# krisbrud/gym-auv

Measured on NVIDIA B200. Metric: env-steps/sec (180-ray LiDAR, whole box), higher is better.
Workload: dtype f32 ray casting on f64 state/culling

## Files before the change

gym_auv_b200/_lib.py:

```python
from __future__ import annotations

import ctypes as C
import os

_HERE = os.path.dirname(os.path.abspath(__file__))
LIB_PATH = os.environ.get("AUV_B200_LIB", os.path.join(_HERE, "libauv_b200.so"))
ABI_VERSION = 22
REC_BYTES = 80
MAX_POLY_VERTS = 192
STATUS_REC_OVERFLOW = 1
STATUS_GEN_GAVE_UP = 2
STATUS_POLY_TOO_LARGE = 4
STATUS_PATH_TOO_LONG = 8
STATUS_BOUNDS = 16
STATUS_GEN_LAND_BLOCKED = 32
PP_W = 12
PATH_STAGE_BLOCKS = 512
NAV_W = 24
N_STATS = 16
STAT_NAMES = [
    "episodes",
    "reward",
    "reward_sq",
    "progress",
    "collisions",
    "reached_goal",
    "timesteps",
    "cross_track_error",
    "pathlength",
    "steps",
]

OBSERVE_STEP = 0
OBSERVE_RESET = 1
REWARDER_IDS = {"colav": 0, "pathfollow": 1}
CULL_IDS = {"reference": 0, "exact": 1}
VELOCITY_IDS = {"zero": 0, "nearest": 1}

_vp = C.c_void_p


class AuvConfig(C.Structure):
    _fields_ = [
        ("t_step_size", C.c_double),
        ("thrust_max_auv", C.c_double),
        ("moment_max_auv", C.c_double),
        ("vessel_width", C.c_double),
        ("look_ahead_distance", C.c_double),
        ("sensor_range", C.c_double),
        ("min_goal_distance", C.c_double),
        ("min_path_progress", C.c_double),
        ("min_cumulative_reward", C.c_double),
        ("feasibility_width_multiplier", C.c_double),
        ("max_timesteps", C.c_int32),
        ("sensor_interval_load_obstacles", C.c_int32),
        ("n_sensors", C.c_int32),
        ("n_sectors", C.c_int32),
        ("use_lidar", C.c_int32),
        ("sensor_log_transform", C.c_int32),
        ("sensor_use_velocity_observations", C.c_int32),
        ("rewarder", C.c_int32),
        ("test_mode", C.c_int32),
        ("cull_mode", C.c_int32),
        ("auto_reset", C.c_int32),
        ("velocity_mode", C.c_int32),
    ]


class AuvRayTable(C.Structure):
    _fields_ = [("cos_sin", _vp), ("weight", _vp), ("sector", _vp), ("unit64", _vp), ("weight_sum", C.c_double)]


class AuvPathHdr(C.Structure):
    _fields_ = [
        ("v0", C.c_int32),
        ("nseg", C.c_int32),
        ("b0", C.c_int32),
        ("s0", C.c_int32),
        ("ox", C.c_double),
        ("oy", C.c_double),
        ("length", C.c_double),
        ("end_x", C.c_double),
        ("end_y", C.c_double),
        ("extent", C.c_double),
    ]


class AuvPathBank(C.Structure):
    _fields_ = [
        ("n_paths", C.c_int32),
        ("n_knots", C.c_int32),
        ("hdr", _vp),
        ("poly_xy", _vp),
        ("poly_cum", _vp),
        ("poly_f32", _vp),
        ("blk_chord", _vp),
        ("blk_dev", _vp),
        ("sb_chord", _vp),
        ("sb_dev", _vp),
        ("pp", _vp),
        ("sub_chord", _vp),
        ("sub_dev", _vp),
    ]


class AuvScenarioPool(C.Structure):
    _fields_ = [
        ("n_scenarios", C.c_int32),
        ("k_moving", C.c_int32),
        ("k_static", C.c_int32),
        ("n_world", C.c_int32),
        ("path_id", _vp),
        ("vessel_init", _vp),
        ("mov_start", _vp),
        ("mov_width", _vp),
        ("mov_track", _vp),
        ("mov_pos0", _vp),
        ("mov_disp0", _vp),
        ("mov_counter0", _vp),
        ("vel_table", _vp),
        ("st_pos", _vp),
        ("st_radius", _vp),
        ("st_rec", _vp),
        ("mov_lin", _vp),
        ("linear_tracks", C.c_int32),
        ("lin_first_wrap", C.c_int32),
        ("lin_wrap_period", C.c_int32),
        ("reserved0", C.c_int32),
        ("world_circle", _vp),
        ("world_voff", _vp),
        ("world_verts", _vp),
        ("world_cell_off", _vp),
        ("world_cell_items", _vp),
        ("world_grid_x0", C.c_double),
        ("world_grid_y0", C.c_double),
        ("world_grid_cell", C.c_double),
        ("world_grid_nx", C.c_int32),
        ("world_grid_ny", C.c_int32),
        ("reset_obs", _vp),
        ("reset_max_progress", _vp),
        ("reset_mask", _vp),
    ]


class AuvBatch(C.Structure):
    _fields_ = [
        ("n_envs", C.c_int32),
        ("mask_words", C.c_int32),
        ("env_offset", C.c_int32),
        ("reset_stride", C.c_int32),
        ("scn_id", _vp),
        ("episode", _vp),
        ("state", _vp),
        ("step_counter", _vp),
        ("t_step", _vp),
        ("cum_reward", _vp),
        ("max_progress", _vp),
        ("cte_sum", _vp),
        ("nearby_mask", _vp),
        ("mov_pos", _vp),
        ("mov_disp", _vp),
        ("mov_counter", _vp),
        ("nav", _vp),
        ("rec", _vp),
        ("rec_cnt", _vp),
        ("status", _vp),
        ("rec_cap", C.c_int32),
        ("reserved1", C.c_int32),
        ("obst_steps", _vp),
        ("prev_seg", _vp),
        ("env_pid", _vp),
    ]


class AuvStepOut(C.Structure):
    _fields_ = [
        ("obs", _vp),
        ("reward", _vp),
        ("done", _vp),
        ("collision", _vp),
        ("reached_goal", _vp),
        ("goal_distance", _vp),
        ("progress", _vp),
        ("lidar_dist", _vp),
        ("windows", _vp),
        ("terminal_obs", _vp),
        ("sector_min_dist", _vp),
        ("sector_feasible_dist", _vp),
        ("stats", _vp),
        ("seg_tests", _vp),
        ("episode_out", _vp),
        ("tracks", _vp),
    ]


class AuvTracks(C.Structure):
    _fields_ = [("count", C.c_int32), ("stride", C.c_int32), ("capacity", C.c_int32), ("reserved0", C.c_int32),
                ("points", _vp), ("head", _vp), ("snap", _vp)]


TRACK_HEAD_W = 8


def track_snap_width(k_moving: int, k_static: int) -> int:
    return 4 + 8 * int(k_moving) + 4 * int(k_static)


class AuvGenParams(C.Structure):
    _fields_ = [
        ("seed", C.c_uint64),
        ("epoch", C.c_uint32),
        ("post_generate_update", C.c_int32),
        ("t_step_size", C.c_double),
        ("vessel_width", C.c_double),
        ("init_pos_jitter", C.c_double),
        ("mov_disp_std", C.c_double),
        ("mov_width_mean", C.c_double),
        ("mov_speed_lo", C.c_double),
        ("mov_speed_hi", C.c_double),
        ("st_disp_std", C.c_double),
        ("st_radius_mean", C.c_double),
        ("path_group", C.c_int32),
        ("path_period", C.c_int32),
        ("land_clearance", C.c_double),
    ]


class AuvRefreshScratch(C.Structure):
    _fields_ = [("seen_episode", _vp), ("ids", _vp), ("count", _vp), ("capacity", C.c_int32), ("reserved0", C.c_int32)]


class AuvPathBuild(C.Structure):
    _fields_ = [("hdr", _vp), ("poly_xy", _vp), ("poly_cum", _vp), ("poly_f32", _vp), ("blk_chord", _vp), ("blk_dev", _vp),
                ("sb_chord", _vp), ("sb_dev", _vp), ("pp", _vp), ("n_knots", C.c_int32), ("vcap", C.c_int32),
                ("sub_chord", _vp), ("sub_dev", _vp)]


class AuvCompact(C.Structure):
    _fields_ = [("head", _vp), ("mask", _vp), ("vals", _vp), ("counter", _vp), ("words", C.c_int32), ("capacity", C.c_int32)]


class AuvDelta(C.Structure):
    _fields_ = [("obs_host", _vp), ("shadow", _vp), ("shipped", _vp), ("gran", C.c_int32), ("ctas", C.c_int32)]


EXPORTS = [
    "auv_abi_version",
    "auv_sizeof",
    "auv_last_error",
    "auv_obs_dim",
    "auv_obstacle_update",
    "auv_vessel_step",
    "auv_navigate",
    "auv_observe",
    "auv_reset",
    "auv_step",
    "auv_step_host",
    "auv_fma_probe",
    "auv_timer_create",
    "auv_timer_destroy",
    "auv_step_timed",
    "auv_timer_read",
    "auv_pipeline_create",
    "auv_pipeline_destroy",
    "auv_pipeline_graph_state",
    "auv_step_chunked",
    "auv_step_host_chunked",
    "auv_step_host_submit",
    "auv_generate_moving_obstacles",
    "auv_linear_wrap",
    "auv_pool_pack",
    "auv_obstacle_state",
    "auv_reset_cache_fill",
    "auv_refresh_finished",
    "auv_step_host_compact_submit",
    "auv_step_host_delta_submit",
    "auv_compact_expand",
    "auv_pathbank_build",
    "auv_random_curve_waypoints",
]

_lib = None


class AuvLibraryError(RuntimeError):
    pass


def load():
    global _lib
    if _lib is not None:
        return _lib
    if not os.path.exists(LIB_PATH):
        raise AuvLibraryError(
            f"{LIB_PATH} not found: build it with `python -m gym_auv_b200.build` "
            "(or __graft_entry__.build()).  There is no CPU fallback."
        )
    lib = C.CDLL(LIB_PATH)
    for name in EXPORTS:
        if not hasattr(lib, name):
            raise AuvLibraryError(f"{LIB_PATH} does not export {name}")
    lib.auv_abi_version.restype = C.c_int
    lib.auv_last_error.restype = C.c_char_p
    lib.auv_obs_dim.argtypes = [C.POINTER(AuvConfig)]
    P = C.POINTER
    lib.auv_obstacle_update.argtypes = [P(AuvConfig), P(AuvScenarioPool), P(AuvBatch), _vp]
    lib.auv_vessel_step.argtypes = [P(AuvConfig), P(AuvBatch), _vp, _vp]
    lib.auv_observe.argtypes = [
        P(AuvConfig), P(AuvRayTable), P(AuvPathBank), P(AuvScenarioPool), P(AuvBatch), P(AuvStepOut), C.c_int, _vp,
    ]
    lib.auv_navigate.argtypes = [P(AuvConfig), P(AuvRayTable), P(AuvPathBank), P(AuvScenarioPool), P(AuvBatch), _vp]
    lib.auv_reset.argtypes = [P(AuvConfig), P(AuvScenarioPool), P(AuvBatch), _vp, _vp]
    lib.auv_step.argtypes = [
        P(AuvConfig), P(AuvRayTable), P(AuvPathBank), P(AuvScenarioPool), P(AuvBatch), _vp, P(AuvStepOut), _vp,
    ]
    lib.auv_step_host.argtypes = [
        P(AuvConfig), P(AuvRayTable), P(AuvPathBank), P(AuvScenarioPool), P(AuvBatch), _vp, _vp, P(AuvStepOut),
        _vp, _vp, _vp, _vp,
    ]
    lib.auv_pipeline_create.argtypes = [C.c_int]
    lib.auv_pipeline_create.restype = _vp
    lib.auv_pipeline_destroy.argtypes = [_vp]
    lib.auv_pipeline_destroy.restype = None
    lib.auv_pipeline_graph_state.argtypes = [_vp]
    lib.auv_step_chunked.argtypes = [
        P(AuvConfig), P(AuvRayTable), P(AuvPathBank), P(AuvScenarioPool), P(AuvBatch), _vp, P(AuvStepOut), _vp,
        _vp, C.c_int,
    ]
    lib.auv_step_host_chunked.argtypes = [
        P(AuvConfig), P(AuvRayTable), P(AuvPathBank), P(AuvScenarioPool), P(AuvBatch), _vp, _vp, P(AuvStepOut),
        _vp, _vp, _vp, _vp, _vp, C.c_int,
    ]
    lib.auv_step_host_submit.argtypes = lib.auv_step_host_chunked.argtypes
    lib.auv_generate_moving_obstacles.argtypes = [P(AuvGenParams), P(AuvPathBank), P(AuvScenarioPool), _vp, C.c_int, _vp, _vp]
    lib.auv_linear_wrap.argtypes = [C.c_double, C.c_double, C.c_int, P(C.c_int32), P(C.c_int32)]
    lib.auv_pool_pack.argtypes = [P(AuvConfig), P(AuvScenarioPool), _vp, C.c_int, _vp]
    lib.auv_obstacle_state.argtypes = [P(AuvConfig), P(AuvScenarioPool), P(AuvBatch), _vp, _vp, _vp, _vp]
    lib.auv_reset_cache_fill.argtypes = [P(AuvConfig), P(AuvRayTable), P(AuvPathBank), P(AuvScenarioPool), P(AuvBatch),
                                         P(AuvStepOut), _vp, C.c_int, C.c_int, _vp]
    lib.auv_refresh_finished.argtypes = [P(AuvConfig), P(AuvRayTable), P(AuvPathBank), P(AuvScenarioPool), P(AuvBatch),
                                         P(AuvBatch), P(AuvStepOut), P(AuvRefreshScratch), P(AuvGenParams), _vp]
    lib.auv_step_host_compact_submit.argtypes = [
        P(AuvConfig), P(AuvRayTable), P(AuvPathBank), P(AuvScenarioPool), P(AuvBatch), _vp, _vp, P(AuvStepOut),
        P(AuvCompact), _vp, _vp, _vp, _vp, C.c_int,
    ]
    lib.auv_step_host_delta_submit.argtypes = [
        P(AuvConfig), P(AuvRayTable), P(AuvPathBank), P(AuvScenarioPool), P(AuvBatch), _vp, _vp, P(AuvStepOut),
        P(AuvDelta), _vp, _vp, _vp, _vp, C.c_int,
    ]
    lib.auv_compact_expand.argtypes = [P(AuvConfig), C.c_int, P(AuvCompact), _vp, _vp, C.c_int]
    lib.auv_pathbank_build.argtypes = [_vp, _vp, _vp, C.c_int, P(AuvPathBuild), _vp, _vp]
    lib.auv_random_curve_waypoints.argtypes = [C.c_uint64, C.c_uint32, C.c_double, _vp, C.c_int, _vp, _vp, _vp]
    lib.auv_timer_create.argtypes = [C.c_int]
    lib.auv_timer_create.restype = _vp
    lib.auv_timer_destroy.argtypes = [_vp]
    lib.auv_timer_destroy.restype = None
    lib.auv_step_timed.argtypes = [
        P(AuvConfig), P(AuvRayTable), P(AuvPathBank), P(AuvScenarioPool), P(AuvBatch), _vp, P(AuvStepOut), _vp,
        _vp, C.c_int,
    ]
    lib.auv_timer_read.argtypes = [_vp, C.c_int, P(C.c_float)]
    lib.auv_fma_probe.argtypes = [_vp, C.c_int, C.c_int, C.c_int, _vp, P(C.c_double)]
    ver = lib.auv_abi_version()
    if ver != ABI_VERSION:
        raise AuvLibraryError(f"ABI mismatch: library {ver}, binding {ABI_VERSION}; rebuild")
    lib.auv_sizeof.argtypes = [C.c_int]
    for i, st in enumerate([AuvConfig, AuvRayTable, AuvPathBank, AuvScenarioPool, AuvBatch, AuvStepOut, AuvGenParams,
                            AuvPathHdr, AuvRefreshScratch, AuvCompact, AuvPathBuild, AuvDelta, AuvTracks]):
        if lib.auv_sizeof(i) != C.sizeof(st):
            raise AuvLibraryError(f"struct layout mismatch for {st.__name__}: C {lib.auv_sizeof(i)} vs ctypes {C.sizeof(st)}")
    _lib = lib
    return lib


def check(rc: int, what: str):
    if rc != 0:
        msg = load().auv_last_error().decode("utf-8", "replace")
        raise AuvLibraryError(f"{what} failed (rc={rc}): {msg}")
```

gym_auv_b200/csrc/auv_kernels.cu:

```cuda
#include "auv_device.cuh"
#include "auv_dynamics.cuh"
#include "auv_geometry.cuh"
#include "auv_navigate.cuh"
#include "auv_generate.cuh"
#include "auv_pathbuild.cuh"
#include "../../include/auv_b200.h"

#include <math.h>

namespace auv {

struct ObstLoad {
  double w, counter;
  int4 tr;
  double2 pos;
};
__device__ __forceinline__ ObstLoad obstacle_load(const AuvScenarioPool& pool, const AuvBatch& batch, long long pe,
                                                  long long ps) {
  ObstLoad o;
  o.w = pool.mov_width[ps];
  o.counter = batch.mov_counter[pe];
  o.tr = reinterpret_cast<const int4*>(pool.mov_track)[ps];
  o.pos = reinterpret_cast<const double2*>(batch.mov_pos)[pe];
  return o;
// ... 127 lines not shown
  double hx, hy;
  float ecx, ecy, rho;
  int a, b;
  int flags;
  int nv;
  int vbase;
  float step_len;
  int pad;
};
static_assert(sizeof(ObstRec) == AUV_REC_BYTES, "ObstRec layout");

__device__ __forceinline__ void reset_env_thread(const AuvScenarioPool& pool, const AuvBatch& batch, int e,
                                                 int scn) {
  const int n = batch.n_envs;
  const int km = pool.k_moving;
  batch.scn_id[e] = scn;
  batch.env_pid[e] = pool.path_id[scn];
  batch.prev_seg[e] = -1;
  batch.obst_steps[e] = 0;
  batch.episode[e] += 1;
  const double* vi = pool.vessel_init + 3ll * scn;
  batch.state[e] = vi[0];
  batch.state[n + e] = vi[1];
  batch.state[2 * n + e] = vi[2];
  batch.state[3 * n + e] = 0.0;
  batch.state[4 * n + e] = 0.0;
  batch.state[5 * n + e] = 0.0;
  batch.step_counter[e] = 0;
  batch.t_step[e] = 0;
  batch.cum_reward[e] = 0.0;
  batch.max_progress[e] = 0.0;
  batch.cte_sum[e] = 0.0;
  if (!pool.linear_tracks)
    for (int j = 0; j < km; ++j) {
      const long long ps = (long long)scn * km + j, pe = (long long)e * km + j;
      reinterpret_cast<double2*>(batch.mov_pos)[pe] = reinterpret_cast<const double2*>(pool.mov_pos0)[ps];
      reinterpret_cast<double2*>(batch.mov_disp)[pe] = reinterpret_cast<const double2*>(pool.mov_disp0)[ps];
      batch.mov_counter[pe] = pool.mov_counter0[ps];
    }
  for (int w = 0; w < batch.mask_words; ++w) batch.nearby_mask[(long long)e * batch.mask_words + w] = 0u;
}

__global__ void __launch_bounds__(128) k_reset(AuvScenarioPool pool, AuvBatch batch,
                                               const uint8_t* __restrict__ reset_mask) {
  const int e = blockIdx.x * blockDim.x + threadIdx.x;
  if (e >= batch.n_envs) return;
  if (reset_mask != nullptr && reset_mask[e] == 0) return;
  reset_env_thread(pool, batch, e, batch.scn_id[e]);
}

struct SlotGeom {
  bool valid, pent, world;
  double cx, cy, rho, geo, hx, hy;
  float step_len;
  int nv, vbase;
};

__device__ __forceinline__ SlotGeom load_slot(const AuvScenarioPool& pool, const AuvBatch& batch, int e, int scn,
                                              int j, double px, double py, int n_upd) {
  SlotGeom g;
  g.valid = g.pent = g.world = false;
  g.cx = g.cy = g.rho = g.geo = 0.0;
  g.hx = 1.0;
  g.hy = 0.0;
  g.step_len = 0.f;
  g.nv = g.vbase = 0;
  const int km = pool.k_moving, ks = pool.k_static, K = km + ks;
  if (j >= K) {
    const int wi = j - K;
    const double* c3 = pool.world_circle + 3ll * wi;
    g.vbase = pool.world_voff[wi];
    g.nv = pool.world_voff[wi + 1] - g.vbase;
    g.valid = g.nv >= 4;
    g.world = true;
    g.cx = c3[0] - px;
    g.cy = c3[1] - py;
    g.rho = c3[2];
  } else if (j < km) {
    const long long ps = (long long)scn * km + j;
    double w;
    double2 pos, dsp;
    if (pool.linear_tracks) {
      const double2* __restrict__ r = reinterpret_cast<const double2*>(pool.mov_lin + ps * 8);
      const double2 p0 = r[0];
      dsp = r[1];
      w = r[2].x;
      pos = p0;
      if (w > 0.0) {
        pos = lin_position(pool, r, p0, dsp, n_upd);
        if (n_upd == 0) dsp = reinterpret_cast<const double2*>(pool.mov_disp0)[ps];
      }
    } else {
      const long long pe = (long long)e * km + j;
      w = pool.mov_width[ps];
      pos = reinterpret_cast<const double2*>(batch.mov_pos)[pe];
      dsp = reinterpret_cast<const double2*>(batch.mov_disp)[pe];
    }
    if (w > 0.0) {
      g.valid = g.pent = true;
      g.geo = w;
      const double dl2 = dsp.x * dsp.x + dsp.y * dsp.y;
      if (dl2 > 0.0) {
        const double inv = rsqrt(dl2);
        g.hx = dsp.x * inv;
        g.hy = dsp.y * inv;
        g.step_len = (float)(dl2 * inv);
      }
      g.cx = (pos.x - px) + w * (5.0 / 18.0) + (w * (2.0 / 9.0)) * g.hx;
      g.cy = (pos.y - py) + (w * (2.0 / 9.0)) * g.hy;
      g.rho = w * 1.1180339887498949;
      g.nv = 6;
    }
  } else {
    const double2* __restrict__ r = reinterpret_cast<const double2*>(pool.st_rec + ((long long)scn * ks + (j - km)) * 4);
    const double2 c = r[0];
    const double rad = r[1].x;
    if (rad > 0.0) {
      g.valid = true;
      g.geo = rad;
      g.cx = c.x - px;
      g.cy = c.y - py;
      g.rho = rad;
      g.nv = ngon_sides(rad) + 1;
    }
  }
  return g;
}

__device__ __forceinline__ bool slot_is_near(const AuvScenarioPool& pool, const AuvBatch& batch,
                                             const double2* __restrict__ unit64, int e, int scn, int j, double px,
                                             double py, int n_upd, double range, double width) {
  const SlotGeom g = load_slot(pool, batch, e, scn, j, px, py, n_upd);
  if (!g.valid) return false;
  const double dc = sqrt(g.cx * g.cx + g.cy * g.cy);
  if (dc - g.rho - width >= range + 1e-6) return false;
  if (dc + g.rho - width < range - 1e-6) return true;
  const double bx0 = g.cx - (g.geo * (2.0 / 9.0)) * g.hx, by0 = g.cy - (g.geo * (2.0 / 9.0)) * g.hy;
  bool in_dummy;
  const double dist = g.world ? world_polygon_distance(reinterpret_cast<const double2*>(pool.world_verts) + g.vbase, g.nv, px,
                                                       py, in_dummy)
                              : boundary_distance(g.pent, g.cx, g.cy, bx0, by0, g.geo, g.hx, g.hy, g.nv, unit64);
  return (dist - width) < range;
}

#ifndef AUV_CULL_COOP
#define AUV_CULL_COOP 1
#endif
template <int G>
__device__ __forceinline__ void cull_env_group(const AuvConfig& cfg, const AuvScenarioPool& pool,
                                               const AuvBatch& batch, const double2* __restrict__ unit64,
                                               int* __restrict__ windows_out, int e, int scn, double px,
                                               double py, double psi, int step_counter, int n_upd, const int lane,
                                               const unsigned gm, const bool store) {
  const int sub = lane & (G - 1);
  const int R = cfg.n_sensors;
  const int S = pool.k_moving + pool.k_static + pool.n_world;
  const bool refresh = (step_counter % cfg.sensor_interval_load_obstacles) == 0;
  const double range = cfg.sensor_range, width = cfg.vessel_width;
  ObstRec* rec = reinterpret_cast<ObstRec*>(batch.rec) + (long long)e * batch.rec_cap;
  int cnt = 0;
  const int K = pool.k_moving + pool.k_static;
  const bool grid = pool.world_cell_off != nullptr && pool.n_world > 0;
  const int S_scan = grid ? K : S;
#if AUV_CULL_COOP
  const unsigned rmask = __ballot_sync(AUV_FULL, refresh && sub == 0 && store);
  for (unsigned rm = rmask; rm; rm &= rm - 1) {
    const int src = __ffs(rm) - 1;
    const int eb = __shfl_sync(AUV_FULL, e, src), sb = __shfl_sync(AUV_FULL, scn, src);
    const int nb = __shfl_sync(AUV_FULL, n_upd, src);
    const double pxb = __shfl_sync(AUV_FULL, px, src), pyb = __shfl_sync(AUV_FULL, py, src);
    for (int base = 0; base < S; base += 32) {
      unsigned word = 0u;
      if (base < S_scan) {
        const int j = base + lane;
        word = __ballot_sync(AUV_FULL, j < S_scan && slot_is_near(pool, batch, unit64, eb, sb, j, pxb, pyb, nb, range, width));
      }
      if (lane == src) batch.nearby_mask[(long long)eb * batch.mask_words + (base >> 5)] = word;
    }
  }
  if (rmask) __syncwarp();
#endif
  if (refresh) {
#if !AUV_CULL_COOP
    for (int base = 0; base < S; base += 32) {
      unsigned word = 0u;
      if (base < S_scan) {
#pragma unroll 1
        for (int k = 0; k < 32 / G; ++k) {
          const int j = base + k * G + sub;
          const bool near = j < S_scan && slot_is_near(pool, batch, unit64, e, scn, j, px, py, n_upd, range, width);
          word |= group_ballot<G>(gm, lane, near) << (k * G);
        }
      }
      if (store && sub == 0) batch.nearby_mask[(long long)e * batch.mask_words + (base >> 5)] = word;
    }
#endif
    if (grid) {
      __syncwarp(gm);
      const double rq = range + width + 1e-3, cell = pool.world_grid_cell;
      const int ix0 = max(0, (int)floor((px - rq - pool.world_grid_x0) / cell));
      const int ix1 = min(pool.world_grid_nx - 1, (int)floor((px + rq - pool.world_grid_x0) / cell));
      const int iy0 = max(0, (int)floor((py - rq - pool.world_grid_y0) / cell));
      const int iy1 = min(pool.world_grid_ny - 1, (int)floor((py + rq - pool.world_grid_y0) / cell));
      for (int iy = iy0; iy <= iy1; ++iy)
        for (int ix = ix0; ix <= ix1; ++ix) {
          const int c = iy * pool.world_grid_nx + ix;
          const int i0 = pool.world_cell_off[c], i1 = pool.world_cell_off[c + 1];
          for (int it = i0 + sub; it < i1; it += G) {
            const int j = K + pool.world_cell_items[it];
            if (store && slot_is_near(pool, batch, unit64, e, scn, j, px, py, n_upd, range, width))
              atomicOr(batch.nearby_mask + (long long)e * batch.mask_words + (j >> 5), 1u << (j & 31));
          }
        }
    }
    __syncwarp(gm);
  }
  for (int base = 0; base < S; base += 32) {
    const unsigned* mw = batch.nearby_mask + (long long)e * batch.mask_words + (base >> 5);
    const unsigned word = refresh ? __ldcg(mw) : *mw;
    if (windows_out != nullptr && store) {
      for (int j = base + sub; j < min(S, base + 32); j += G)
        reinterpret_cast<int2*>(windows_out)[(long long)e * S + j] = make_int2(0, 0);
      __syncwarp(gm);
    }
    const int nw = __popc(word);
    for (int r = sub; r < nw; r += G) {
      unsigned wv = word;
      for (int t = 0; t < r; ++t) wv &= wv - 1;
      const int j = base + __ffs(wv) - 1;
      const SlotGeom g = load_slot(pool, batch, e, scn, j, px, py, n_upd);
      int wa = 0, wb = 0;
      bool allrays = false, inside = false;
      double bx0 = 0.0, by0 = 0.0;
      if (g.valid) {
        int lo, hi;
        cull_bounds(g.cx, g.cy, g.rho, psi, R, lo, hi);
        window_from_bounds(lo, hi, R, cfg.cull_mode, wa, wb, allrays);
        bx0 = g.cx - (g.geo * (2.0 / 9.0)) * g.hx;
        by0 = g.cy - (g.geo * (2.0 / 9.0)) * g.hy;
        if (g.cx * g.cx + g.cy * g.cy <= g.rho * g.rho) {
          if (g.pent)
            inside = vessel_inside_pentagon(bx0, by0, g.geo, g.hx, g.hy);
          else if (g.world)
            world_polygon_distance(reinterpret_cast<const double2*>(pool.world_verts) + g.vbase, g.nv, px, py, inside);
        }
      }
      if (!store) continue;
      if (windows_out != nullptr) reinterpret_cast<int2*>(windows_out)[(long long)e * S + j] = make_int2(wa, wb);
      const int idx = cnt + r;
      AUV_CHECK(batch.status, j >= 0 && j < S && idx >= 0);
      if (idx >= batch.rec_cap) {
        if (batch.status != nullptr) atomicOr(batch.status, AUV_STATUS_REC_OVERFLOW);
        continue;
      }
      ObstRec q;
      q.cx = g.pent ? bx0 : g.cx;
      q.cy = g.pent ? by0 : g.cy;
      q.geo = g.geo;
      q.hx = g.hx;
      q.hy = g.hy;
      q.ecx = (float)g.cx;
      q.ecy = (float)g.cy;
      q.rho = (float)g.rho;
      q.a = wa;
      q.b = wb;
      q.flags = (g.pent ? (OFLAG_FILLED | OFLAG_PENTAGON) : 0) | (g.world ? (OFLAG_FILLED | OFLAG_WORLD) : 0) |
                (inside ? OFLAG_INSIDE : 0) | (allrays ? OFLAG_ALLRAYS : 0);
      q.nv = g.valid ? g.nv : 1;
      q.vbase = g.vbase;
      q.step_len = g.step_len;
      q.pad = 0;
      rec[idx] = q;
    }
    cnt = min(cnt + nw, batch.rec_cap);
  }
  if (store && sub == 0) {
    batch.rec_cnt[e] = cnt;
    batch.nav[(long long)e * AUV_NAV_W + NAV_CNT] = (double)cnt;
  }
}

__global__ void __launch_bounds__(128) k_worker_fill(AuvBatch wb, const int* __restrict__ ids, int first, int n,
                                                     const int* __restrict__ n_dev) {
  const int w = blockIdx.x * blockDim.x + threadIdx.x;
  if (w >= wb.n_envs) return;
  if (n_dev != nullptr) n = min(n, *n_dev);
  const int k = n > 0 ? min(w, n - 1) : 0;
  wb.scn_id[w] = ids ? ids[k] : first + k;
}
__global__ void __launch_bounds__(128) k_cache_scatter(AuvScenarioPool pool, AuvBatch wb, const float* __restrict__ wobs,
                                                       int obs_dim, int use_lidar, int n, const int* __restrict__ n_dev) {
  const int w = (blockIdx.x * blockDim.x + threadIdx.x) >> 5, lane = threadIdx.x & 31;
  if (n_dev != nullptr) n = min(n, *n_dev);
  if (w >= n || w >= wb.n_envs) return;
  const int m = wb.scn_id[w];
  float* dst = const_cast<float*>(pool.reset_obs) + (long long)m * obs_dim;
  const float* src = wobs + (long long)w * obs_dim;
  for (int k = lane; k < obs_dim; k += 32) dst[k] = src[k];
  if (lane == 0) const_cast<double*>(pool.reset_max_progress)[m] = wb.max_progress[w];
  if (use_lidar)
    for (int k = lane; k < wb.mask_words; k += 32)
      const_cast<uint32_t*>(pool.reset_mask)[(long long)m * wb.mask_words + k] = wb.nearby_mask[(long long)w * wb.mask_words + k];
}
__global__ void __launch_bounds__(128) k_refresh_collect(AuvBatch live, int n_scenarios, int* __restrict__ seen,
                                                         int* __restrict__ ids, int* __restrict__ count, int capacity) {
  const int e = blockIdx.x * blockDim.x + threadIdx.x;
  if (e >= live.n_envs) return;
  const int ep = live.episode[e];
  if (ep == seen[e]) return;
  const int k = atomicAdd(count, 1);
  if (k >= capacity) return;
  seen[e] = ep;
  ids[k] = (int)(((long long)live.scn_id[e] + (live.reset_stride > 0 ? live.reset_stride : live.n_envs)) % n_scenarios);
}

template <int G>
__device__ __noinline__ void obstacle_update_group(const AuvConfig& cfg, const AuvScenarioPool& pool, const AuvBatch& batch,
                                                   int e, int scn, int sub, bool store) {
  if (!store) return;
  const int km = pool.k_moving;
  const long long pe0 = (long long)e * km, ps0 = (long long)scn * km;
  for (int j = sub; j < km; j += 2 * G) {
    const bool two = j + G < km;
    const ObstLoad a = obstacle_load(pool, batch, pe0 + j, ps0 + j);
    const ObstLoad b = obstacle_load(pool, batch, pe0 + (two ? j + G : j), ps0 + (two ? j + G : j));
    obstacle_finish(cfg, pool, batch, pe0 + j, ps0 + j, a);
    if (two) obstacle_finish(cfg, pool, batch, pe0 + j + G, ps0 + j + G, b);
  }
}

__device__ __forceinline__ unsigned smem_u32(const void* p) { return (unsigned)__cvta_generic_to_shared(p); }
__device__ __forceinline__ void mbar_init(unsigned long long* bar, unsigned count) {
  asm volatile("mbarrier.init.shared::cta.b64 [%0], %1;" ::"r"(smem_u32(bar)), "r"(count) : "memory");
  asm volatile("fence.mbarrier_init.release.cluster;" ::: "memory");
}
__device__ __forceinline__ void mbar_expect_tx(unsigned long long* bar, unsigned bytes) {
  asm volatile("mbarrier.arrive.expect_tx.shared::cta.b64 _, [%0], %1;" ::"r"(smem_u32(bar)), "r"(bytes) : "memory");
}
__device__ __forceinline__ void bulk_g2s(void* dst, const void* src, unsigned bytes, unsigned long long* bar) {
  asm volatile("cp.async.bulk.shared::cluster.global.mbarrier::complete_tx::bytes [%0], [%1], %2, [%3];" ::"r"(smem_u32(dst)),
               "l"(src), "r"(bytes), "r"(smem_u32(bar))
               : "memory");
}
__device__ __forceinline__ void mbar_wait(unsigned long long* bar, unsigned parity) {
  asm volatile(
      "{\n"
      ".reg .pred p;\n"
      "AUV_WAIT:\n"
      "mbarrier.try_wait.parity.shared::cta.b64 p, [%0], %1;\n"
      "@p bra AUV_DONE;\n"
      "bra AUV_WAIT;\n"
      "AUV_DONE:\n"
      "}\n" ::"r"(smem_u32(bar)),
      "r"(parity)
      : "memory");
}

#ifndef AUV_NAV_G
#define AUV_NAV_G 4
#endif
#ifndef AUV_NAV_THREADS
#define AUV_NAV_THREADS 128
#endif
#ifndef AUV_NAV_MINB
#define AUV_NAV_MINB (1024 / AUV_NAV_THREADS)
#endif
#ifndef AUV_NAV_PHASE_SYNC
#define AUV_NAV_PHASE_SYNC 0
#endif
constexpr int NAV_STAGE_SB = (AUV_PATH_STAGE_BLOCKS + AUV_PATH_SUPER - 1) / AUV_PATH_SUPER;
constexpr int NAV_SUBBLOCKS = AUV_NAV_THREADS / 128;
struct __align__(16) NavStage {
  float4 chord[AUV_PATH_STAGE_BLOCKS];
  float2 aux[AUV_PATH_STAGE_BLOCKS];
  float4 sbc[NAV_STAGE_SB];
  float2 sba[NAV_STAGE_SB];
};
#ifndef AUV_NAV_SPLIT
#define AUV_NAV_SPLIT 1
#endif
template <bool DYN, bool OBST, int G>
__global__ void __launch_bounds__(AUV_NAV_THREADS, AUV_NAV_MINB) k_vessel_nav(const __grid_constant__ AuvConfig cfg,
                                                                const __grid_constant__ AuvPathBank paths,
                                                                const __grid_constant__ AuvScenarioPool pool,
                                                                const __grid_constant__ AuvBatch batch,
                                                                const double2* __restrict__ unit64,
                                                                int* __restrict__ windows_out,
                                                                const float* __restrict__ actions,
                                                                float* __restrict__ obs_out, int obs_dim, int e0, int e1) {
  extern __shared__ __align__(16) unsigned char nav_smem[];
  NavStage* stages = reinterpret_cast<NavStage*>(nav_smem);
  __shared__ __align__(8) unsigned long long s_bar[NAV_SUBBLOCKS];
  __shared__ int s_pid[AUV_NAV_THREADS / 32];
  const int lane = threadIdx.x & 31, sub = lane & (G - 1);
  const int sbk = threadIdx.x >> 7, tsb = threadIdx.x & 127;
  NavStage& st = stages[sbk];
  const unsigned gm = group_mask<G>(lane);
  const int eraw = e0 + (blockIdx.x * AUV_NAV_THREADS + threadIdx.x) / G;
  const bool store = eraw < e1;
  const int e = store ? eraw : e1 - 1;
  const int n = batch.n_envs;
  const int scn = batch.scn_id[e];
  const int pid = batch.env_pid[e];
  const int prev_seg = batch.prev_seg[e];
  int step_counter = batch.step_counter[e];
  int n_upd = batch.obst_steps[e];
  S6 y = load_state(batch.state, n, e);
  float2 act = make_float2(0.f, 0.f);
  if (DYN) act = reinterpret_cast<const float2*>(actions)[e];
  if (tsb == 0) mbar_init(&s_bar[sbk], 1);
  {
    int same;
    __match_all_sync(AUV_FULL, pid, &same);
    if (lane == 0) s_pid[threadIdx.x >> 5] = same ? pid : -1;
  }
  __syncthreads();
  const AuvPathHdr h = paths.hdr[pid];
  const int nblk = (h.nseg + AUV_PATH_BLOCK - 1) / AUV_PATH_BLOCK;
  const int nsb = (nblk + AUV_PATH_SUPER - 1) / AUV_PATH_SUPER;
  bool staged = s_pid[4 * sbk] >= 0 && nblk <= AUV_PATH_STAGE_BLOCKS;
#pragma unroll
  for (int w = 1; w < 4; ++w) staged = staged && s_pid[4 * sbk + w] == s_pid[4 * sbk];
  if (staged && tsb == 0) {
    const unsigned nb2 = (unsigned)(nblk + 1) & ~1u, ns2 = (unsigned)(nsb + 1) & ~1u;
    mbar_expect_tx(&s_bar[sbk], nb2 * 24u + ns2 * 24u);
    bulk_g2s(st.chord, reinterpret_cast<const float4*>(paths.blk_chord) + h.b0, nb2 * 16u, &s_bar[sbk]);
    bulk_g2s(st.aux, reinterpret_cast<const float2*>(paths.blk_dev) + h.b0, nb2 * 8u, &s_bar[sbk]);
    bulk_g2s(st.sbc, reinterpret_cast<const float4*>(paths.sb_chord) + h.s0, ns2 * 16u, &s_bar[sbk]);
    bulk_g2s(st.sba, reinterpret_cast<const float2*>(paths.sb_dev) + h.s0, ns2 * 8u, &s_bar[sbk]);
  }
  if (OBST) {
    ++n_upd;
    if (store && sub == 0) batch.obst_steps[e] = n_upd;
    if (!pool.linear_tracks) {
      obstacle_update_group<G>(cfg, pool, batch, e, scn, sub, store);
      __syncwarp();
    }
  }
  if (DYN) {
    y = vessel_rk_step(cfg, y, act);
    ++step_counter;
    if (store && sub == 0) {
      store_state(batch.state, n, e, y);
      batch.step_counter[e] = step_counter;
    }
  }
  if (AUV_NAV_PHASE_SYNC) __syncthreads();
  PathTabs T;
  if (staged) {
    mbar_wait(&s_bar[sbk], 0);
    T.sbc = st.sbc;
    T.sba = st.sba;
    T.chord = st.chord;
    T.aux = st.aux;
  } else {
    T.sbc = reinterpret_cast<const float4*>(paths.sb_chord) + h.s0;
    T.sba = reinterpret_cast<const float2*>(paths.sb_dev) + h.s0;
    T.chord = reinterpret_cast<const float4*>(paths.blk_chord) + h.b0;
    T.aux = reinterpret_cast<const float2*>(paths.blk_dev) + h.b0;
  }
  int seg;
  const double s = project_group<G>(paths, h, T, y.x, y.y, prev_seg, lane, gm, seg, batch.status);
  AUV_CHECK(batch.status, seg >= 0 && seg < h.nseg && (!staged || (nblk <= AUV_PATH_STAGE_BLOCKS && nsb <= NAV_STAGE_SB)));
  if (store && sub == 0) batch.prev_seg[e] = seg;
  if (AUV_NAV_SPLIT) {
    if (store && sub == 0) batch.nav[(long long)e * AUV_NAV_W + NAV_S] = s;
    return;
  }
  if (AUV_NAV_PHASE_SYNC) __syncthreads();
  navigate_env(cfg, paths, h, batch, pid, e, scn, s, y.x, y.y, y.psi, y.u, y.v, y.r,
               obs_out ? obs_out + (long long)e * obs_dim : nullptr, store && sub == 0);
  if (AUV_NAV_PHASE_SYNC) __syncthreads();
  if (cfg.use_lidar)
    cull_env_group<G>(cfg, pool, batch, unit64, windows_out, e, scn, y.x, y.y, y.psi, step_counter, n_upd, lane, gm, store);
}

template <int G>
__global__ void __launch_bounds__(128, 8) k_nav_cull(const __grid_constant__ AuvConfig cfg, const __grid_constant__ AuvPathBank paths,
                                                     const __grid_constant__ AuvScenarioPool pool,
                                                     const __grid_constant__ AuvBatch batch, const double2* __restrict__ unit64,
                                                     int* __restrict__ windows_out, float* __restrict__ obs_out, int obs_dim,
                                                     int e0, int e1) {
  const int lane = threadIdx.x & 31, sub = lane & (G - 1);
  const unsigned gm = group_mask<G>(lane);
  const int eraw = e0 + (blockIdx.x * 128 + threadIdx.x) / G;
  const bool store = eraw < e1;
  const int e = store ? eraw : e1 - 1;
  const int n = batch.n_envs;
  const int scn = batch.scn_id[e];
  const int pid = batch.env_pid[e];
  const int step_counter = batch.step_counter[e];
  const int n_upd = batch.obst_steps[e];
  const S6 y = load_state(batch.state, n, e);
  const double s = batch.nav[(long long)e * AUV_NAV_W + NAV_S];
  const AuvPathHdr h = paths.hdr[pid];
  __syncwarp();
  navigate_env(cfg, paths, h, batch, pid, e, scn, s, y.x, y.y, y.psi, y.u, y.v, y.r,
               obs_out ? obs_out + (long long)e * obs_dim : nullptr, store && sub == 0);
  if (cfg.use_lidar)
    cull_env_group<G>(cfg, pool, batch, unit64, windows_out, e, scn, y.x, y.y, y.psi, step_counter, n_upd, lane, gm, store);
}

#ifndef AUV_LIDAR_THREADS
#define AUV_LIDAR_THREADS 256
#endif
#ifndef AUV_LIDAR_RCAP
#define AUV_LIDAR_RCAP 96
#endif
#ifndef AUV_LIDAR_MAX_ENVS
#define AUV_LIDAR_MAX_ENVS 32
#endif

struct LidarArgs {
  AuvConfig cfg;
  AuvRayTable rays;
  AuvPathBank paths;
  AuvScenarioPool pool;
  AuvBatch batch;
  AuvStepOut out;
  const void* pad0;
  int mode;
  int obs_dim;
  int e0, e1;
  int envs_per_cta;
  int vmax;
  float pen_clear_ray;
  float inv_log_range;
  double clear_closeness;
  double inv_weight_sum;
  double feas_width;
  AuvTracks trk;
};

struct LidarSmem {
  double* hand;
  void* sdist;
  ObstRec* rec;
  int* rec_env;
  float2* verts;
  float2* unit;
  int* off;
  float* pen;
  int* flag;
  int* next;
};
__host__ __device__ constexpr size_t lidar_smem_bytes_for(int E, int rpad, int vmax, int vel) {
  return (size_t)E * 16 * 8 + (size_t)E * rpad * (vel ? 8 : 4) + AUV_LIDAR_RCAP * sizeof(ObstRec) + AUV_LIDAR_RCAP * 4 +
         (size_t)(AUV_LIDAR_THREADS / 32) * vmax * 8 + 64 * 8 + 48 * 4 + 32 * 4 + 32 * 4 + 32 * 4;
}
__device__ __forceinline__ LidarSmem lidar_carve(unsigned char* p, int E, int rpad, int vmax, int vel) {
  LidarSmem s;
  s.hand = reinterpret_cast<double*>(p);
  p += (size_t)E * 16 * 8;
  s.sdist = p;
  p += (size_t)E * rpad * (vel ? 8 : 4);
  s.rec = reinterpret_cast<ObstRec*>(p);
  p += AUV_LIDAR_RCAP * sizeof(ObstRec);
  s.rec_env = reinterpret_cast<int*>(p);
  p += AUV_LIDAR_RCAP * 4;
  s.verts = reinterpret_cast<float2*>(p);
  p += (size_t)(AUV_LIDAR_THREADS / 32) * vmax * 8;
  s.unit = reinterpret_cast<float2*>(p);
  p += 64 * 8;
  s.off = reinterpret_cast<int*>(p);
  p += 48 * 4;
  s.pen = reinterpret_cast<float*>(p);
  p += 32 * 4;
  s.flag = reinterpret_cast<int*>(p);
  p += 32 * 4;
  s.next = reinterpret_cast<int*>(p);
  return s;
}

__device__ __forceinline__ float cast_ngon(float ecx, float ecy, float rho, int nn, const float2* __restrict__ u64,
                                           float c, float s, float theta, float tc, float hc, float best, float rangef) {
  const float g = asinf(fminf(fmaxf(-hc / rho, -1.f), 1.f));
  const float invd = (float)nn * 0.15915494309189535f;
  const int sh = 6 - (31 - __clz(nn));
  const bool outside = tc * tc + hc * hc > rho * rho * 1.0001f + 1e-3f;
#pragma unroll
  for (int sol = 0; sol < 2; ++sol) {
    if (sol == 1 && outside) break;
    const float p = (sol == 0 ? theta + 3.14159265358979f - g : theta + g) * invd;
    const float kf = floorf(p);
    const int k0 = (int)kf;
    const int first = (p - kf < 0.5f) ? k0 - 1 : k0;
    float xp, yp;
    {
      const float2 un = u64[(first & (nn - 1)) << sh];
      const float vx = fmaf(rho, un.x, ecx), vy = fmaf(rho, un.y, ecy);
      xp = vx * c + vy * s;
      yp = vy * c - vx * s;
    }
#pragma unroll
    for (int w = 1; w <= 2; ++w) {
      const float2 un = u64[((first + w) & (nn - 1)) << sh];
      const float vx = fmaf(rho, un.x, ecx), vy = fmaf(rho, un.y, ecy);
      const float xc = vx * c + vy * s;
      const float yc = vy * c - vx * s;
      if ((yp <= 0.f && yc >= 0.f) || (yp >= 0.f && yc <= 0.f)) {
        const float t = xp + (xc - xp) * (yp / (yp - yc));
        if (t >= 0.f && t <= rangef) best = fminf(best, t);
      }
      xp = xc;
      yp = yc;
    }
  }
  return best;
}

__device__ __forceinline__ float cast_chain(const float2* __restrict__ vp, int nq, float c, float s, float best,
                                            float rangef) {
  float2 v = vp[0];
  float xp = v.x * c + v.y * s;
  float yp = v.y * c - v.x * s;
  for (int k = 1; k < nq; ++k) {
    v = vp[k];
    const float xc = v.x * c + v.y * s;
    const float yc = v.y * c - v.x * s;
    if ((yp <= 0.f && yc >= 0.f) || (yp >= 0.f && yc <= 0.f)) {
      const float t = xp + (xc - xp) * (yp / (yp - yc));
      if (t >= 0.f && t <= rangef) best = fminf(best, t);
    }
    xp = xc;
    yp = yc;
  }
  return best;
}

template <bool VEL>
__device__ __forceinline__ float range_get(const void* row, int i) {
  if (VEL) return __uint_as_float((unsigned)(reinterpret_cast<const unsigned long long*>(row)[i] >> 32));
  return reinterpret_cast<const float*>(row)[i];
}
template <bool VEL>
__device__ __forceinline__ void range_min(void* row, int i, float d, int slot) {
  if (VEL)
    atomicMin(reinterpret_cast<unsigned long long*>(row) + i,
              ((unsigned long long)__float_as_uint(d) << 32) | (unsigned)min(slot, 255));
  else
    atomicMin(reinterpret_cast<int*>(row) + i, __float_as_int(d));
}

#ifndef AUV_LIDAR_MINB
#define AUV_LIDAR_MINB 5
#endif
#ifndef AUV_LIDAR_LONG_POLY
#define AUV_LIDAR_LONG_POLY 1
#endif
template <bool VEL>
__device__ __noinline__ void cast_long_polygon(const double2* __restrict__ wv, int nq, int vmax, float2* wverts, double px,
                                               double py, double cpsi, double spsi, const double2* __restrict__ cos_sin,
                                               float ecx, float ecy, float rho, void* row, int slot, int lane, int n1, int n2,
                                               int lo1, int lo2, float rangef) {
  const float slack = rho * 1e-5f + 1e-4f;
  const int tot = n1 + n2;
  for (int v0 = 0; v0 < nq - 1; v0 += vmax - 1) {
    const int nqc = min(nq - v0, vmax);
    __syncwarp();
    for (int k = lane; k < nqc; k += 32) {
      const double2 w = wv[v0 + k];
      wverts[k] = make_float2((float)(w.x - px), (float)(w.y - py));
    }
    __syncwarp();
    for (int u = lane; u < tot; u += 32) {
      const int i = u < n1 ? lo1 + u : lo2 + (u - n1);
      const float cur = range_get<VEL>(row, i);
      const double2 cs = cos_sin[i];
      const float c = (float)(cs.x * cpsi - cs.y * spsi), sn = (float)(cs.y * cpsi + cs.x * spsi);
      const float tc = ecx * c + ecy * sn;
      const float hc = ecy * c - ecx * sn;
      if (fabsf(hc) > rho + slack || tc + rho + slack < 0.f || tc - rho - slack > cur) continue;
      const float got = cast_chain(wverts, nqc, c, sn, cur, rangef);
      if (got < cur) range_min<VEL>(row, i, got, slot);
    }
  }
}

template <bool COUNT, bool VEL, bool WORLD, bool TRACK = false>
__global__ void __launch_bounds__(AUV_LIDAR_THREADS, AUV_LIDAR_MINB) k_lidar(const __grid_constant__ LidarArgs A) {
  extern __shared__ __align__(16) unsigned char smem_raw[];
  constexpr int NW = AUV_LIDAR_THREADS / 32;
  const AuvConfig& cfg = A.cfg;
  const AuvBatch& batch = A.batch;
  const int tid = threadIdx.x, lane = tid & 31, warp = tid >> 5;
  const int R = cfg.n_sensors;
  const int rpad = cfg.use_lidar ? ((R + 31) & ~31) : 32;
  const int E = A.envs_per_cta;
  const int env0 = A.e0 + blockIdx.x * E;
  const int ne = min(E, A.e1 - env0);
  const LidarSmem sm = lidar_carve(smem_raw, E, rpad, A.vmax, VEL ? 1 : 0);
  const float rangef = (float)cfg.sensor_range;
  const float widthf = (float)cfg.vessel_width;
  const int n = batch.n_envs;
#define HAND(el, k) sm.hand[(el) * 16 + ((k) - NAV_HAND)]

  for (int k = tid; k < ne * 16; k += AUV_LIDAR_THREADS)
    sm.hand[k] = batch.nav[(long long)(env0 + (k >> 4)) * AUV_NAV_W + NAV_HAND + (k & 15)];
  if (cfg.use_lidar) {
    if (tid < 64) {
      const double2 un = reinterpret_cast<const double2*>(A.rays.unit64)[tid];
      sm.unit[tid] = make_float2((float)un.x, (float)un.y);
    }
    if (VEL) {
      const unsigned long long key0 = ((unsigned long long)__float_as_uint(rangef) << 32) | 255ull;
      for (int k = tid; k < ne * rpad; k += AUV_LIDAR_THREADS) reinterpret_cast<unsigned long long*>(sm.sdist)[k] = key0;
    } else {
      for (int k = tid; k < ne * rpad / 4; k += AUV_LIDAR_THREADS)
        reinterpret_cast<float4*>(sm.sdist)[k] = make_float4(rangef, rangef, rangef, rangef);
    }
  }
  __syncthreads();
  unsigned long long ntests = 0;
  if (cfg.use_lidar) {
    if (warp == 0) {
      const int c = lane < ne ? (int)HAND(lane, NAV_CNT) : 0;
      const int incl = warp_incl_scan(c, lane);
      sm.off[lane + 1] = incl;
      if (lane == 0) sm.off[0] = 0;
    }
    __syncthreads();
    const int total = sm.off[ne];
    const double2* __restrict__ unit = reinterpret_cast<const double2*>(A.rays.unit64);
    const double2* __restrict__ cos_sin = reinterpret_cast<const double2*>(A.rays.cos_sin);
    const float dth_f = (float)(2.0 * AUV_PI / (double)R);
    float2* wverts = sm.verts + (size_t)warp * A.vmax;
    for (int r0 = 0; r0 < total; r0 += AUV_LIDAR_RCAP) {
      const int nr = min(AUV_LIDAR_RCAP, total - r0);
      for (int k = tid; k < nr * 5; k += AUV_LIDAR_THREADS) {
        const int r = r0 + k / 5, piece = k - (k / 5) * 5;
        int lo = 0, hi = ne - 1;
        while (lo < hi) {
          const int mid = (lo + hi + 1) >> 1;
          if (sm.off[mid] <= r) lo = mid; else hi = mid - 1;
        }
        const int idx = r - sm.off[lo];
        AUV_CHECK(batch.status, lo >= 0 && lo < ne && idx >= 0 && idx < batch.rec_cap && k < AUV_LIDAR_RCAP * 5);
        const uint4* g = reinterpret_cast<const uint4*>(reinterpret_cast<const ObstRec*>(batch.rec) +
                                                        (long long)(env0 + lo) * batch.rec_cap + idx);
        reinterpret_cast<uint4*>(sm.rec)[k] = g[piece];
        if (piece == 0) sm.rec_env[r - r0] = lo | (idx << 8);
      }
      __syncthreads();
      for (int rr = warp; rr < nr; rr += NW) {
        const ObstRec& q = sm.rec[rr];
        const int el = sm.rec_env[rr] & 255, slot = sm.rec_env[rr] >> 8;
        const int fl = q.flags, nq = q.nv;
        AUV_CHECK(batch.status, rr < AUV_LIDAR_RCAP && el >= 0 && el < ne && slot >= 0 && slot < batch.rec_cap);
        int n1, n2 = 0, lo1 = 0, lo2 = 0;
        if (fl & OFLAG_ALLRAYS) {
          n1 = R;
        } else {
          lo1 = max(q.a, 0);
          const int hi1 = min(q.b, R);
          n1 = max(0, hi1 - lo1);
          lo2 = max(q.a + R, 0);
          if (n1 > 0) lo2 = max(lo2, hi1);
          n2 = max(0, min(q.b + R, R) - lo2);
        }
        const int tot = n1 + n2;
        if (COUNT) {
          for (int i = lane; i < R; i += 32) {
            const int hits = ((q.a <= i && i < q.b) ? 1 : 0) + ((q.a <= i - R && i - R < q.b) ? 1 : 0);
            if ((fl & OFLAG_ALLRAYS) || hits > 0) ntests += (unsigned)((nq - 1) * max(hits, 1));
          }
        }
        if (tot == 0) continue;
        void* row = VEL ? (void*)(reinterpret_cast<unsigned long long*>(sm.sdist) + (size_t)el * rpad)
                        : (void*)(reinterpret_cast<float*>(sm.sdist) + (size_t)el * rpad);
        if (fl & OFLAG_INSIDE) {
          for (int u = lane; u < tot; u += 32) range_min<VEL>(row, u < n1 ? lo1 + u : lo2 + (u - n1), 0.f, slot);
          continue;
        }
        const bool world = WORLD && (fl & OFLAG_WORLD);
        const bool ngon = !(fl & OFLAG_PENTAGON) && !world && nq > 16;
        if (!ngon) {
          if (nq > A.vmax) {
            if (AUV_LIDAR_LONG_POLY && world)
              cast_long_polygon<VEL>(reinterpret_cast<const double2*>(A.pool.world_verts) + q.vbase, nq, A.vmax, wverts,
                                     HAND(el, NAV_X), HAND(el, NAV_Y), HAND(el, NAV_COSPSI), HAND(el, NAV_SINPSI), cos_sin,
                                     q.ecx, q.ecy, q.rho, row, slot, lane, n1, n2, lo1, lo2, rangef);
            else if (lane == 0 && batch.status != nullptr)
              atomicOr(batch.status, AUV_STATUS_POLY_TOO_LARGE);
            continue;
          }
          __syncwarp();
          if (world) {
            const double px = HAND(el, NAV_X), py = HAND(el, NAV_Y);
            const double2* wv = reinterpret_cast<const double2*>(A.pool.world_verts) + q.vbase;
            for (int k = lane; k < nq; k += 32) {
              const double2 w = wv[k];
              wverts[k] = make_float2((float)(w.x - px), (float)(w.y - py));
            }
          } else if (fl & OFLAG_PENTAGON) {
            if (lane < 6) {
              double vx, vy;
              pent_vertex(lane == 5 ? 0 : lane, q.cx, q.cy, q.geo, q.hx, q.hy, vx, vy);
              wverts[lane] = make_float2((float)vx, (float)vy);
            }
          } else {
            const int ne_ = nq - 1, sh = 6 - (31 - __clz(ne_));
            if (lane < nq) {
              const double2 un = __ldg(&unit[(lane == ne_ ? 0 : lane) << sh]);
              wverts[lane] = make_float2((float)(q.cx + q.geo * un.x), (float)(q.cy + q.geo * un.y));
            }
          }
          __syncwarp();
        }
        const double cpsi = HAND(el, NAV_COSPSI), spsi = HAND(el, NAV_SINPSI);
        const float psi_m_pi = (float)(HAND(el, NAV_PSI) - AUV_PI);
        const float ecx = q.ecx, ecy = q.ecy, rho = q.rho;
        const float slack = rho * 1e-5f + 1e-4f;
        AUV_CHECK(batch.status, tot <= R && (n1 == 0 || (lo1 >= 0 && lo1 + n1 <= R)) && (n2 == 0 || (lo2 >= 0 && lo2 + n2 <= R)) &&
                                    (ngon || nq <= A.vmax));
        for (int u = lane; u < tot; u += 32) {
          const int i = u < n1 ? lo1 + u : lo2 + (u - n1);
          AUV_CHECK(batch.status, i >= 0 && i < R && i < rpad);
          const float cur = range_get<VEL>(row, i);
          const double2 cs = cos_sin[i];
          const float c = (float)(cs.x * cpsi - cs.y * spsi), sn = (float)(cs.y * cpsi + cs.x * spsi);
          const float tc = ecx * c + ecy * sn;
          const float hc = ecy * c - ecx * sn;
          if (fabsf(hc) > rho + slack || tc + rho + slack < 0.f || tc - rho - slack > cur) continue;
          float got;
          if (ngon) {
            const float theta = fmaf((float)(i + 1), dth_f, psi_m_pi);
            got = cast_ngon(ecx, ecy, rho, nq - 1, sm.unit, c, sn, theta, tc, hc, cur, rangef);
          } else {
            got = cast_chain(wverts, nq, c, sn, cur, rangef);
          }
          if (got < cur) range_min<VEL>(row, i, got, slot);
        }
      }
      __syncthreads();
    }
  }
  if (COUNT) {
#pragma unroll
    for (int o = 16; o > 0; o >>= 1) ntests += __shfl_xor_sync(AUV_FULL, ntests, o);
    if (lane == 0 && ntests) atomicAdd(A.out.seg_tests, ntests);
  }

  if (cfg.use_lidar) {
    const bool pooling = A.out.sector_min_dist != nullptr || A.out.sector_feasible_dist != nullptr;
    const bool vel_obs = cfg.sensor_use_velocity_observations != 0;
    const bool vec2 = (A.obs_dim & 1) == 0;
    const double2* __restrict__ cos_sin = reinterpret_cast<const double2*>(A.rays.cos_sin);
    for (int el = warp; el < ne; el += NW) {
      const int e = env0 + el;
      float* obs = A.out.obs + (long long)e * A.obs_dim;
      const int cnt = sm.off[el + 1] - sm.off[el];
      const void* row = VEL ? (const void*)(reinterpret_cast<const unsigned long long*>(sm.sdist) + (size_t)el * rpad)
                            : (const void*)(reinterpret_cast<const float*>(sm.sdist) + (size_t)el * rpad);
      float extra = 0.f;
      bool collision = false;
      if (cnt > 0) {
        const double cpsi = HAND(el, NAV_COSPSI), spsi = HAND(el, NAV_SINPSI);
        const ObstRec* grec = reinterpret_cast<const ObstRec*>(batch.rec) + (long long)e * batch.rec_cap;
        for (int k = lane; k < (R + 1) / 2; k += 32) {
          float cl2[2] = {0.f, 0.f};
#pragma unroll
          for (int h = 0; h < 2; ++h) {
            const int i = 2 * k + h;
            if (i >= R) continue;
            const float d = range_get<VEL>(row, i);
            float vxr = 0.f, vyr = 0.f;
            if (d < rangef) {
              if (cfg.sensor_log_transform)
                cl2[h] = 1.f - fminf(fmaxf(__logf(1.f + d) * A.inv_log_range, 0.f), 1.f);
              else
                cl2[h] = 1.f - fminf(fmaxf(d / rangef, 0.f), 1.f);
              cl2[h] = fminf(fmaxf(cl2[h], -1.f), 1.f);
              if (VEL) {
                const int slot = (int)(reinterpret_cast<const unsigned long long*>(row)[i] & 255ull);
                const ObstRec& q = grec[slot];
                if (q.flags & OFLAG_PENTAGON) {
                  const double2 cs = cos_sin[i];
                  const double c = cs.x * cpsi - cs.y * spsi, sn = cs.y * cpsi + cs.x * spsi;
                  const double dx = (double)q.step_len * q.hx, dy = (double)q.step_len * q.hy;
                  vxr = (float)(-sn * dx + c * dy);
                  vyr = (float)(-c * dx - sn * dy);
                }
              }
              extra += A.rays.weight[i] * (rangef * __expf(-0.1f * d + fmaxf(0.f, vyr)) - A.pen_clear_ray);
              collision = collision || (d < widthf);
            }
            if (vel_obs) {
              obs[6 + R + i] = fminf(fmaxf(vxr, -1.f), 1.f);
              obs[6 + 2 * R + i] = fminf(fmaxf(vyr, -1.f), 1.f);
            }
            if (!vec2) obs[6 + i] = cl2[h];
          }
          if (vec2) {
            if (2 * k + 1 < R)
              reinterpret_cast<float2*>(obs + 6)[k] = make_float2(cl2[0], cl2[1]);
            else
              obs[6 + 2 * k] = cl2[0];
          }
        }
        collision = __any_sync(AUV_FULL, collision);
        extra = warp_sum(extra);
      } else {
        if (vec2) {
          float2* o2 = reinterpret_cast<float2*>(obs + 6);
          for (int k = lane; k < R / 2; k += 32) o2[k] = make_float2(0.f, 0.f);
          if ((R & 1) && lane == 0) obs[6 + R - 1] = 0.f;
        } else {
          for (int i = lane; i < R; i += 32) obs[6 + i] = 0.f;
        }
        if (vel_obs)
          for (int k = lane; k < 2 * R; k += 32) obs[6 + R + k] = 0.f;
      }
      if (lane == 0) {
        sm.pen[el] = extra;
        sm.flag[el] = collision ? 1 : 0;
      }
      if (A.out.lidar_dist != nullptr)
        for (int i = lane; i < R; i += 32) A.out.lidar_dist[(long long)e * R + i] = range_get<VEL>(row, i);

      if (pooling) {
        const int ns = cfg.n_sectors;
        float* prow = reinterpret_cast<float*>(sm.verts + (size_t)warp * A.vmax);
        float* ssec = prow;
        __syncwarp();
        ssec[lane] = rangef;
        __syncwarp();
        for (int i0 = 0; i0 < R; i0 += 32) {
          const int i = i0 + lane;
          float d = i < R ? range_get<VEL>(row, i) : INFINITY;
          const int sid = i < R ? (int)A.rays.sector[i] : -1 - lane;
#pragma unroll
          for (int o = 1; o < 32; o <<= 1) {
            const float od = __shfl_down_sync(AUV_FULL, d, o);
            const int os = __shfl_down_sync(AUV_FULL, sid, o);
            if (lane + o < 32 && os == sid) d = fminf(d, od);
          }
          const int ps = __shfl_up_sync(AUV_FULL, sid, 1);
          const bool head = i < R && (lane == 0 || ps != sid);
          if (head && sid < 32) ssec[sid] = fminf(ssec[sid], d);
          __syncwarp();
        }
        if (A.out.sector_min_dist != nullptr && lane < ns) A.out.sector_min_dist[(long long)e * ns + lane] = ssec[lane];
        if (A.out.sector_feasible_dist != nullptr) {
          const float* frow;
          if (VEL) {
            float* tmp = reinterpret_cast<float*>(const_cast<void*>(row));
            __syncwarp();
            for (int i0 = 0; i0 < R; i0 += 32) {
              const int i = i0 + lane;
              const float d = i < R ? range_get<VEL>(row, i) : 0.f;
              __syncwarp();
              if (i < R) tmp[i] = d;
              __syncwarp();
            }
            frow = tmp;
          } else {
            frow = reinterpret_cast<const float*>(row);
          }
          if (lane < ns) {
            int lo = 0, hi = R;
            for (int k = 0; k < R; ++k) {
              const int sd = A.rays.sector[k];
              if (sd < lane) lo = k + 1;
              if (sd <= lane) hi = k + 1;
            }
            A.out.sector_feasible_dist[(long long)e * ns + lane] =
                hi > lo ? feasibility_pooling(frow + lo, hi - lo, A.feas_width, 2.0 * AUV_PI / (double)R) : rangef;
          }
        }
        __syncwarp();
      }
    }
  }
  __syncthreads();

  if (warp == 0 && lane < ne) {
    const int el = lane, e = env0 + el;
    const bool collision = cfg.use_lidar && (sm.flag[el] & 1);
    const double progress = HAND(el, NAV_H_PROGRESS), goal_dist = HAND(el, NAV_H_GOAL);
    const bool reached = HAND(el, NAV_REACHED) != 0.0;
    int fl = 0;
    if (A.mode == AUV_OBSERVE_RESET) {
      if (A.out.collision) A.out.collision[e] = collision;
// ... 154 lines not shown
      if (v != 0.f) s_vals[el * rpad + run + __popc(m & ((1u << lane) - 1u))] = v;
      if (lane == 0) s_mask[el * words + w] = m;
      run += __popc(m);
    }
    if (lane == 0) s_off[el + 1] = run;
  }
  __syncthreads();
  if (warp == 0) {
    const int c = lane < ne ? s_off[lane + 1] : 0;
    const int incl = warp_incl_scan(c, lane);
    __syncwarp();
    s_off[lane + 1] = incl;
    if (lane == 0) s_off[0] = 0;
    const int total = __shfl_sync(AUV_FULL, incl, 31);
    if (lane == 0) s_base = total > 0 ? atomicAdd(counter, (total + 31) & ~31) : 0;
  }
  __syncthreads();
  const int base = s_base, total = s_off[ne];
  for (int k = tid; k < ne * 8; k += AUV_SHIP_THREADS) {
    const int el = k >> 3, f = k & 7;
    float v;
    if (f < 6) v = obs[(long long)(env0 + el) * obs_dim + f];
    else if (f == 6) v = __int_as_float(s_off[el + 1] - s_off[el]);
    else v = __int_as_float(base + s_off[el]);
    head_h[(long long)env0 * 8 + k] = v;
  }
  for (int k = tid; k < ne * words; k += AUV_SHIP_THREADS) mask_h[(long long)env0 * words + k] = s_mask[k];
  if (tid < ne) {
    reward_h[env0 + tid] = reward[env0 + tid];
    done_h[env0 + tid] = done[env0 + tid];
  }
  if (base + total <= capacity)
    for (int k = tid; k < total; k += AUV_SHIP_THREADS) {
      int lo = 0, hi = ne - 1;
      while (lo < hi) {
        const int mid = (lo + hi + 1) >> 1;
        if (s_off[mid] <= k) lo = mid; else hi = mid - 1;
      }
      vals_h[base + k] = s_vals[lo * rpad + (k - s_off[lo])];
    }
}

#define AUV_DELTA_THREADS 64
#define AUV_DELTA_UNROLL 2
__global__ void __launch_bounds__(AUV_DELTA_THREADS, 24) k_obs_delta(const float* __restrict__ obs, float* __restrict__ shadow,
                                                                float* __restrict__ obs_h, long long f0, long long f1, int g4,
                                                                const float* __restrict__ reward,
                                                                const uint8_t* __restrict__ done, float* __restrict__ reward_h,
                                                                uint8_t* __restrict__ done_h, int e0, int e1,
                                                                unsigned long long* __restrict__ shipped) {
  const int lane = threadIdx.x & 31;
  const long long nthreads = (long long)gridDim.x * AUV_DELTA_THREADS;
  const long long gtid = (long long)blockIdx.x * AUV_DELTA_THREADS + threadIdx.x;
  for (long long e = e0 + gtid; e < e1; e += nthreads) {
    reward_h[e] = reward[e];
    done_h[e] = done[e];
  }
  const long long qfull = f1 >> 2, qend = (f1 + 3) >> 2;
  const unsigned cm = (g4 >= 32 ? 0xffffffffu : ((1u << g4) - 1u)) << (lane & ~(g4 - 1));
  unsigned count = 0u;
  for (long long qb = (f0 >> 2) + gtid - lane; qb < qend; qb += nthreads * AUV_DELTA_UNROLL) {
    uint4 cur[AUV_DELTA_UNROLL], old[AUV_DELTA_UNROLL];
#pragma unroll
    for (int u = 0; u < AUV_DELTA_UNROLL; ++u) {
      const long long q = qb + u * nthreads + lane;
      cur[u] = old[u] = make_uint4(0u, 0u, 0u, 0u);
      if (q < qfull) {
        cur[u] = __ldcs(reinterpret_cast<const uint4*>(obs) + q);
        old[u] = __ldcs(reinterpret_cast<const uint4*>(shadow) + q);
      }
    }
#pragma unroll
    for (int u = 0; u < AUV_DELTA_UNROLL; ++u) {
      const long long q = qb + u * nthreads + lane;
      const bool full = q < qfull, part = !full && q < qend;
      bool changed = (cur[u].x != old[u].x) | (cur[u].y != old[u].y) | (cur[u].z != old[u].z) | (cur[u].w != old[u].w);
      if (part)
        for (long long i = q << 2; i < f1; ++i) changed |= __float_as_uint(obs[i]) != __float_as_uint(shadow[i]);
      const unsigned any = __ballot_sync(AUV_FULL, changed);
      const bool ship = (any & cm) != 0u;
      if (ship) {
        if (full) {
          reinterpret_cast<uint4*>(obs_h)[q] = cur[u];
          reinterpret_cast<uint4*>(shadow)[q] = cur[u];
        } else if (part) {
          for (long long i = q << 2; i < f1; ++i) obs_h[i] = shadow[i] = obs[i];
        }
      }
      count += __popc(__ballot_sync(AUV_FULL, ship && (full || part) && (lane & (g4 - 1)) == 0));
    }
  }
  if (shipped != nullptr && lane == 0 && count) atomicAdd(shipped, (unsigned long long)count);
}

__global__ void __launch_bounds__(256) k_fma_probe(float* sink, int iters) {
  float a0 = threadIdx.x * 1e-3f, a1 = a0 + 1.f, a2 = a0 + 2.f, a3 = a0 + 3.f;
  float a4 = a0 + 4.f, a5 = a0 + 5.f, a6 = a0 + 6.f, a7 = a0 + 7.f;
  const float m = 0.999f, c = 1e-3f;
  for (int i = 0; i < iters; ++i) {
    a0 = fmaf(a0, m, c);
    a1 = fmaf(a1, m, c);
    a2 = fmaf(a2, m, c);
    a3 = fmaf(a3, m, c);
    a4 = fmaf(a4, m, c);
    a5 = fmaf(a5, m, c);
    a6 = fmaf(a6, m, c);
    a7 = fmaf(a7, m, c);
  }
  const float r = a0 + a1 + a2 + a3 + a4 + a5 + a6 + a7;
  if (r == 12345.678f) sink[0] = r;
}

}

#include <stdio.h>
#include <stdlib.h>
#include <string.h>
#include <atomic>

static thread_local char g_err[512] = "";

static int set_err(int code, const char* msg) {
  snprintf(g_err, sizeof(g_err), "%s", msg);
  return code;
}
static int cuda_check(cudaError_t e, const char* where) {
  if (e == cudaSuccess) return 0;
  snprintf(g_err, sizeof(g_err), "%s: %s", where, cudaGetErrorString(e));
  return (int)e;
}

extern "C" {

static int check_pool_tracks(const AuvScenarioPool* pool, const AuvBatch* batch);

int auv_abi_version(void) { return AUV_ABI_VERSION; }
int auv_sizeof(int which) {
  switch (which) {
    case 0: return (int)sizeof(AuvConfig);
    case 1: return (int)sizeof(AuvRayTable);
    case 2: return (int)sizeof(AuvPathBank);
    case 3: return (int)sizeof(AuvScenarioPool);
    case 4: return (int)sizeof(AuvBatch);
    case 5: return (int)sizeof(AuvStepOut);
    case 6: return (int)sizeof(AuvGenParams);
    case 7: return (int)sizeof(AuvPathHdr);
    case 8: return (int)sizeof(AuvRefreshScratch);
    case 9: return (int)sizeof(AuvCompact);
    case 10: return (int)sizeof(AuvPathBuild);
    case 11: return (int)sizeof(AuvDelta);
    case 12: return (int)sizeof(AuvTracks);
    default: return AUV_EINVAL;
  }
}
const char* auv_last_error(void) { return g_err; }

int auv_obs_dim(const AuvConfig* cfg) {
  if (!cfg) return AUV_EINVAL;
  int d = 6;
  if (cfg->use_lidar) {
    d += cfg->n_sensors;
    if (cfg->sensor_use_velocity_observations) d += 2 * cfg->n_sensors;
  }
  return d;
}

static int check_cfg(const AuvConfig* cfg) {
  if (!cfg) return set_err(AUV_EINVAL, "cfg is NULL");
  if (cfg->use_lidar && (cfg->n_sensors <= 0 || cfg->n_sensors > AUV_MAX_RAYS))
    return set_err(AUV_EINVAL, "n_sensors out of range");
  if (!(cfg->t_step_size > 0.0)) return set_err(AUV_EINVAL, "t_step_size must be > 0");
  if (cfg->sensor_interval_load_obstacles <= 0)
    return set_err(AUV_EINVAL, "sensor_interval_load_obstacles must be > 0");
  if (cfg->use_lidar && (cfg->n_sectors <= 0 || cfg->n_sectors > 32))
    return set_err(AUV_EINVAL, "n_sectors must be in 1..32");
  return 0;
}

static int launch_obstacle_update(const AuvConfig* cfg, const AuvScenarioPool* pool, const AuvBatch* batch,
                                  int e0, int cnt, void* stream) {
  const long long total = (long long)cnt * pool->k_moving;
  if (total == 0) return 0;
  const int threads = 256;
  const long long blocks = (total + threads - 1) / threads;
  auv::k_obstacle_update<<<(unsigned)blocks, threads, 0, (cudaStream_t)stream>>>(*cfg, *pool, *batch, e0, cnt);
  return cuda_check(cudaGetLastError(), "k_obstacle_update");
}

int auv_obstacle_update(const AuvConfig* cfg, const AuvScenarioPool* pool, AuvBatch* batch,
                        void* stream) {
  if (int rc = check_cfg(cfg)) return rc;
  if (!pool || !batch) return set_err(AUV_EINVAL, "pool/batch is NULL");
  if (batch->n_envs <= 0) return set_err(AUV_EINVAL, "n_envs must be > 0");
  if (!batch->obst_steps) return set_err(AUV_EINVAL, "batch.obst_steps is NULL");
  if (int rc = check_pool_tracks(pool, batch)) return rc;
  return launch_obstacle_update(cfg, pool, batch, 0, batch->n_envs, stream);
}

int auv_vessel_step(const AuvConfig* cfg, AuvBatch* batch, const float* actions, void* stream) {
  if (int rc = check_cfg(cfg)) return rc;
  if (!batch || !actions) return set_err(AUV_EINVAL, "batch/actions is NULL");
  if (batch->n_envs <= 0) return set_err(AUV_EINVAL, "n_envs must be > 0");
  const int threads = 128;
  const int blocks = (batch->n_envs + threads - 1) / threads;
  auv::k_vessel_step<<<blocks, threads, 0, (cudaStream_t)stream>>>(*cfg, *batch, actions);
  return cuda_check(cudaGetLastError(), "k_vessel_step");
}

int auv_reset(const AuvConfig* cfg, const AuvScenarioPool* pool, AuvBatch* batch,
              const uint8_t* reset_mask, void* stream) {
  if (int rc = check_cfg(cfg)) return rc;
  if (!pool || !batch) return set_err(AUV_EINVAL, "pool/batch is NULL");
  if (batch->n_envs <= 0) return set_err(AUV_EINVAL, "n_envs must be > 0");
  if (!batch->obst_steps || !batch->prev_seg || !batch->env_pid)
    return set_err(AUV_EINVAL, "batch.obst_steps / prev_seg / env_pid is NULL");
  if (int rc = check_pool_tracks(pool, batch)) return rc;
  const int threads = 128;
  const int blocks = (batch->n_envs + threads - 1) / threads;
  auv::k_reset<<<blocks, threads, 0, (cudaStream_t)stream>>>(*pool, *batch, reset_mask);
  return cuda_check(cudaGetLastError(), "k_reset");
}

static int check_pool_tracks(const AuvScenarioPool* pool, const AuvBatch* batch) {
  if (pool->k_static > 0 && !pool->st_rec) return set_err(AUV_EINVAL, "pool.st_rec is NULL (auv_pool_pack)");
  if (pool->k_moving > 0) {
    if (pool->linear_tracks) {
      if (!pool->mov_lin) return set_err(AUV_EINVAL, "pool.mov_lin is NULL with linear_tracks (auv_pool_pack)");
      if (pool->lin_first_wrap <= 0 || pool->lin_wrap_period <= 0)
        return set_err(AUV_EINVAL, "pool.lin_first_wrap / lin_wrap_period not set (auv_linear_wrap)");
    } else if (!batch->mov_pos || !batch->mov_disp || !batch->mov_counter) {
      return set_err(AUV_EINVAL, "batch.mov_pos / mov_disp / mov_counter is NULL with table-driven tracks");
    }
  }
  return 0;
}

static int check_batch(const AuvConfig* cfg, const AuvScenarioPool* pool, const AuvBatch* batch) {
  if (batch->n_envs <= 0) return set_err(AUV_EINVAL, "n_envs must be > 0");
  if (!batch->nav) return set_err(AUV_EINVAL, "batch.nav is NULL");
  if (pool->n_world < 0) return set_err(AUV_EINVAL, "n_world < 0");
  const int slots = pool->k_moving + pool->k_static + pool->n_world;
  if (slots > AUV_MAX_OBSTACLES) return set_err(AUV_EINVAL, "too many obstacle slots");
  if (batch->mask_words * 32 < slots) return set_err(AUV_EINVAL, "mask_words too small");
  if (pool->n_world > 0 && (!pool->world_circle || !pool->world_voff || !pool->world_verts))
    return set_err(AUV_EINVAL, "world arrays are NULL");
  if (cfg->use_lidar && (!batch->rec_cnt || (slots > 0 && (!batch->rec || batch->rec_cap <= 0))))
    return set_err(AUV_EINVAL, "batch.rec / rec_cnt / rec_cap missing");
  if (!batch->obst_steps || !batch->prev_seg || !batch->env_pid)
    return set_err(AUV_EINVAL, "batch.obst_steps / prev_seg / env_pid is NULL");
  if (int rc = check_pool_tracks(pool, batch)) return rc;
  return 0;
}

static int check_tracks(const AuvStepOut* out, const AuvBatch* batch) {
  const AuvTracks* t = out->tracks;
  if (t == nullptr) return 0;
  if (!t->points || !t->head || !t->snap) return set_err(AUV_EINVAL, "tracks: points / head / snap is NULL");
  if (t->count < 1 || t->stride < 1 || t->capacity < 1)
    return set_err(AUV_EINVAL, "tracks: count, stride and capacity must be >= 1");
  if ((long long)(t->count - 1) * t->stride >= (long long)batch->n_envs)
    return set_err(AUV_EINVAL, "tracks: (count - 1) * stride must be < n_envs");
  if ((size_t)t->points & 15u) return set_err(AUV_EINVAL, "tracks: points must be 16-byte aligned");
  if ((size_t)t->head & 15u) return set_err(AUV_EINVAL, "tracks: head must be 16-byte aligned");
  if ((size_t)t->snap & 7u) return set_err(AUV_EINVAL, "tracks: snap must be 8-byte aligned");
  if (out->seg_tests != nullptr) return set_err(AUV_EINVAL, "tracks cannot be recorded together with out.seg_tests");
  return 0;
}

static int check_observe_args(const AuvConfig* cfg, const AuvRayTable* rays, const AuvPathBank* paths,
                              const AuvScenarioPool* pool, AuvBatch* batch, AuvStepOut* out, int mode) {
  if (int rc = check_cfg(cfg)) return rc;
  if (!paths || !pool || !batch || !out) return set_err(AUV_EINVAL, "NULL argument");
  if (int rc = check_tracks(out, batch)) return rc;
  if (cfg->use_lidar && (!rays || !rays->unit64 || !rays->cos_sin || !rays->weight || !rays->sector))
    return set_err(AUV_EINVAL, "ray table is NULL with use_lidar");
  if (!out->obs) return set_err(AUV_EINVAL, "out.obs is NULL");
  if (mode == AUV_OBSERVE_STEP && (!out->reward || !out->done))
    return set_err(AUV_EINVAL, "out.reward/out.done is NULL");
  if (mode == AUV_OBSERVE_STEP && cfg->auto_reset &&
      (!pool->reset_obs || !pool->reset_max_progress || (cfg->use_lidar && !pool->reset_mask)))
    return set_err(AUV_EINVAL, "auto_reset needs the pool's cached first observations (pool.reset_*)");
  return check_batch(cfg, pool, batch);
}

static int nav_configure(size_t smem) {
  if (smem <= 48 * 1024) return 0;
  static std::atomic<size_t> configured[64];
  int dev = 0;
  if (cudaGetDevice(&dev) != cudaSuccess || dev < 0 || dev >= 64) dev = 0;
  if (smem <= configured[dev].load(std::memory_order_acquire)) return 0;
  const void* fns[3] = {(const void*)auv::k_vessel_nav<true, true, AUV_NAV_G>, (const void*)auv::k_vessel_nav<true, false, AUV_NAV_G>,
                        (const void*)auv::k_vessel_nav<false, false, AUV_NAV_G>};
  for (int i = 0; i < 3; ++i)
    if (int rc = cuda_check(cudaFuncSetAttribute(fns[i], cudaFuncAttributeMaxDynamicSharedMemorySize, (int)smem),
                            "cudaFuncSetAttribute(k_vessel_nav)"))
      return rc;
  configured[dev].store(smem, std::memory_order_release);
  return 0;
}

static int launch_vessel_nav(const AuvConfig* cfg, const AuvRayTable* rays, const AuvPathBank* paths,
                             const AuvScenarioPool* pool, AuvBatch* batch, AuvStepOut* out,
                             const float* actions, void* stream, int e0 = 0, int cnt = -1, bool with_obstacles = false,
                             cudaEvent_t between = nullptr ) {
  if ((paths->sub_chord == nullptr) != (paths->sub_dev == nullptr))
    return set_err(AUV_EINVAL, "paths: sub_chord and sub_dev are both set or both NULL");
  if (cnt < 0) cnt = batch->n_envs - e0;
  const int per_cta = AUV_NAV_THREADS / AUV_NAV_G;
  const int blocks = (cnt + per_cta - 1) / per_cta;
#ifndef AUV_NAV_EXTRA_SMEM
#define AUV_NAV_EXTRA_SMEM 0
#endif
  const size_t nsm = sizeof(auv::NavStage) * auv::NAV_SUBBLOCKS + AUV_NAV_EXTRA_SMEM;
  if (int rc = nav_configure(nsm)) return rc;
  const double2* unit = rays ? reinterpret_cast<const double2*>(rays->unit64) : nullptr;
  int* win = out ? out->windows : nullptr;
  float* obs = out ? out->obs : nullptr;
  const int od = auv_obs_dim(cfg);
  cudaStream_t s = (cudaStream_t)stream;
  if (actions && with_obstacles && pool->k_moving > 0)
    auv::k_vessel_nav<true, true, AUV_NAV_G><<<blocks, AUV_NAV_THREADS, nsm, s>>>(*cfg, *paths, *pool, *batch, unit, win, actions, obs, od, e0, e0 + cnt);
  else if (actions)
    auv::k_vessel_nav<true, false, AUV_NAV_G><<<blocks, AUV_NAV_THREADS, nsm, s>>>(*cfg, *paths, *pool, *batch, unit, win, actions, obs, od, e0, e0 + cnt);
  else
    auv::k_vessel_nav<false, false, AUV_NAV_G><<<blocks, AUV_NAV_THREADS, nsm, s>>>(*cfg, *paths, *pool, *batch, unit, win, nullptr, obs, od, e0, e0 + cnt);
  if (AUV_NAV_SPLIT) {
    if (int rc = cuda_check(cudaGetLastError(), "k_vessel_nav")) return rc;
    if (between != nullptr) cudaEventRecord(between, s);
    auv::k_nav_cull<AUV_NAV_G><<<(cnt + 31) / 32, 128, 0, s>>>(*cfg, *paths, *pool, *batch, unit, win, obs, od, e0, e0 + cnt);
    return cuda_check(cudaGetLastError(), "k_nav_cull");
  }
  return cuda_check(cudaGetLastError(), "k_vessel_nav");
}

static std::atomic<size_t> g_lidar_smem_configured[64];
static int lidar_configure(size_t smem) {
  int dev = 0;
  if (cudaGetDevice(&dev) != cudaSuccess || dev < 0 || dev >= 64) dev = 0;
  if (smem <= g_lidar_smem_configured[dev].load(std::memory_order_acquire)) return 0;
  const void* fns[12] = {(const void*)auv::k_lidar<false, false, false>, (const void*)auv::k_lidar<true, false, false>,
                         (const void*)auv::k_lidar<false, true, false>,  (const void*)auv::k_lidar<true, true, false>,
                         (const void*)auv::k_lidar<false, false, true>,  (const void*)auv::k_lidar<true, false, true>,
                         (const void*)auv::k_lidar<false, true, true>,   (const void*)auv::k_lidar<true, true, true>,
                         (const void*)auv::k_lidar<false, false, false, true>, (const void*)auv::k_lidar<false, true, false, true>,
                         (const void*)auv::k_lidar<false, false, true, true>,  (const void*)auv::k_lidar<false, true, true, true>};
  for (int i = 0; i < 12; ++i)
    if (int rc = cuda_check(cudaFuncSetAttribute(fns[i], cudaFuncAttributeMaxDynamicSharedMemorySize, (int)smem),
                            "cudaFuncSetAttribute(k_lidar)"))
      return rc;
  size_t seen = g_lidar_smem_configured[dev].load(std::memory_order_relaxed);
  while (seen < smem && !g_lidar_smem_configured[dev].compare_exchange_weak(seen, smem, std::memory_order_release)) {
  }
  return 0;
}
static int lidar_vmax(const AuvScenarioPool* pool) { return pool->n_world > 0 ? AUV_MAX_POLY_VERTS : 16; }
static int lidar_velocity(const AuvConfig* cfg) { return cfg->use_lidar && cfg->velocity_mode == AUV_VELOCITY_NEAREST; }
static int lidar_rpad(const AuvConfig* cfg) { return cfg->use_lidar ? ((cfg->n_sensors + 31) & ~31) : 32; }
static int lidar_envs_per_cta(const AuvConfig* cfg) {
  int e = AUV_LIDAR_MAX_ENVS;
  const size_t row = (size_t)lidar_rpad(cfg) * (lidar_velocity(cfg) ? 8 : 4);
  while (e > 1 && row * e > 40 * 1024) e >>= 1;
  return e;
}
static size_t lidar_smem_bytes(const AuvConfig* cfg, const AuvScenarioPool* pool) {
  return auv::lidar_smem_bytes_for(lidar_envs_per_cta(cfg), lidar_rpad(cfg), lidar_vmax(pool), lidar_velocity(cfg));
}

static int launch_lidar(const AuvConfig* cfg, const AuvRayTable* rays, const AuvPathBank* paths,
                        const AuvScenarioPool* pool, AuvBatch* batch, AuvStepOut* out, int mode,
                        void* stream, int e0 = 0, int cnt = -1) {
  if (cnt < 0) cnt = batch->n_envs - e0;
  auv::LidarArgs args;
  args.cfg = *cfg;
  if (rays) args.rays = *rays; else memset(&args.rays, 0, sizeof(args.rays));
  args.paths = *paths;
  args.pool = *pool;
  args.batch = *batch;
  args.out = *out;
  args.mode = mode;
  args.obs_dim = auv_obs_dim(cfg);
  args.e0 = e0;
  args.e1 = e0 + cnt;
  args.envs_per_cta = lidar_envs_per_cta(cfg);
  args.vmax = lidar_vmax(pool);
  args.clear_closeness = -cfg->sensor_range * exp(-0.1 * cfg->sensor_range);
  args.pen_clear_ray = (float)(-args.clear_closeness);
  args.inv_log_range = (float)(1.0 / log1p(cfg->sensor_range));
  args.inv_weight_sum = (rays && rays->weight_sum > 0.0) ? 1.0 / rays->weight_sum : 0.0;
  args.feas_width = cfg->vessel_width * cfg->feasibility_width_multiplier;
  const bool track = out->tracks != nullptr;
  if (track) args.trk = *out->tracks; else memset(&args.trk, 0, sizeof(args.trk));
  const size_t smem = lidar_smem_bytes(cfg, pool);
  if (int rc = lidar_configure(smem)) return rc;
  const int blocks = (cnt + args.envs_per_cta - 1) / args.envs_per_cta;
  cudaStream_t s = (cudaStream_t)stream;
  const bool count = out->seg_tests != nullptr, vel = lidar_velocity(cfg) != 0;
  const bool world = pool->n_world > 0;
#define AUV_LAUNCH_LIDAR(C, V, W) auv::k_lidar<C, V, W><<<blocks, AUV_LIDAR_THREADS, smem, s>>>(args)
#define AUV_LAUNCH_LIDAR_TRACK(V, W) auv::k_lidar<false, V, W, true><<<blocks, AUV_LIDAR_THREADS, smem, s>>>(args)
  if (track) {
    if (world && vel) AUV_LAUNCH_LIDAR_TRACK(true, true);
    else if (world) AUV_LAUNCH_LIDAR_TRACK(false, true);
    else if (vel) AUV_LAUNCH_LIDAR_TRACK(true, false);
    else AUV_LAUNCH_LIDAR_TRACK(false, false);
  } else if (world) {
    if (count && vel) AUV_LAUNCH_LIDAR(true, true, true);
    else if (count) AUV_LAUNCH_LIDAR(true, false, true);
    else if (vel) AUV_LAUNCH_LIDAR(false, true, true);
    else AUV_LAUNCH_LIDAR(false, false, true);
  } else {
    if (count && vel) AUV_LAUNCH_LIDAR(true, true, false);
    else if (count) AUV_LAUNCH_LIDAR(true, false, false);
    else if (vel) AUV_LAUNCH_LIDAR(false, true, false);
    else AUV_LAUNCH_LIDAR(false, false, false);
  }
#undef AUV_LAUNCH_LIDAR
#undef AUV_LAUNCH_LIDAR_TRACK
  return cuda_check(cudaGetLastError(), "k_lidar");
}

int auv_navigate(const AuvConfig* cfg, const AuvRayTable* rays, const AuvPathBank* paths,
                 const AuvScenarioPool* pool, AuvBatch* batch, void* stream) {
  if (int rc = check_cfg(cfg)) return rc;
  if (!paths || !pool || !batch) return set_err(AUV_EINVAL, "NULL argument");
  if (cfg->use_lidar && (!rays || !rays->unit64)) return set_err(AUV_EINVAL, "ray table is NULL with use_lidar");
  if (int rc = check_batch(cfg, pool, batch)) return rc;
  return launch_vessel_nav(cfg, rays, paths, pool, batch, nullptr, nullptr, stream);
}

int auv_observe(const AuvConfig* cfg, const AuvRayTable* rays, const AuvPathBank* paths,
                const AuvScenarioPool* pool, AuvBatch* batch, AuvStepOut* out, int mode,
                void* stream) {
  if (int rc = check_observe_args(cfg, rays, paths, pool, batch, out, mode)) return rc;
  if (int rc = launch_vessel_nav(cfg, rays, paths, pool, batch, out, nullptr, stream)) return rc;
  return launch_lidar(cfg, rays, paths, pool, batch, out, mode, stream);
}

int auv_step(const AuvConfig* cfg, const AuvRayTable* rays, const AuvPathBank* paths,
             const AuvScenarioPool* pool, AuvBatch* batch, const float* actions, AuvStepOut* out,
             void* stream) {
  if (!actions) return set_err(AUV_EINVAL, "actions is NULL");
  if (int rc = check_observe_args(cfg, rays, paths, pool, batch, out, AUV_OBSERVE_STEP)) return rc;
  if (int rc = launch_vessel_nav(cfg, rays, paths, pool, batch, out, actions, stream, 0, -1, true)) return rc;
  return launch_lidar(cfg, rays, paths, pool, batch, out, AUV_OBSERVE_STEP, stream);
}

#define AUV_PIPE_MAX_STREAMS 16
#define AUV_PIPE_MAX_CHUNKS 64
struct AuvPipeline {
  int n_streams;
  cudaStream_t st[AUV_PIPE_MAX_STREAMS];
  cudaEvent_t fork, join[AUV_PIPE_MAX_STREAMS];
  cudaEvent_t chunk[AUV_PIPE_MAX_CHUNKS];
  cudaGraphExec_t gexec;
  unsigned long long gkey;
  int graph_state;
};

AuvPipeline* auv_pipeline_create(int n_streams) {
  if (n_streams <= 0 || n_streams > AUV_PIPE_MAX_STREAMS) {
    set_err(AUV_EINVAL, "n_streams out of range");
    return nullptr;
  }
  AuvPipeline* p = new AuvPipeline;
  p->n_streams = n_streams;
  p->gexec = nullptr;
  p->gkey = 0;
  p->graph_state = getenv("AUV_B200_NO_GRAPH") ? -1 : 0;
  bool ok = cudaEventCreateWithFlags(&p->fork, cudaEventDisableTiming) == cudaSuccess;
  int made = 0;
  for (; ok && made < n_streams; ++made) {
    ok = cudaStreamCreateWithFlags(&p->st[made], cudaStreamNonBlocking) == cudaSuccess &&
         cudaEventCreateWithFlags(&p->join[made], cudaEventDisableTiming) == cudaSuccess;
  }
  for (int c = 0; ok && c < AUV_PIPE_MAX_CHUNKS; ++c)
    ok = cudaEventCreateWithFlags(&p->chunk[c], cudaEventDisableTiming) == cudaSuccess;
  if (!ok) {
    cuda_check(cudaGetLastError(), "auv_pipeline_create");
    delete p;
    return nullptr;
  }
  return p;
}
void auv_pipeline_destroy(AuvPipeline* p) {
  if (!p) return;
  for (int i = 0; i < p->n_streams; ++i) {
    cudaStreamDestroy(p->st[i]);
    cudaEventDestroy(p->join[i]);
  }
  for (int c = 0; c < AUV_PIPE_MAX_CHUNKS; ++c) cudaEventDestroy(p->chunk[c]);
  cudaEventDestroy(p->fork);
  if (p->gexec) cudaGraphExecDestroy(p->gexec);
  delete p;
}

int auv_pipeline_graph_state(const AuvPipeline* p) { return p ? p->graph_state : AUV_EINVAL; }

static int chunk_size(int n, int n_chunks) {
  int c = (n + n_chunks - 1) / n_chunks;
  return (c + 255) / 256 * 256;
}

static int step_chunked(const AuvConfig* cfg, const AuvRayTable* rays, const AuvPathBank* paths,
                        const AuvScenarioPool* pool, AuvBatch* batch, const float* actions, AuvStepOut* out,
                        void* stream, AuvPipeline* p, int n_chunks) {
  if (!p) return set_err(AUV_EINVAL, "pipeline is NULL");
  if (n_chunks <= 0) return set_err(AUV_EINVAL, "n_chunks must be > 0");
  if (int rc = check_observe_args(cfg, rays, paths, pool, batch, out, AUV_OBSERVE_STEP)) return rc;
  cudaStream_t s = (cudaStream_t)stream;
  const int n = batch->n_envs;
  const int cs = chunk_size(n, n_chunks);
  if (int rc = cuda_check(cudaEventRecord(p->fork, s), "fork")) return rc;
  int used = 0;
  for (int c = 0, e0 = 0; e0 < n; ++c, e0 += cs) {
    const int cnt = n - e0 < cs ? n - e0 : cs;
    cudaStream_t cst = p->st[c % p->n_streams];
    void* vs = (void*)cst;
    if (c < p->n_streams) {
      if (int rc = cuda_check(cudaStreamWaitEvent(cst, p->fork, 0), "wait fork")) return rc;
      used = c + 1;
    }
    if (int rc = launch_vessel_nav(cfg, rays, paths, pool, batch, out, actions, vs, e0, cnt, true)) return rc;
    if (int rc = launch_lidar(cfg, rays, paths, pool, batch, out, AUV_OBSERVE_STEP, vs, e0, cnt)) return rc;
  }
  for (int i = 0; i < used; ++i) {
    if (int rc = cuda_check(cudaEventRecord(p->join[i], p->st[i]), "join record")) return rc;
    if (int rc = cuda_check(cudaStreamWaitEvent(s, p->join[i], 0), "join wait")) return rc;
  }
  return 0;
}

static int launch_obs_ship(const AuvConfig* cfg, const AuvStepOut* out, const AuvCompact* cb, float* reward_host,
                           uint8_t* done_host, int e0, int cnt, cudaStream_t s) {
  const int R = cfg->use_lidar ? cfg->n_sensors : 0;
  const int words = cb->words;
  const size_t smem = (size_t)AUV_SHIP_ENVS * words * 32 * 4 + (size_t)AUV_SHIP_ENVS * words * 4 + (AUV_SHIP_ENVS + 1) * 4 + 16;
  static std::atomic<size_t> configured[64];
  int dev = 0;
  if (cudaGetDevice(&dev) != cudaSuccess || dev < 0 || dev >= 64) dev = 0;
  if (smem > 48 * 1024 && smem > configured[dev].load()) {
    if (int rc = cuda_check(cudaFuncSetAttribute(auv::k_obs_ship, cudaFuncAttributeMaxDynamicSharedMemorySize, (int)smem),
                            "cudaFuncSetAttribute(k_obs_ship)"))
      return rc;
    configured[dev].store(smem);
  }
  const int blocks = (cnt + AUV_SHIP_ENVS - 1) / AUV_SHIP_ENVS;
  auv::k_obs_ship<<<blocks, AUV_SHIP_THREADS, smem, s>>>(out->obs, auv_obs_dim(cfg), R, words, e0, e0 + cnt, out->reward, out->done,
                                                        cb->head, cb->mask, cb->vals, cb->counter, cb->capacity, reward_host,
                                                        done_host);
  return cuda_check(cudaGetLastError(), "k_obs_ship");
}

static int launch_obs_delta(const AuvConfig* cfg, const AuvStepOut* out, const AuvDelta* d, float* reward_host,
                            uint8_t* done_host, int e0, int cnt, cudaStream_t s) {
  const long long od = auv_obs_dim(cfg);
  const long long f0 = od * e0, f1 = od * (e0 + cnt);
  const long long quads = (f1 - f0 + 3) / 4;
  static std::atomic<int> sms[64];
  int dev = 0;
  if (cudaGetDevice(&dev) != cudaSuccess || dev < 0 || dev >= 64) dev = 0;
  int n_sm = sms[dev].load();
  if (n_sm == 0) {
    if (cudaDeviceGetAttribute(&n_sm, cudaDevAttrMultiProcessorCount, dev) != cudaSuccess || n_sm <= 0) n_sm = 148;
    sms[dev].store(n_sm);
  }
  long long blocks = d->ctas > 0 ? d->ctas : 2 * n_sm;
  const long long need = (quads + AUV_DELTA_THREADS - 1) / AUV_DELTA_THREADS;
  if (blocks > need) blocks = need;
  if (blocks < 1) blocks = 1;
  auv::k_obs_delta<<<(int)blocks, AUV_DELTA_THREADS, 0, s>>>(out->obs, d->shadow, d->obs_host, f0, f1, d->gran / 4, out->reward,
                                                            out->done, reward_host, done_host, e0, e0 + cnt, d->shipped);
  return cuda_check(cudaGetLastError(), "k_obs_delta");
}

static int enqueue_host_step(const AuvConfig* cfg, const AuvRayTable* rays, const AuvPathBank* paths,
                             const AuvScenarioPool* pool, AuvBatch* batch, const float* actions_host,
                             float* actions_dev, AuvStepOut* out, float* obs_host, float* reward_host,
                             uint8_t* done_host, cudaStream_t s, cudaStream_t ds, AuvPipeline* p, int n_chunks,
                             const AuvCompact* cb = nullptr, const AuvDelta* dl = nullptr) {
  const int n = batch->n_envs;
  const int cs = chunk_size(n, n_chunks);
  const size_t od = (size_t)auv_obs_dim(cfg);
  if (int rc = cuda_check(cudaMemcpyAsync(actions_dev, actions_host, (size_t)n * 2 * sizeof(float), cudaMemcpyHostToDevice, s),
                          "H2D actions"))
    return rc;
  if (cb != nullptr)
    if (int rc = cuda_check(cudaMemsetAsync(cb->counter, 0, sizeof(int32_t), s), "compact counter")) return rc;
  for (int c = 0, e0 = 0; e0 < n; ++c, e0 += cs) {
    const int cnt = n - e0 < cs ? n - e0 : cs;
    if (int rc = launch_vessel_nav(cfg, rays, paths, pool, batch, out, actions_dev, (void*)s, e0, cnt, true)) return rc;
    if (int rc = launch_lidar(cfg, rays, paths, pool, batch, out, AUV_OBSERVE_STEP, (void*)s, e0, cnt)) return rc;
    if (ds != s) {
      if (int rc = cuda_check(cudaEventRecord(p->chunk[c], s), "range done")) return rc;
      if (int rc = cuda_check(cudaStreamWaitEvent(ds, p->chunk[c], 0), "copy stream wait")) return rc;
    }
    if (dl != nullptr) {
      if (int rc = launch_obs_delta(cfg, out, dl, reward_host, done_host, e0, cnt, ds)) return rc;
    } else if (cb != nullptr) {
      if (int rc = launch_obs_ship(cfg, out, cb, reward_host, done_host, e0, cnt, ds)) return rc;
    } else if (int rc = cuda_check(cudaMemcpyAsync(obs_host + od * e0, out->obs + od * e0, (size_t)cnt * od * sizeof(float),
                                                   cudaMemcpyDeviceToHost, ds), "D2H obs"))
      return rc;
  }
  if (cb == nullptr && dl == nullptr) {
    if (int rc = cuda_check(cudaMemcpyAsync(reward_host, out->reward, (size_t)n * sizeof(float), cudaMemcpyDeviceToHost, ds),
                            "D2H reward"))
      return rc;
    if (int rc = cuda_check(cudaMemcpyAsync(done_host, out->done, (size_t)n, cudaMemcpyDeviceToHost, ds), "D2H done"))
      return rc;
  }
  if (ds != s) {
    if (int rc = cuda_check(cudaEventRecord(p->join[0], ds), "join record")) return rc;
    return cuda_check(cudaStreamWaitEvent(s, p->join[0], 0), "join wait");
  }
  return 0;
}

static unsigned long long fnv1a(unsigned long long h, const void* data, size_t n) {
  const unsigned char* b = (const unsigned char*)data;
  for (size_t i = 0; i < n; ++i) h = (h ^ b[i]) * 1099511628211ull;
  return h;
}

static int step_host_chunked(const AuvConfig* cfg, const AuvRayTable* rays, const AuvPathBank* paths,
                             const AuvScenarioPool* pool, AuvBatch* batch, const float* actions_host,
                             float* actions_dev, AuvStepOut* out, float* obs_host, float* reward_host,
                             uint8_t* done_host, void* stream, AuvPipeline* p, int n_chunks,
                             const AuvCompact* cb = nullptr, const AuvDelta* dl = nullptr) {
  if (!p) return set_err(AUV_EINVAL, "pipeline is NULL");
  if (n_chunks <= 0 || n_chunks > AUV_PIPE_MAX_CHUNKS) return set_err(AUV_EINVAL, "n_chunks out of range");
  if (int rc = check_observe_args(cfg, rays, paths, pool, batch, out, AUV_OBSERVE_STEP)) return rc;
  cudaStream_t s = (cudaStream_t)stream, ds = p->st[0];
  if (p->graph_state >= 0 && p->n_streams >= 2) {
    unsigned long long key = 1469598103934665603ull;
    key = fnv1a(key, cfg, sizeof(*cfg));
    if (rays) key = fnv1a(key, rays, sizeof(*rays));
    key = fnv1a(key, paths, sizeof(*paths));
    key = fnv1a(key, pool, sizeof(*pool));
    key = fnv1a(key, batch, sizeof(*batch));
    key = fnv1a(key, out, sizeof(*out));
    if (out->tracks) key = fnv1a(key, out->tracks, sizeof(*out->tracks));
    const void* ptrs[6] = {actions_host, actions_dev, obs_host, reward_host, done_host, (const void*)(size_t)n_chunks};
    key = fnv1a(key, ptrs, sizeof(ptrs));
    if (cb) key = fnv1a(key, cb, sizeof(*cb));
    if (dl) key = fnv1a(key, dl, sizeof(*dl));
    if (p->graph_state == 0 || key != p->gkey) {
      if (p->gexec) {
        cudaGraphExecDestroy(p->gexec);
        p->gexec = nullptr;
      }
      p->graph_state = 0;
      if (int rc0 = lidar_configure(lidar_smem_bytes(cfg, pool))) return rc0;
      if (int rc0 = nav_configure(sizeof(auv::NavStage) * auv::NAV_SUBBLOCKS + AUV_NAV_EXTRA_SMEM)) return rc0;
      cudaStream_t cs = p->st[1];
      cudaGraph_t graph = nullptr;
      int rc = 0;
      if (cudaStreamBeginCapture(cs, cudaStreamCaptureModeRelaxed) == cudaSuccess) {
        rc = enqueue_host_step(cfg, rays, paths, pool, batch, actions_host, actions_dev, out, obs_host, reward_host,
                               done_host, cs, ds, p, n_chunks, cb, dl);
        const cudaError_t ce = cudaStreamEndCapture(cs, &graph);
        if (rc == 0 && ce == cudaSuccess && graph != nullptr &&
            cudaGraphInstantiate(&p->gexec, graph, 0) == cudaSuccess) {
          p->graph_state = 1;
          p->gkey = key;
        }
        if (graph) cudaGraphDestroy(graph);
      }
      if (p->graph_state != 1) {
        cudaGetLastError();
        p->graph_state = -1;
        if (rc) return rc;
      }
    }
    if (p->graph_state == 1) return cuda_check(cudaGraphLaunch(p->gexec, s), "cudaGraphLaunch");
  }
  return enqueue_host_step(cfg, rays, paths, pool, batch, actions_host, actions_dev, out, obs_host, reward_host, done_host,
                           s, ds, p, n_chunks, cb, dl);
}

int auv_step_chunked(const AuvConfig* cfg, const AuvRayTable* rays, const AuvPathBank* paths,
                     const AuvScenarioPool* pool, AuvBatch* batch, const float* actions, AuvStepOut* out,
                     void* stream, AuvPipeline* p, int n_chunks) {
  if (!actions) return set_err(AUV_EINVAL, "actions is NULL");
  return step_chunked(cfg, rays, paths, pool, batch, actions, out, stream, p, n_chunks);
}

int auv_step_host_submit(const AuvConfig* cfg, const AuvRayTable* rays, const AuvPathBank* paths,
                         const AuvScenarioPool* pool, AuvBatch* batch, const float* actions_host,
                         float* actions_dev, AuvStepOut* out, float* obs_host, float* reward_host,
                         uint8_t* done_host, void* stream, AuvPipeline* p, int n_chunks) {
  if (!cfg || !batch || !out || !actions_host || !actions_dev || !obs_host || !reward_host || !done_host)
    return set_err(AUV_EINVAL, "NULL argument");
  return step_host_chunked(cfg, rays, paths, pool, batch, actions_host, actions_dev, out, obs_host, reward_host,
                           done_host, stream, p, n_chunks);
}

int auv_step_host_compact_submit(const AuvConfig* cfg, const AuvRayTable* rays, const AuvPathBank* paths,
                                 const AuvScenarioPool* pool, AuvBatch* batch, const float* actions_host,
                                 float* actions_dev, AuvStepOut* out, const AuvCompact* cb, float* reward_host,
                                 uint8_t* done_host, void* stream, AuvPipeline* p, int n_chunks) {
  if (!cfg || !batch || !out || !actions_host || !actions_dev || !cb || !reward_host || !done_host)
    return set_err(AUV_EINVAL, "NULL argument");
  if (!cb->head || !cb->mask || !cb->vals || !cb->counter) return set_err(AUV_EINVAL, "compact buffers are NULL");
  if (cfg->sensor_use_velocity_observations) return set_err(AUV_ENOTSUP, "compact transfer with velocity observations");
  const int R = cfg->use_lidar ? cfg->n_sensors : 0;
  if (cb->words != (R + 31) / 32 || cb->words <= 0) return set_err(AUV_EINVAL, "compact.words must be ceil(n_sensors / 32) >= 1");
  if ((long long)cb->capacity < (long long)batch->n_envs * cb->words * 32)
    return set_err(AUV_EINVAL, "compact.capacity must be >= n_envs * words * 32");
  return step_host_chunked(cfg, rays, paths, pool, batch, actions_host, actions_dev, out, nullptr, reward_host, done_host,
                           stream, p, n_chunks, cb);
}

int auv_step_host_delta_submit(const AuvConfig* cfg, const AuvRayTable* rays, const AuvPathBank* paths,
                               const AuvScenarioPool* pool, AuvBatch* batch, const float* actions_host,
                               float* actions_dev, AuvStepOut* out, const AuvDelta* d, float* reward_host,
                               uint8_t* done_host, void* stream, AuvPipeline* p, int n_chunks) {
  if (!cfg || !batch || !out || !actions_host || !actions_dev || !d || !reward_host || !done_host)
    return set_err(AUV_EINVAL, "NULL argument");
  if (!d->obs_host || !d->shadow) return set_err(AUV_EINVAL, "delta buffers are NULL");
  if (d->gran != 8 && d->gran != 16 && d->gran != 32) return set_err(AUV_EINVAL, "delta.gran must be 8, 16 or 32");
  if (((size_t)d->obs_host | (size_t)d->shadow | (size_t)out->obs) & 15u)
    return set_err(AUV_EINVAL, "delta: obs_host, shadow and out->obs must be 16 B aligned");
  return step_host_chunked(cfg, rays, paths, pool, batch, actions_host, actions_dev, out, nullptr, reward_host, done_host,
                           stream, p, n_chunks, nullptr, d);
}

int auv_compact_expand(const AuvConfig* cfg, int n_envs, const AuvCompact* cb, uint32_t* prev_mask, float* obs_host,
                       int n_threads) {
  if (!cfg || !cb || !prev_mask || !obs_host || n_envs <= 0) return set_err(AUV_EINVAL, "bad auv_compact_expand arguments");
  const int od = auv_obs_dim(cfg), words = cb->words;
  const float* head = cb->head;
  const uint32_t* mask = cb->mask;
  const float* vals = cb->vals;
  if (n_threads < 1) n_threads = 1;
#pragma omp parallel for num_threads(n_threads) schedule(static)
  for (int e = 0; e < n_envs; ++e) {
    float* row = obs_host + (size_t)e * od;
    const float* h = head + (size_t)e * 8;
    for (int k = 0; k < 6; ++k) row[k] = h[k];
    int off;
    memcpy(&off, h + 7, sizeof(int));
    const float* v = vals + off;
    uint32_t* pm = prev_mask + (size_t)e * words;
    const uint32_t* nm = mask + (size_t)e * words;
    float* cl = row + 6;
    for (int w = 0; w < words; ++w) {
      uint32_t clear = pm[w] & ~nm[w];
      while (clear) {
        cl[w * 32 + __builtin_ctz(clear)] = 0.f;
        clear &= clear - 1;
      }
      uint32_t set = nm[w];
      while (set) {
        cl[w * 32 + __builtin_ctz(set)] = *v++;
        set &= set - 1;
      }
      pm[w] = nm[w];
    }
  }
  return 0;
}

int auv_step_host_chunked(const AuvConfig* cfg, const AuvRayTable* rays, const AuvPathBank* paths,
                          const AuvScenarioPool* pool, AuvBatch* batch, const float* actions_host,
                          float* actions_dev, AuvStepOut* out, float* obs_host, float* reward_host,
                          uint8_t* done_host, void* stream, AuvPipeline* p, int n_chunks) {
  if (int rc = auv_step_host_submit(cfg, rays, paths, pool, batch, actions_host, actions_dev, out, obs_host, reward_host,
                                    done_host, stream, p, n_chunks))
    return rc;
  return cuda_check(cudaStreamSynchronize((cudaStream_t)stream), "sync");
}

#define AUV_TIMER_EVENTS 4
struct AuvTimer {
  int capacity;
  cudaEvent_t* ev;
};

AuvTimer* auv_timer_create(int capacity) {
  if (capacity <= 0) return nullptr;
  AuvTimer* t = new AuvTimer;
  t->capacity = capacity;
  t->ev = new cudaEvent_t[(size_t)capacity * AUV_TIMER_EVENTS];
  for (int i = 0; i < capacity * AUV_TIMER_EVENTS; ++i)
    if (cudaEventCreate(&t->ev[i]) != cudaSuccess) {
      for (int k = 0; k < i; ++k) cudaEventDestroy(t->ev[k]);
      delete[] t->ev;
      delete t;
      return nullptr;
    }
  return t;
}
void auv_timer_destroy(AuvTimer* t) {
  if (!t) return;
  for (int i = 0; i < t->capacity * AUV_TIMER_EVENTS; ++i) cudaEventDestroy(t->ev[i]);
  delete[] t->ev;
  delete t;
}
int auv_step_timed(const AuvConfig* cfg, const AuvRayTable* rays, const AuvPathBank* paths,
                   const AuvScenarioPool* pool, AuvBatch* batch, const float* actions, AuvStepOut* out,
                   void* stream, AuvTimer* t, int slot) {
  if (!t || slot < 0 || slot >= t->capacity) return set_err(AUV_EINVAL, "bad timer/slot");
  if (!actions) return set_err(AUV_EINVAL, "actions is NULL");
  if (int rc = check_observe_args(cfg, rays, paths, pool, batch, out, AUV_OBSERVE_STEP)) return rc;
  cudaStream_t s = (cudaStream_t)stream;
  cudaEvent_t* e = t->ev + AUV_TIMER_EVENTS * slot;
  cudaEventRecord(e[0], s);
  if (!AUV_NAV_SPLIT) cudaEventRecord(e[1], s);
  if (int rc = launch_vessel_nav(cfg, rays, paths, pool, batch, out, actions, stream, 0, -1, true,
                                 AUV_NAV_SPLIT ? e[1] : nullptr))
    return rc;
  cudaEventRecord(e[2], s);
  if (int rc = launch_lidar(cfg, rays, paths, pool, batch, out, AUV_OBSERVE_STEP, stream)) return rc;
  return cuda_check(cudaEventRecord(e[3], s), "cudaEventRecord");
}
int auv_timer_read(AuvTimer* t, int slot, float* ms) {
  if (!t || !ms || slot < 0 || slot >= t->capacity) return set_err(AUV_EINVAL, "bad timer/slot");
  cudaEvent_t* e = t->ev + AUV_TIMER_EVENTS * slot;
  for (int k = 0; k < AUV_TIMER_EVENTS - 1; ++k)
    if (int rc = cuda_check(cudaEventElapsedTime(&ms[k], e[k], e[k + 1]), "cudaEventElapsedTime")) return rc;
  return 0;
}

int auv_step_host(const AuvConfig* cfg, const AuvRayTable* rays, const AuvPathBank* paths,
                  const AuvScenarioPool* pool, AuvBatch* batch, const float* actions_host,
                  float* actions_dev, AuvStepOut* out, float* obs_host, float* reward_host,
                  uint8_t* done_host, void* stream) {
  if (!cfg || !batch || !out || !actions_host || !actions_dev || !obs_host || !reward_host || !done_host)
    return set_err(AUV_EINVAL, "NULL argument");
  if (int rc = check_tracks(out, batch)) return rc;
  cudaStream_t s = (cudaStream_t)stream;
  const size_t n = (size_t)batch->n_envs;
  if (int rc = cuda_check(cudaMemcpyAsync(actions_dev, actions_host, n * 2 * sizeof(float),
                                          cudaMemcpyHostToDevice, s), "H2D actions"))
    return rc;
  if (int rc = auv_step(cfg, rays, paths, pool, batch, actions_dev, out, stream)) return rc;
  const size_t od = (size_t)auv_obs_dim(cfg);
  if (int rc = cuda_check(cudaMemcpyAsync(obs_host, out->obs, n * od * sizeof(float),
                                          cudaMemcpyDeviceToHost, s), "D2H obs"))
    return rc;
  if (int rc = cuda_check(cudaMemcpyAsync(reward_host, out->reward, n * sizeof(float),
                                          cudaMemcpyDeviceToHost, s), "D2H reward"))
    return rc;
  if (int rc = cuda_check(cudaMemcpyAsync(done_host, out->done, n, cudaMemcpyDeviceToHost, s), "D2H done"))
    return rc;
  return cuda_check(cudaStreamSynchronize(s), "sync");
}

static int check_gen_world(const AuvGenParams* gp, const AuvScenarioPool* pool) {
  if (pool->n_world < 0) return set_err(AUV_EINVAL, "n_world < 0");
  if (pool->n_world == 0) return 0;
  if (!pool->world_circle || !pool->world_voff || !pool->world_verts) return set_err(AUV_EINVAL, "world arrays are NULL");
  if (pool->world_cell_off &&
      (!pool->world_cell_items || pool->world_grid_nx <= 0 || pool->world_grid_ny <= 0 || !(pool->world_grid_cell > 0.0)))
    return set_err(AUV_EINVAL, "world grid: NULL items or empty grid");
  if (!(gp->land_clearance >= 0.0)) return set_err(AUV_EINVAL, "land_clearance must be >= 0");
  return 0;
}

static int launch_generate(const AuvGenParams* gp, const AuvPathBank* paths, const AuvScenarioPool* pool,
                           const int32_t* ids, int n_ids, const int32_t* n_ids_dev, int32_t* status, cudaStream_t s) {
  const int threads = 128;
  auv::k_generate_scenario_heads<<<(unsigned)((n_ids + threads - 1) / threads), threads, 0, s>>>(*gp, *paths, *pool, ids, n_ids,
                                                                                               n_ids_dev, status);
  if (int rc = cuda_check(cudaGetLastError(), "k_generate_scenario_heads")) return rc;
  const long long total = (long long)n_ids * (pool->k_moving + pool->k_static);
  if (total == 0) return 0;
  cudaLaunchConfig_t lc = {};
  lc.gridDim = dim3((unsigned)((total + threads - 1) / threads));
  lc.blockDim = dim3(threads);
  lc.stream = s;
  cudaLaunchAttribute at[1];
  at[0].id = cudaLaunchAttributeProgrammaticStreamSerialization;
  at[0].val.programmaticStreamSerializationAllowed = 1;
  lc.attrs = at;
  lc.numAttrs = 1;
  return cuda_check(cudaLaunchKernelEx(&lc, auv::k_generate_moving_obstacles, *gp, *paths, *pool, ids, n_ids, n_ids_dev, status),
                    "k_generate_moving_obstacles");
}

int auv_generate_moving_obstacles(const AuvGenParams* gp, const AuvPathBank* paths, const AuvScenarioPool* pool,
                                  const int32_t* ids, int n_ids, int32_t* status, void* stream) {
  if (!gp || !paths || !pool) return set_err(AUV_EINVAL, "NULL argument");
  if (n_ids <= 0 || (!ids && n_ids > pool->n_scenarios)) return set_err(AUV_EINVAL, "n_ids out of range");
  if (paths->n_paths <= 0) return set_err(AUV_EINVAL, "empty path bank");
  if (pool->k_moving < 0 || pool->k_static < 0) return set_err(AUV_EINVAL, "negative slot count");
  if (!pool->path_id || !pool->vessel_init) return set_err(AUV_EINVAL, "pool.path_id / vessel_init is NULL");
  if (pool->k_moving > 0 && (!pool->mov_start || !pool->mov_width || !pool->mov_track || !pool->vel_table ||
                             !pool->mov_pos0 || !pool->mov_disp0 || !pool->mov_counter0))
    return set_err(AUV_EINVAL, "moving-obstacle arrays are NULL");
  if (pool->k_static > 0 && (!pool->st_pos || !pool->st_radius)) return set_err(AUV_EINVAL, "static-obstacle arrays are NULL");
  if (int rc = check_gen_world(gp, pool)) return rc;
  return launch_generate(gp, paths, pool, ids, n_ids, nullptr, status, (cudaStream_t)stream);
}

int auv_linear_wrap(double dt, double counter0, int vel_len, int32_t* first_wrap, int32_t* wrap_period) {
  if (!(dt > 0.0) || vel_len < 2 || !first_wrap || !wrap_period) return set_err(AUV_EINVAL, "bad auv_linear_wrap arguments");
  const int limit = 1 << 30;
  double c = counter0;
  int n = 0;
  for (;;) {
    ++n;
    c += dt;
    if ((int)floor(c) >= vel_len - 1) break;
    if (n >= limit) return set_err(AUV_EINVAL, "track never wraps");
  }
  *first_wrap = n;
  c = 0.0;
  n = 0;
  for (;;) {
    ++n;
    c += dt;
    if ((int)floor(c) >= vel_len - 1) break;
    if (n >= limit) return set_err(AUV_EINVAL, "track never wraps");
  }
  *wrap_period = n;
  return 0;
}

int auv_pool_pack(const AuvConfig* cfg, const AuvScenarioPool* pool, const int32_t* ids, int n_ids, void* stream) {
  if (int rc = check_cfg(cfg)) return rc;
  if (!pool) return set_err(AUV_EINVAL, "pool is NULL");
  if (n_ids <= 0 || (!ids && n_ids > pool->n_scenarios)) return set_err(AUV_EINVAL, "n_ids out of range");
  if (pool->k_static > 0 && (!pool->st_rec || !pool->st_pos || !pool->st_radius))
    return set_err(AUV_EINVAL, "static-obstacle arrays are NULL");
  if (pool->k_moving > 0 && pool->linear_tracks &&
      (!pool->mov_lin || !pool->mov_pos0 || !pool->mov_start || !pool->mov_width || !pool->mov_track || !pool->vel_table))
    return set_err(AUV_EINVAL, "moving-obstacle arrays are NULL");
  const long long total = (long long)n_ids * (pool->k_moving + pool->k_static);
  if (total == 0) return 0;
  const int threads = 128;
  auv::k_pool_pack<<<(unsigned)((total + threads - 1) / threads), threads, 0, (cudaStream_t)stream>>>(*cfg, *pool, ids, n_ids);
  return cuda_check(cudaGetLastError(), "k_pool_pack");
}

int auv_obstacle_state(const AuvConfig* cfg, const AuvScenarioPool* pool, const AuvBatch* batch, double* pos,
                       double* disp, double* counter, void* stream) {
  if (int rc = check_cfg(cfg)) return rc;
  if (!pool || !batch) return set_err(AUV_EINVAL, "pool/batch is NULL");
  if (batch->n_envs <= 0) return set_err(AUV_EINVAL, "n_envs must be > 0");
  if (!batch->obst_steps) return set_err(AUV_EINVAL, "batch.obst_steps is NULL");
  if (int rc = check_pool_tracks(pool, batch)) return rc;
  const long long total = (long long)batch->n_envs * pool->k_moving;
  if (total == 0) return 0;
  const int threads = 128;
  auv::k_obstacle_state<<<(unsigned)((total + threads - 1) / threads), threads, 0, (cudaStream_t)stream>>>(*cfg, *pool, *batch, pos,
                                                                                                         disp, counter);
  return cuda_check(cudaGetLastError(), "k_obstacle_state");
}

static int reset_cache_fill(const AuvConfig* cfg, const AuvRayTable* rays, const AuvPathBank* paths,
                            const AuvScenarioPool* pool, AuvBatch* worker, AuvStepOut* wout, const int32_t* ids, int first,
                            int n, const int32_t* n_dev, void* stream) {
  if (n <= 0 || n > worker->n_envs) return set_err(AUV_EINVAL, "n must be in 1..worker.n_envs");
  if (!pool->reset_obs || !pool->reset_max_progress || (cfg->use_lidar && !pool->reset_mask))
    return set_err(AUV_EINVAL, "pool.reset_* is NULL");
  if (int rc = check_observe_args(cfg, rays, paths, pool, worker, wout, AUV_OBSERVE_RESET)) return rc;
  cudaStream_t s = (cudaStream_t)stream;
  const int wn = worker->n_envs, threads = 128;
  auv::k_worker_fill<<<(wn + threads - 1) / threads, threads, 0, s>>>(*worker, ids, first, n, n_dev);
  if (int rc = cuda_check(cudaGetLastError(), "k_worker_fill")) return rc;
  if (int rc = auv_reset(cfg, pool, worker, nullptr, stream)) return rc;
  if (int rc = auv_observe(cfg, rays, paths, pool, worker, wout, AUV_OBSERVE_RESET, stream)) return rc;
  auv::k_cache_scatter<<<(n * 32 + threads - 1) / threads, threads, 0, s>>>(*pool, *worker, wout->obs, auv_obs_dim(cfg),
                                                                          cfg->use_lidar, n, n_dev);
  return cuda_check(cudaGetLastError(), "k_cache_scatter");
}

int auv_reset_cache_fill(const AuvConfig* cfg, const AuvRayTable* rays, const AuvPathBank* paths,
                         const AuvScenarioPool* pool, AuvBatch* worker, AuvStepOut* worker_out, const int32_t* ids,
                         int first, int n, void* stream) {
  if (!cfg || !paths || !pool || !worker || !worker_out) return set_err(AUV_EINVAL, "NULL argument");
  if (!ids && (first < 0 || first + n > pool->n_scenarios)) return set_err(AUV_EINVAL, "scenario range out of bounds");
  return reset_cache_fill(cfg, rays, paths, pool, worker, worker_out, ids, first, n, nullptr, stream);
}

int auv_refresh_finished(const AuvConfig* cfg, const AuvRayTable* rays, const AuvPathBank* paths,
                         const AuvScenarioPool* pool, const AuvBatch* live, AuvBatch* worker, AuvStepOut* worker_out,
                         const AuvRefreshScratch* rs, const AuvGenParams* gp, void* stream) {
  if (!cfg || !paths || !pool || !live || !worker || !worker_out || !rs || !gp) return set_err(AUV_EINVAL, "NULL argument");
  if (!rs->seen_episode || !rs->ids || !rs->count || rs->capacity <= 0 || rs->capacity > worker->n_envs)
    return set_err(AUV_EINVAL, "refresh scratch: NULL array or capacity not in 1..worker.n_envs");
  if (pool->n_scenarios != 2 * (live->reset_stride > 0 ? live->reset_stride : live->n_envs))
    return set_err(AUV_EINVAL, "refresh needs a pool of exactly 2 * reset_stride (default n_envs) scenarios");
  if (int rc = check_gen_world(gp, pool)) return rc;
  cudaStream_t s = (cudaStream_t)stream;
  const int threads = 128;
  if (int rc = cuda_check(cudaMemsetAsync(rs->count, 0, sizeof(int32_t), s), "memset")) return rc;
  auv::k_refresh_collect<<<(live->n_envs + threads - 1) / threads, threads, 0, s>>>(*live, pool->n_scenarios, rs->seen_episode,
                                                                                    rs->ids, rs->count, rs->capacity);
  if (int rc = cuda_check(cudaGetLastError(), "k_refresh_collect")) return rc;
  if (int rc = launch_generate(gp, paths, pool, rs->ids, rs->capacity, rs->count, live->status, s)) return rc;
  return reset_cache_fill(cfg, rays, paths, pool, worker, worker_out, rs->ids, 0, rs->capacity, rs->count, stream);
}

int auv_pathbank_build(const double* waypoints, const int32_t* n_wp, const int32_t* path_ids, int n,
                       const AuvPathBuild* out, int32_t* status, void* stream) {
  if (!waypoints || !n_wp || !out || n <= 0) return set_err(AUV_EINVAL, "bad auv_pathbank_build arguments");
  if (!out->hdr || !out->poly_xy || !out->poly_cum || !out->poly_f32 || !out->blk_chord || !out->blk_dev || !out->sb_chord ||
      !out->sb_dev || !out->pp)
    return set_err(AUV_EINVAL, "AuvPathBuild holds a NULL array");
  if (out->n_knots != auv::PB_NK) return set_err(AUV_EINVAL, "n_knots must be 1000");
  if ((out->sub_chord == nullptr) != (out->sub_dev == nullptr))
    return set_err(AUV_EINVAL, "AuvPathBuild: sub_chord and sub_dev are both set or both NULL");
  if (out->vcap <= 0 || out->vcap % (2 * AUV_PATH_BLOCK * AUV_PATH_SUPER) != 0)
    return set_err(AUV_EINVAL, "vcap must be a positive multiple of 2 * AUV_PATH_BLOCK * AUV_PATH_SUPER");
  const size_t smem = auv::pathbuild_smem_bytes();
  static std::atomic<int> configured[64];
  int dev = 0;
  if (cudaGetDevice(&dev) != cudaSuccess || dev < 0 || dev >= 64) dev = 0;
  if (!configured[dev].load()) {
    if (int rc = cuda_check(cudaFuncSetAttribute(auv::k_path_build, cudaFuncAttributeMaxDynamicSharedMemorySize, (int)smem),
                            "cudaFuncSetAttribute(k_path_build)"))
      return rc;
    configured[dev].store(1);
  }
  auv::PathBuildOut o;
  o.hdr = out->hdr;
  o.poly_xy = out->poly_xy;
  o.poly_cum = out->poly_cum;
  o.poly_f32 = out->poly_f32;
  o.blk_chord = out->blk_chord;
  o.blk_dev = out->blk_dev;
  o.sb_chord = out->sb_chord;
  o.sb_dev = out->sb_dev;
  o.pp = out->pp;
  o.vcap = out->vcap;
  o.sub_chord = out->sub_chord;
  o.sub_dev = out->sub_dev;
  auv::k_path_build<<<n, auv::PB_THREADS, smem, (cudaStream_t)stream>>>(waypoints, n_wp, path_ids, n, o, status);
  return cuda_check(cudaGetLastError(), "k_path_build");
}

int auv_random_curve_waypoints(uint64_t seed, uint32_t epoch, double length, const int32_t* path_ids, int n,
                               double* waypoints, int32_t* n_wp, void* stream) {
  if (!waypoints || !n_wp || n <= 0 || !(length > 0.0)) return set_err(AUV_EINVAL, "bad auv_random_curve_waypoints arguments");
  auv::k_random_curve_waypoints<<<(n + 127) / 128, 128, 0, (cudaStream_t)stream>>>(seed, epoch, length, path_ids, n, waypoints, n_wp);
  return cuda_check(cudaGetLastError(), "k_random_curve_waypoints");
}

int auv_fma_probe(float* sink, int blocks, int threads, int iters, void* stream, double* flops_out) {
  if (!sink || blocks <= 0 || threads <= 0 || threads > 256 || iters <= 0)
    return set_err(AUV_EINVAL, "bad probe arguments");
  auv::k_fma_probe<<<blocks, threads, 0, (cudaStream_t)stream>>>(sink, iters);
  if (flops_out) *flops_out = 2.0 * 8.0 * (double)iters * (double)blocks * (double)threads;
  return cuda_check(cudaGetLastError(), "k_fma_probe");
}

}
```

gym_auv_b200/vec_env.py:

```python
from __future__ import annotations

import ctypes as C
import os
import time
from typing import Dict, Optional

import numpy as np
import torch

from . import _lib
from .config import Config
from .scenarios import LAND_CLEARANCE, ScenarioSet, linear_track_positions, table_track_positions
from .spaces import Box, Dict as DictSpace


def sector_partition(isensor: int, n_sensors: int, n_sectors: int, c: float = 0.1) -> int:
    a, b = n_sensors, n_sectors

    def sigma(x):
        return b / (1 + np.exp((-x + a / 2) / (c * a)))

    return int(np.floor(sigma(isensor) - sigma(0)))


# ... 140 lines not shown
        host_transfer: Optional[str] = None,
        delta_gran: int = 16,
        record_tracks: int = 0,
        track_capacity: int = 2048,
        count_ray_tests: Optional[bool] = None,
        _shared: Optional[dict] = None,
    ):
        self.device = torch.device(device)
        if self.device.type != "cuda" or not torch.cuda.is_available():
            raise RuntimeError("AUVVecEnv needs a CUDA device: the step path has no CPU fallback")
        self.lib = _lib.load()
        self.config = config.copy() if config is not None else Config()
        self.scenarios = scenarios
        if _shared is None:
            scenarios.validate()
        self.num_envs = N = int(num_envs)
        self.test_mode = test_mode
        self.debug = debug
        self.env_offset = int(env_offset)
        self.cfg = make_auv_config(self.config, scenarios.rewarder, test_mode, auto_reset, cull_mode, velocity_mode)
        self._velocity_mode = velocity_mode
        self.obs_dim = self.lib.auv_obs_dim(C.byref(self.cfg))
        self.n_sensors = R = int(self.config.vessel.n_sensors)
        dev = self.device
        t = lambda a, dt: torch.as_tensor(np.ascontiguousarray(a), dtype=dt).to(dev)

        self.sensor_angles, cos_sin, weight, wsum, sector = ray_table(R, int(self.config.vessel.n_sectors))
        k64 = np.arange(64) * (2 * np.pi / 64)
        unit64 = np.stack([np.cos(k64), np.sin(k64)], axis=1)
        unit64[np.abs(unit64) < 1e-15] = 0.0
        if _shared is not None:
            self._ray = _shared["ray"]
        else:
            self._ray = dict(cos_sin=t(cos_sin, torch.float64), weight=t(weight, torch.float32),
                             sector=t(sector, torch.uint8), unit64=t(unit64, torch.float64))
        self.sector_index = sector
        self.rays = _lib.AuvRayTable(
            self._ray["cos_sin"].data_ptr(), self._ray["weight"].data_ptr(), self._ray["sector"].data_ptr(), self._ray["unit64"].data_ptr(), wsum
        )

        bank = scenarios.bank
        self._bank = _shared["bank"] if _shared is not None else bank.device_arrays(dev)
        b = self._bank
        self.paths = _lib.AuvPathBank(
            bank.n_paths, getattr(bank, "n_knots", None) or bank.knots.shape[1], b["hdr"].data_ptr(), b["poly_xy"].data_ptr(), b["poly_cum"].data_ptr(),
            b["poly_f32"].data_ptr(), b["blk_chord"].data_ptr(), b["blk_dev"].data_ptr(), b["sb_chord"].data_ptr(), b["sb_dev"].data_ptr(),
            b["pp"].data_ptr(), b["sub_chord"].data_ptr(), b["sub_dev"].data_ptr(),
        )

        M, Km, Ks = scenarios.n_scenarios, scenarios.k_moving, scenarios.k_static
        self.k_moving, self.k_static = Km, Ks
        mw = max(1, (Km + Ks + scenarios.world.n + 31) // 32)
        if mw > 32:
            raise ValueError("at most 1024 obstacle slots (moving + static + world polygons) per env")
        if _shared is None:
            pos0, disp0, counter0 = scenarios.initial_obstacle_state(float(self.config.simulation.t_step_size))
            vel = scenarios.vel_table if len(scenarios.vel_table) else np.zeros((1, 2))
        self._pool = _shared["pool"] if _shared is not None else dict(
            path_id=t(scenarios.path_id, torch.int32),
            vessel_init=t(scenarios.vessel_init, torch.float64),
            mov_start=t(scenarios.mov_start, torch.float64),
            mov_width=t(scenarios.mov_width, torch.float64),
            mov_track=t(scenarios.mov_track, torch.int32),
            mov_pos0=t(pos0, torch.float64),
            mov_disp0=t(disp0, torch.float64),
            mov_counter0=t(counter0, torch.float64),
            vel_table=t(vel, torch.float64),
            st_pos=t(scenarios.st_pos, torch.float64),
            st_radius=t(scenarios.st_radius, torch.float64),
            st_rec=torch.zeros((M, max(Ks, 1), 4), dtype=torch.float64, device=dev),
        )
        if _shared is not None:
            self.linear = _shared["linear"]
        else:
            lin = scenarios.linear_track_info(float(self.config.simulation.t_step_size)) if linear_tracks else None
            self.linear = None
            if lin is not None and Km > 0:
                first, period = C.c_int32(0), C.c_int32(0)
                _lib.check(self.lib.auv_linear_wrap(float(self.config.simulation.t_step_size), lin["counter0"],
                                                    lin["vel_len"], C.byref(first), C.byref(period)), "auv_linear_wrap")
                self.linear = dict(first_wrap=int(first.value), wrap_period=int(period.value), **lin)
                self._pool["mov_lin"] = torch.zeros((M, Km, 8), dtype=torch.float64, device=dev)
        world = scenarios.world
        self.n_world = Pw = world.n
        if Pw and _shared is None:
            self._pool.update(
                world_circle=t(world.circle, torch.float64), world_voff=t(world.voff, torch.int32),
                world_verts=t(world.verts, torch.float64),
            )
            if world_grid and Pw > 32:
                g = world.grid(float(self.config.vessel.sensor_range) + 10.0)
                self._pool.update(world_cell_off=t(g["off"], torch.int32), world_cell_items=t(g["items"], torch.int32))
                self._pool["world_grid"] = g
        if _shared is None:
            self._pool.update(
                reset_obs=torch.zeros((M, self.obs_dim), dtype=torch.float32, device=dev),
                reset_max_progress=torch.zeros(M, dtype=torch.float64, device=dev),
                reset_mask=torch.zeros((M, mw), dtype=torch.int32, device=dev),
            )
        p = self._pool
        wptr = lambda k: p[k].data_ptr() if k in p else None
        lin = self.linear
        self.pool = _lib.AuvScenarioPool(
            M, Km, Ks, Pw, p["path_id"].data_ptr(), p["vessel_init"].data_ptr(), p["mov_start"].data_ptr(),
            p["mov_width"].data_ptr(), p["mov_track"].data_ptr(), p["mov_pos0"].data_ptr(), p["mov_disp0"].data_ptr(),
            p["mov_counter0"].data_ptr(), p["vel_table"].data_ptr(), p["st_pos"].data_ptr(), p["st_radius"].data_ptr(),
            p["st_rec"].data_ptr(), wptr("mov_lin"), int(lin is not None), lin["first_wrap"] if lin else 0,
            lin["wrap_period"] if lin else 0, 0,
            wptr("world_circle"), wptr("world_voff"), wptr("world_verts"),
            wptr("world_cell_off"), wptr("world_cell_items"),
            p["world_grid"]["x0"] if "world_grid" in p else 0.0, p["world_grid"]["y0"] if "world_grid" in p else 0.0,
            p["world_grid"]["cell"] if "world_grid" in p else 0.0,
            p["world_grid"]["nx"] if "world_grid" in p else 0, p["world_grid"]["ny"] if "world_grid" in p else 0,
            p["reset_obs"].data_ptr(), p["reset_max_progress"].data_ptr(), p["reset_mask"].data_ptr(),
        )
        if _shared is None:
            with torch.cuda.device(self.device):
                _lib.check(self.lib.auv_pool_pack(C.byref(self.cfg), C.byref(self.pool), None, M, self._stream()),
                           "auv_pool_pack")

        z = lambda shape, dt: torch.zeros(shape, dtype=dt, device=dev)
        self._st = dict(
            scn_id=((torch.arange(N, device=dev, dtype=torch.int64) + self.env_offset) % M).to(torch.int32),
            episode=z(N, torch.int32),
            state=z((6, N), torch.float64),
            step_counter=z(N, torch.int32),
            t_step=z(N, torch.int32),
            cum_reward=z(N, torch.float64),
            max_progress=z(N, torch.float64),
            cte_sum=z(N, torch.float64),
            nearby_mask=z((N, mw), torch.int32),
            nav=z((N, _lib.NAV_W), torch.float64),
            obst_steps=z(N, torch.int32),
            prev_seg=torch.full((N,), -1, dtype=torch.int32, device=dev),
            env_pid=z(N, torch.int32),
        )
        if self.linear is None:
            self._st.update(
                mov_pos=z((N, max(Km, 1), 2), torch.float64),
                mov_disp=z((N, max(Km, 1), 2), torch.float64),
                mov_counter=z((N, max(Km, 1)), torch.float64),
            )
        slots = Km + Ks + Pw
        self.rec_cap = int(max_nearby) if max_nearby is not None else (slots if slots <= 64 else 64)
        self.rec_cap = max(1, min(self.rec_cap, max(slots, 1)))
        self._scratch = dict(
            rec=torch.zeros((N, self.rec_cap, _lib.REC_BYTES), dtype=torch.uint8, device=dev),
            rec_cnt=z(N, torch.int32), status=z(1, torch.int32),
        )
        s = self._st
        sptr = lambda k: s[k].data_ptr() if k in s else None
        self.reset_stride = int(reset_stride)
        self.batch = _lib.AuvBatch(
            N, mw, self.env_offset, self.reset_stride, s["scn_id"].data_ptr(), s["episode"].data_ptr(), s["state"].data_ptr(),
            s["step_counter"].data_ptr(), s["t_step"].data_ptr(), s["cum_reward"].data_ptr(),
            s["max_progress"].data_ptr(), s["cte_sum"].data_ptr(), s["nearby_mask"].data_ptr(),
            sptr("mov_pos"), sptr("mov_disp"), sptr("mov_counter"), s["nav"].data_ptr(),
            self._scratch["rec"].data_ptr(), self._scratch["rec_cnt"].data_ptr(),
            self._scratch["status"].data_ptr(), self.rec_cap, 0,
            s["obst_steps"].data_ptr(), s["prev_seg"].data_ptr(), s["env_pid"].data_ptr(),
        )

        K = Km + Ks + Pw
        self._out = dict(
            obs=z((N, self.obs_dim), torch.float32),
            reward=z(N, torch.float32),
            done=z(N, torch.uint8),
            collision=z(N, torch.uint8),
            reached_goal=z(N, torch.uint8),
            goal_distance=z(N, torch.float32),
            progress=z(N, torch.float32),
            terminal_obs=z((N, self.obs_dim), torch.float32),
            stats=z(_lib.N_STATS, torch.float64),
            seg_tests=z(1, torch.int64),
            episode_out=z((N, 8), torch.float32),
        )
        if sector_outputs and self.config.vessel.use_lidar:
            ns = int(self.config.vessel.n_sectors)
            self._out["sector_min_dist"] = z((N, ns), torch.float32)
            self._out["sector_feasible_dist"] = z((N, ns), torch.float32)
        if debug:
            self._out["lidar_dist"] = z((N, max(R, 1)), torch.float32)
            self._out["windows"] = z((N, max(K, 1), 2), torch.int32)
        count_ray_tests = bool(debug) if count_ray_tests is None else bool(count_ray_tests)
        if count_ray_tests and int(record_tracks) > 0:
            raise ValueError("record_tracks cannot be combined with the ray-test counter of debug: "
                             "pass count_ray_tests=False")
        if int(record_tracks) > 0:
            del self._out["seg_tests"]
        o = self._out
        ptr = lambda k: o[k].data_ptr() if k in o else None
        self.record_tracks = Kt = max(0, min(int(record_tracks), N))
        self.track_capacity = T = int(track_capacity)
        self.tracked_envs = np.zeros(0, dtype=np.int64)
        self._tracks, self.tracks = None, None
        if Kt:
            if T < 1:
                raise ValueError("track_capacity must be >= 1")
            stride = N // Kt
            self.tracked_envs = np.arange(Kt, dtype=np.int64) * stride
            W = _lib.track_snap_width(Km, Ks)
            self._tracks = dict(points=z((Kt, 2, T, 4), torch.float32), head=z((Kt, 2, _lib.TRACK_HEAD_W), torch.int32),
                                snap=z((Kt, 2, W), torch.float64), stride=stride)
            tk = self._tracks
            self.tracks = _lib.AuvTracks(Kt, stride, T, 0, tk["points"].data_ptr(), tk["head"].data_ptr(),
                                         tk["snap"].data_ptr())
        self.out = _lib.AuvStepOut(
            ptr("obs"), ptr("reward"), ptr("done"), ptr("collision"), ptr("reached_goal"), ptr("goal_distance"),
            ptr("progress"), ptr("lidar_dist"), ptr("windows"), ptr("terminal_obs"), ptr("sector_min_dist"),
            ptr("sector_feasible_dist"), ptr("stats"),
            ptr("seg_tests") if count_ray_tests else None, ptr("episode_out"),
            C.addressof(self.tracks) if Kt else None,
        )
        self.actions_dev = z((N, 2), torch.float32)
        self._pinned = None
        can_compact = bool(self.config.vessel.use_lidar) and not bool(self.config.vessel.sensor_use_velocity_observations)
        if host_transfer not in (None, "dense", "compact", "delta"):
            raise ValueError("host_transfer must be 'dense', 'compact' or 'delta'")
        if host_transfer == "compact" and not can_compact:
            raise ValueError("host_transfer='compact' needs LiDAR observations without velocity channels")
        if host_transfer is None:
            host_transfer = "delta" if compact_host is None else ("compact" if compact_host and can_compact else "dense")
        self.host_transfer = host_transfer
        self.compact_host = self.host_transfer == "compact"
        self.delta_gran = int(delta_gran)
        self._delta_seen = (0, 0)
        import os as _os

        self.host_threads = int(host_threads) if host_threads else max(1, min(16, len(_os.sched_getaffinity(0))))
        self.expand_seconds = 0.0
        self.wait_seconds = 0.0
        self.chunks = max(1, int(chunks))
        self.host_chunks = max(1, min(64, int(host_chunks))) if host_chunks else self.chunks
        self._pipe = None
        if self.chunks > 1 or self.host_chunks > 1:
            ns = int(chunk_streams) if chunk_streams else max(2, min(self.chunks, 4))
            with torch.cuda.device(self.device):
                self._pipe = self.lib.auv_pipeline_create(ns)
            if not self._pipe:
                raise _lib.AuvLibraryError("auv_pipeline_create failed: " + self.lib.auv_last_error().decode())
            self.chunk_streams = ns
        self.total_steps = 0

        self.action_space = Box(low=np.array([-1, -0.15]), high=np.array([1, 0.15]), dtype=np.float32)
        self.observation_space = Box(low=-np.ones(self.obs_dim), high=np.ones(self.obs_dim), dtype=np.float32)
        self.dict_observation = bool(self.config.vessel.use_dict_observation) and bool(self.config.vessel.use_lidar)
        if self.dict_observation:
            self.observation_space = DictSpace({
                "proprioceptive": Box(-1.0, 1.0, shape=(6,), dtype=np.float32),
                "lidar": Box(-1.0, 1.0, shape=((self.obs_dim - 6) // R, R), dtype=np.float32),
            })
        self._max_nearby = max_nearby
        self._cull_mode = cull_mode
        if auto_reset and _shared is None:
            self._build_reset_cache()

    def _worker(self, cap: int) -> "AUVVecEnv":
        if not hasattr(self, "_workers"):
            self._workers = {}
        w = self._workers.get(cap)
        if w is None:
            w = self._workers[cap] = AUVVecEnv(
                self.scenarios, cap, self.config, device=self.device, test_mode=self.test_mode, auto_reset=False,
                cull_mode=self._cull_mode, max_nearby=self._max_nearby, velocity_mode=self._velocity_mode,
                _shared=self._shared_tables())
        return w

    def _build_reset_cache(self, ids: Optional[torch.Tensor] = None, chunk: int = 65536):
        M = self.scenarios.n_scenarios
        total = M if ids is None else int(ids.numel())
        if total == 0:
            return
        cap = 1024 if total <= 1024 else (8192 if total <= 8192 else min(chunk, 65536))
        w = self._worker(cap)
        idp = ids.to(self.device, torch.int32).contiguous() if ids is not None else None
        cfg, rays, paths, pool, _ = self._refs()
        with torch.cuda.device(self.device):
            for start in range(0, total, cap):
                n = min(cap, total - start)
                p = C.c_void_p(idp.data_ptr() + 4 * start) if idp is not None else None
                _lib.check(self.lib.auv_reset_cache_fill(cfg, rays, paths, pool, C.byref(w.batch), C.byref(w.out), p,
                                                         start if idp is None else 0, n, self._stream()),
                           "auv_reset_cache_fill")
        if cap > 8192:
            torch.cuda.synchronize(self.device)
            self._workers.pop(cap, None)

    def gen_params(self, seed: int, epoch: int) -> "_lib.AuvGenParams":
        v = self.config.vessel
        return _lib.AuvGenParams(
            seed=int(seed) & 0xFFFFFFFFFFFFFFFF, epoch=int(epoch) & 0xFFFFFFFF,
            post_generate_update=int(bool(self.scenarios.post_generate_update)),
            t_step_size=float(self.config.simulation.t_step_size), vessel_width=float(v.vessel_width),
            init_pos_jitter=50.0, mov_disp_std=500.0, mov_width_mean=10.0, mov_speed_lo=1.0, mov_speed_hi=3.0,
            st_disp_std=250.0, st_radius_mean=30.0,
            path_group=int(self.scenarios.path_group), path_period=int(self.scenarios.path_period or self.scenarios.n_scenarios),
            land_clearance=LAND_CLEARANCE,
        )

    def regenerate_scenarios(self, ids: Optional[torch.Tensor] = None, seed: int = 0, epoch: int = 1):
        M, Km = self.scenarios.n_scenarios, self.k_moving
        if Km and self._pool["vel_table"].shape[0] < M * Km:
            raise ValueError("pool.vel_table must hold n_scenarios * k_moving entries (constant-velocity tracks)")
        gp = self.gen_params(seed, epoch)
        self._pool["host_stale"] = True
        idp, n = None, M
        if ids is not None:
            ids = ids.to(self.device, torch.int32).contiguous()
            idp, n = C.c_void_p(ids.data_ptr()), int(ids.numel())
            if n == 0:
                return 0
        with torch.cuda.device(self.device):
            _lib.check(self.lib.auv_generate_moving_obstacles(
                C.byref(gp), C.byref(self.paths), C.byref(self.pool), idp, n,
                C.c_void_p(self._scratch["status"].data_ptr()), self._stream()), "auv_generate_moving_obstacles")
        self._build_reset_cache(ids)
        return n

    def regenerate_paths(self, ids: Optional[torch.Tensor] = None, seed: int = 0, epoch: int = 1, length: float = 800.0):
        from .pathbank import DevicePathBank

        bank = self.scenarios.bank
        if not isinstance(bank, DevicePathBank):
            raise ValueError("regenerate_paths needs a device-built path bank (scenarios built with device_paths=True)")
        n = bank.n_paths
        idp = None
        if ids is not None:
            ids = ids.to(self.device, torch.int32).contiguous()
            idp, n = C.c_void_p(ids.data_ptr()), int(ids.numel())
            if n == 0:
                return 0
        wp = torch.zeros((n, 2, 8), dtype=torch.float64, device=self.device)
        nwp = torch.zeros(n, dtype=torch.int32, device=self.device)
        bs = bank.build_struct(self._bank)
        with torch.cuda.device(self.device):
            _lib.check(self.lib.auv_random_curve_waypoints(int(seed) & 0xFFFFFFFFFFFFFFFF, int(epoch) & 0xFFFFFFFF, float(length),
                                                           idp, n, C.c_void_p(wp.data_ptr()), C.c_void_p(nwp.data_ptr()),
                                                           self._stream()), "auv_random_curve_waypoints")
            _lib.check(self.lib.auv_pathbank_build(C.c_void_p(wp.data_ptr()), C.c_void_p(nwp.data_ptr()), idp, n, C.byref(bs),
                                                   C.c_void_p(self._scratch["status"].data_ptr()), self._stream()),
                       "auv_pathbank_build")
        hw, hn = wp.cpu().numpy(), nwp.cpu().numpy()
        slots = range(bank.n_paths) if ids is None else ids.cpu().numpy().tolist()
        for k, pth in enumerate(slots):
            bank.waypoints[int(pth)] = hw[k, :, : int(hn[k])].copy()
            self.scenarios.waypoints[int(pth)] = bank.waypoints[int(pth)]
        bank._tables = None
        self.check_status()
        return n

    def refresh_finished(self, seed: int = 0) -> int:
        N, M = self.reset_stride or self.num_envs, self.scenarios.n_scenarios
        if M != 2 * N:
            raise ValueError("refresh_finished needs a pool of exactly 2 * reset_stride (default num_envs) scenarios")
        ep = self._st["episode"]
        if getattr(self, "_seen_episode", None) is None:
            self._seen_episode = torch.zeros_like(ep)
            self._gen_epoch = 1
        changed = torch.nonzero(ep != self._seen_episode).flatten()
        self._seen_episode.copy_(ep)
        if changed.numel() == 0:
            return 0
        free = (self._st["scn_id"][changed].to(torch.int64) + N) % M
        self._gen_epoch += 1
        return self.regenerate_scenarios(free, seed=seed, epoch=self._gen_epoch)

    def refresh_finished_device(self, seed: int = 0, capacity: int = 4096):
        N, M = self.num_envs, self.scenarios.n_scenarios
        if M != 2 * (self.reset_stride or N):
            raise ValueError("refresh_finished_device needs a pool of exactly 2 * reset_stride (default num_envs) scenarios")
        capacity = int(min(capacity, 65536))
        rs = getattr(self, "_refresh", None)
        if rs is None or rs["cap"] != capacity:
            dev = self.device
            rs = self._refresh = dict(
                cap=capacity, seen=self._st["episode"].clone(), ids=torch.zeros(capacity, dtype=torch.int32, device=dev),
                count=torch.zeros(1, dtype=torch.int32, device=dev), epoch=getattr(self, "_gen_epoch", 1))
            rs["struct"] = _lib.AuvRefreshScratch(rs["seen"].data_ptr(), rs["ids"].data_ptr(), rs["count"].data_ptr(),
                                                  capacity, 0)
        w = self._worker(1024 if capacity <= 1024 else (8192 if capacity <= 8192 else 65536))
        rs["epoch"] += 1
        self._gen_epoch = rs["epoch"]
        gp = self.gen_params(seed, rs["epoch"])
        self._pool["host_stale"] = True
        cfg, rays, paths, pool, batch = self._refs()
        with torch.cuda.device(self.device):
            _lib.check(self.lib.auv_refresh_finished(cfg, rays, paths, pool, batch, C.byref(w.batch), C.byref(w.out),
                                                     C.byref(rs["struct"]), C.byref(gp), self._stream()),
                       "auv_refresh_finished")

    def pull_scenarios(self) -> ScenarioSet:
        import dataclasses

        p = self._pool
        h = lambda k: p[k].cpu().numpy().copy()
        return dataclasses.replace(
            self.scenarios, path_id=h("path_id"), vessel_init=h("vessel_init"), mov_start=h("mov_start"),
            mov_width=h("mov_width"), mov_track=h("mov_track"), vel_table=h("vel_table"), st_pos=h("st_pos"),
            st_radius=h("st_radius"), _bank=self.scenarios.bank, _world=self.scenarios._world,
        )

    def _shared_tables(self):
        return dict(ray=self._ray, bank=self._bank, pool=self._pool, linear=self.linear)

    def obstacle_state(self):
        if self.linear is None:
            return self._st["mov_pos"], self._st["mov_disp"], self._st["mov_counter"]
        N, Km = self.num_envs, max(self.k_moving, 1)
        pos = torch.zeros((N, Km, 2), dtype=torch.float64, device=self.device)
        disp = torch.zeros_like(pos)
        cnt = torch.zeros((N, Km), dtype=torch.float64, device=self.device)
        if self.k_moving:
            with torch.cuda.device(self.device):
                _lib.check(self.lib.auv_obstacle_state(
                    C.byref(self.cfg), C.byref(self.pool), C.byref(self.batch), C.c_void_p(pos.data_ptr()),
                    C.c_void_p(disp.data_ptr()), C.c_void_p(cnt.data_ptr()), self._stream()), "auv_obstacle_state")
        return pos, disp, cnt

    def _stream(self):
        return C.c_void_p(torch.cuda.current_stream(self.device).cuda_stream)

    def _refs(self):
        return C.byref(self.cfg), C.byref(self.rays), C.byref(self.paths), C.byref(self.pool), C.byref(self.batch)

    def check_status(self):
        st = int(self._scratch["status"].item())
        if st & _lib.STATUS_GEN_GAVE_UP:
            raise RuntimeError("scenario generator: an obstacle slot was still rejected after 100000 draws")
        if st & _lib.STATUS_GEN_LAND_BLOCKED:
            raise RuntimeError("scenario generator: a scenario's start area is covered by land "
                               "(no vessel start clear of land after 4096 draws)")
        if st & _lib.STATUS_BOUNDS:
            raise RuntimeError("AUV_DEBUG_BOUNDS build: an index check inside a step kernel failed "
                               f"(source lines OR-ed together: {st >> 8})")
        if st & _lib.STATUS_PATH_TOO_LONG:
            raise RuntimeError("a generated path's polyline does not fit its slot: raise DevicePathBank(vcap=...)")
        if st & _lib.STATUS_POLY_TOO_LARGE:
            raise RuntimeError(f"a world polygon has more than {_lib.MAX_POLY_VERTS} vertices: split it")
        if st & _lib.STATUS_REC_OVERFLOW:
            raise RuntimeError(
                f"more than max_nearby={self.rec_cap} obstacles were within sensor range of one env: "
                "construct AUVVecEnv with a larger max_nearby"
            )

    def observation_dict(self, obs=None):
        o = self._out["obs"] if obs is None else obs
        R = self.n_sensors
        return {"proprioceptive": o[:, :6], "lidar": o[:, 6:].reshape(o.shape[0], -1, R)}

    def _fmt(self, obs):
        return self.observation_dict(obs) if self.dict_observation else obs

    def reset(self, check: bool = True) -> torch.Tensor:
        cfg, rays, paths, pool, batch = self._refs()
        with torch.cuda.device(self.device):
            _lib.check(self.lib.auv_reset(cfg, pool, batch, None, self._stream()), "auv_reset")
            _lib.check(
                self.lib.auv_observe(cfg, rays, paths, pool, batch, C.byref(self.out), _lib.OBSERVE_RESET, self._stream()),
                "auv_observe",
            )
        if check:
            self.check_status()
        return self._fmt(self._out["obs"])

    def reset_envs(self, mask: torch.Tensor, scenario_ids: Optional[torch.Tensor] = None) -> torch.Tensor:
        mask = mask.to(device=self.device, dtype=torch.uint8).contiguous()
        if scenario_ids is not None:
            sel = mask.bool()
            self._st["scn_id"][sel] = scenario_ids.to(self.device, torch.int32)[sel]
        cfg, rays, paths, pool, batch = self._refs()
        with torch.cuda.device(self.device):
            _lib.check(self.lib.auv_reset(cfg, pool, batch, C.c_void_p(mask.data_ptr()), self._stream()), "auv_reset")
            _lib.check(
                self.lib.auv_observe(cfg, rays, paths, pool, batch, C.byref(self.out), _lib.OBSERVE_RESET, self._stream()),
                "auv_observe",
            )
        return self._out["obs"]

    def step(self, actions: torch.Tensor):
        if actions.shape != (self.num_envs, 2):
            raise ValueError(f"actions must have shape ({self.num_envs}, 2), got {tuple(actions.shape)}")
        a = actions.to(device=self.device, dtype=torch.float32).contiguous()
        cfg, rays, paths, pool, batch = self._refs()
        with torch.cuda.device(self.device):
            if self._pipe and self.chunks > 1:
                _lib.check(
                    self.lib.auv_step_chunked(cfg, rays, paths, pool, batch, C.c_void_p(a.data_ptr()), C.byref(self.out),
                                              self._stream(), self._pipe, self.chunks),
                    "auv_step_chunked",
                )
            else:
                _lib.check(
                    self.lib.auv_step(cfg, rays, paths, pool, batch, C.c_void_p(a.data_ptr()), C.byref(self.out), self._stream()),
                    "auv_step",
                )
        self.total_steps += 1
        return self._fmt(self._out["obs"]), self._out["reward"], self._out["done"], self.info()

    def step_host(self, actions: np.ndarray):
        if self.host_transfer != "dense":
            self.step_async(actions)
            return self.step_wait()
        pin = self.step_host_buffers()
        pin["act"].numpy()[...] = actions
        cfg, rays, paths, pool, batch = self._refs()
        with torch.cuda.device(self.device):
            hargs = (cfg, rays, paths, pool, batch, C.c_void_p(pin["act"].data_ptr()),
                     C.c_void_p(self.actions_dev.data_ptr()), C.byref(self.out), C.c_void_p(pin["obs"].data_ptr()),
                     C.c_void_p(pin["reward"].data_ptr()), C.c_void_p(pin["done"].data_ptr()), self._stream())
            if self._pipe and self.host_chunks > 1:
                _lib.check(self.lib.auv_step_host_chunked(*hargs, self._pipe, self.host_chunks), "auv_step_host_chunked")
            else:
                _lib.check(self.lib.auv_step_host(*hargs), "auv_step_host")
        self.total_steps += 1
        return pin["obs"].numpy(), pin["reward"].numpy(), pin["done"].numpy()

    def step_async(self, actions: np.ndarray):
        if getattr(self, "_async_pending", False):
            raise RuntimeError("step_async() called twice without step_wait()")
        if self._pinned is None:
            self.step_host_buffers()
        if self._pipe is None:
            with torch.cuda.device(self.device):
                self._pipe = self.lib.auv_pipeline_create(2)
            if not self._pipe:
                raise _lib.AuvLibraryError("auv_pipeline_create failed: " + self.lib.auv_last_error().decode())
            self.chunk_streams = 2
        if getattr(self, "_async_stream", None) is None:
            self._async_stream = torch.cuda.Stream(device=self.device)
            self._async_done = torch.cuda.Event()
        pin = self._pinned
        if getattr(self, "_async_call", None) is None:
            cfg, rays, paths, pool, batch = self._refs()
            head = (cfg, rays, paths, pool, batch, C.c_void_p(pin["act"].data_ptr()), C.c_void_p(self.actions_dev.data_ptr()),
                    C.byref(self.out))
            tail = (C.c_void_p(pin["reward"].data_ptr()), C.c_void_p(pin["done"].data_ptr()),
                    C.c_void_p(self._async_stream.cuda_stream), self._pipe, max(1, self.host_chunks))
            if self.host_transfer == "delta":
                self._async_call = (self.lib.auv_step_host_delta_submit, head + (C.byref(pin["delta"]),) + tail,
                                    "auv_step_host_delta_submit")
            elif self.compact_host:
                self._async_call = (self.lib.auv_step_host_compact_submit, head + (C.byref(pin["compact"]),) + tail,
                                    "auv_step_host_compact_submit")
            else:
                self._async_call = (self.lib.auv_step_host_submit, head + (C.c_void_p(pin["obs"].data_ptr()),) + tail,
                                    "auv_step_host_submit")
            self._act_np = pin["act"].numpy()
        self._act_np[...] = actions
        cur = torch.cuda.current_stream(self.device)
        if cur != self._async_stream:
            self._async_stream.wait_stream(cur)
        fn, fargs, name = self._async_call
        with torch.cuda.device(self.device):
            rc = fn(*fargs)
        if rc:
            _lib.check(rc, name)
        self._async_done.record(self._async_stream)
        self._async_pending = True
        self.total_steps += 1

    def step_wait(self):
        if not getattr(self, "_async_pending", False):
            raise RuntimeError("step_wait() without a pending step_async()")
        t0 = time.perf_counter()
        self._async_done.synchronize()
        self.wait_seconds += time.perf_counter() - t0
        torch.cuda.current_stream(self.device).wait_event(self._async_done)
        self._async_pending = False
        pin = self._pinned
        if self.compact_host:
            t0 = time.perf_counter()
            _lib.check(self.lib.auv_compact_expand(
                C.byref(self.cfg), self.num_envs, C.byref(pin["compact"]), C.c_void_p(pin["prev_mask"].ctypes.data),
                C.c_void_p(pin["obs_dense"].ctypes.data), self.host_threads), "auv_compact_expand")
            self.expand_seconds += time.perf_counter() - t0
            return pin["obs_dense"], pin["reward"].numpy(), pin["done"].numpy()
        return pin["obs"].numpy(), pin["reward"].numpy(), pin["done"].numpy()

    def groups(self, n_groups: int = 2, **kw):
        n = self.num_envs // int(n_groups)
        if n <= 0:
            raise ValueError("more groups than envs")
        shared = self._shared_tables()
        kw.setdefault("host_chunks", max(1, self.host_chunks // int(n_groups)))
        kw.setdefault("host_transfer", self.host_transfer)
        kw.setdefault("delta_gran", self.delta_gran)
        kw.setdefault("record_tracks", self.record_tracks)
        kw.setdefault("track_capacity", self.track_capacity)
        return [AUVVecEnv(self.scenarios, n, self.config, device=self.device, test_mode=self.test_mode,
                          auto_reset=bool(self.cfg.auto_reset), cull_mode=self._cull_mode, env_offset=g * n,
                          max_nearby=self._max_nearby, velocity_mode=self._velocity_mode,
                          reset_stride=self.reset_stride or self.num_envs, host_threads=self.host_threads,
                          _shared=shared, **kw)
                for g in range(int(n_groups))]

    def ring(self, n_groups: int = 4, **kw) -> "EnvGroupRing":
        return EnvGroupRing(self.groups(n_groups, **kw))

    def step_host_buffers(self):
        N = self.num_envs
        if self._pinned is None:
            self._pinned = dict(
                act=torch.zeros((N, 2), dtype=torch.float32).pin_memory(),
                reward=torch.zeros(N, dtype=torch.float32).pin_memory(),
                done=torch.zeros(N, dtype=torch.uint8).pin_memory(),
            )
            if self.compact_host:
                W = (self.n_sensors + 31) // 32
                p = self._pinned
                p["head"] = torch.zeros((N, 8), dtype=torch.float32).pin_memory()
                p["mask"] = torch.zeros((N, W), dtype=torch.int32).pin_memory()
                p["vals"] = torch.zeros(N * W * 32, dtype=torch.float32).pin_memory()
                p["counter"] = torch.zeros(1, dtype=torch.int32, device=self.device)
                p["prev_mask"] = np.zeros((N, W), dtype=np.uint32)
                p["obs_dense"] = np.zeros((N, self.obs_dim), dtype=np.float32)
                p["compact"] = _lib.AuvCompact(p["head"].data_ptr(), p["mask"].data_ptr(), p["vals"].data_ptr(),
                                               p["counter"].data_ptr(), W, N * W * 32)
            else:
                self._pinned["obs"] = torch.zeros((N, self.obs_dim), dtype=torch.float32).pin_memory()
                if self.host_transfer == "delta":
                    p = self._pinned
                    p["shadow"] = torch.zeros((N, self.obs_dim), dtype=torch.float32, device=self.device)
                    p["shipped"] = torch.zeros(1, dtype=torch.int64, device=self.device)
                    p["delta"] = _lib.AuvDelta(p["obs"].data_ptr(), p["shadow"].data_ptr(), p["shipped"].data_ptr(),
                                               self.delta_gran, int(os.environ.get("AUV_B200_DELTA_CTAS", "0")))
        return self._pinned

    @property
    def h2d_bytes_per_step(self) -> int:
        return self.num_envs * 2 * 4

    @property
    def d2h_bytes_per_step(self) -> int:
        if self.compact_host and self._pinned is not None:
            p = self._pinned
            nz = int(p["head"].numpy().view(np.int32)[:, 6].sum())
            return self.num_envs * (32 + 4 * p["mask"].shape[1] + 4 + 1) + 4 * nz
        if self.host_transfer == "delta" and self._pinned is not None:
            chunks, steps = int(self._pinned["shipped"].item()), self.total_steps
            c0, s0 = self._delta_seen
            self._delta_seen = (chunks, steps)
            return self.num_envs * (4 + 1) + int((chunks - c0) * self.delta_gran * 4 / max(1, steps - s0))
        return self.num_envs * (self.obs_dim * 4 + 4 + 1)

    def info(self) -> Dict[str, torch.Tensor]:
        o = self._out
        return dict(
            collision=o["collision"],
            reached_goal=o["reached_goal"],
            goal_distance=o["goal_distance"],
            progress=o["progress"],
            terminal_observation=o["terminal_obs"],
        )

    def obstacle_update(self):
        cfg, _, _, pool, batch = self._refs()
        with torch.cuda.device(self.device):
            _lib.check(self.lib.auv_obstacle_update(cfg, pool, batch, self._stream()), "auv_obstacle_update")

    def vessel_step(self, actions: torch.Tensor):
        a = actions.to(device=self.device, dtype=torch.float32).contiguous()
        cfg, _, _, _, batch = self._refs()
        with torch.cuda.device(self.device):
            _lib.check(self.lib.auv_vessel_step(cfg, batch, C.c_void_p(a.data_ptr()), self._stream()), "auv_vessel_step")

    def navigate(self):
        cfg, rays, paths, pool, batch = self._refs()
        with torch.cuda.device(self.device):
            _lib.check(self.lib.auv_navigate(cfg, rays, paths, pool, batch, self._stream()), "auv_navigate")
        return self._st["nav"]

    def observe(self, mode=_lib.OBSERVE_STEP):
        cfg, rays, paths, pool, batch = self._refs()
        with torch.cuda.device(self.device):
            _lib.check(
                self.lib.auv_observe(cfg, rays, paths, pool, batch, C.byref(self.out), mode, self._stream()),
                "auv_observe",
            )
        return self._out["obs"]

    def _track_slot(self, i: int) -> Optional[int]:
        if self._tracks is None:
            return None
        i, stride = int(i), self._tracks["stride"]
        if i < 0 or i % stride or i // stride >= self.record_tracks:
            return None
        return i // stride

    def _track_sync(self):
        torch.cuda.current_stream(self.device).synchronize()
        if getattr(self, "_async_stream", None) is not None:
            self._async_stream.synchronize()

    def _path_table(self, pid: int):
        from .pathbank import DevicePathBank, build_path

        bank = self.scenarios.bank
        if isinstance(bank, DevicePathBank) and bank._tables is None:
            return build_path(bank.waypoints[pid])
        return bank.tables[pid]

    def _assemble(self, head_row, points_row, snap_row):
        if self.linear is None and self.k_moving and self._pool.get("host_stale"):
            raise RuntimeError("obstacle histories of a table-driven pool are rebuilt from the host scenarios, which "
                               "GPU scenario generation has made stale: record tracks with linear_tracks='auto' "
                               "on generated pools")
        return assemble_episode(head_row, points_row, snap_row, self.track_capacity, self.k_moving, self.k_static,
                                float(self.config.simulation.t_step_size), self.linear, self.scenarios,
                                self._path_table, self.scenarios.world_polygons)

    def last_episode(self, i: int) -> Optional[dict]:
        slot = self._track_slot(i)
        if slot is None:
            return None
        self._track_sync()
        tk = self._tracks
        head = tk["head"][slot].cpu().numpy()
        p = pick_finished_row(head)
        if p is None:
            return None
        return self._assemble(head[p], tk["points"][slot, p].cpu().numpy(), tk["snap"][slot, p].cpu().numpy())

    def current_episode(self, i: int) -> Optional[dict]:
        slot = self._track_slot(i)
        if slot is None:
            return None
        self._track_sync()
        tk, i = self._tracks, int(i)
        ep, scn = int(self._st["episode"][i].item()), int(self._st["scn_id"][i].item())
        p = ep & 1
        head = tk["head"][slot, p].cpu().numpy()
        if int(head[0]) != ep or int(head[1]) == 0:
            head = np.array([ep, 0, 0, 0, 0, scn, 0, 0], dtype=np.int32)
        pool, km, ks = self._pool, self.k_moving, self.k_static
        parts = [pool["path_id"][scn:scn + 1].to(torch.float64), pool["vessel_init"][scn]]
        if km:
            parts.append(pool["mov_lin"][scn].reshape(-1) if "mov_lin" in pool
                         else torch.zeros(8 * km, dtype=torch.float64, device=self.device))
        if ks:
            parts.append(pool["st_rec"][scn, :ks].reshape(-1))
        snap = torch.cat(parts).cpu().numpy()
        return self._assemble(head, tk["points"][slot, p].cpu().numpy(), snap)

    @property
    def state(self) -> torch.Tensor:
        return self._st["state"]

    def get_attr(self, name: str):
        table = dict(
            t_step=self._st["t_step"], cumulative_reward=self._st["cum_reward"], episode=self._st["episode"],
            step_counter=self._st["step_counter"], max_progress=self._st["max_progress"], scn_id=self._st["scn_id"],
            nearby_mask=self._st["nearby_mask"], nav=self._st["nav"], obst_steps=self._st["obst_steps"],
        )
        if name in table:
            return table[name]
        if name in ("mov_pos", "mov_disp", "mov_counter"):
            return dict(zip(("mov_pos", "mov_disp", "mov_counter"), self.obstacle_state()))[name]
        if name in self._out:
            return self._out[name]
        raise AttributeError(name)

    def episode_stats(self, reduce: bool = True) -> Dict[str, float]:
        from .sharding import reduce_stats, summarize_stats

        self.check_status()
        st = self._out["stats"].clone()
        st[9] = float(self.total_steps) * self.num_envs
        if reduce:
            st = reduce_stats(st)
        return summarize_stats(st.cpu().numpy(), float(self.config.simulation.t_step_size))

    def close(self):
        if self._pipe:
            torch.cuda.synchronize(self.device)
            self.lib.auv_pipeline_destroy(self._pipe)
            self._pipe = None
            self._async_call = None

    def __del__(self):
        try:
            self.close()
        except Exception:
            pass


class EnvGroupRing:

    def __init__(self, groups):
        self.groups = list(groups)
        self.pending = []
        self.spins = 0

    def __len__(self):
        return len(self.groups)

    @property
    def envs_per_group(self) -> int:
        return self.groups[0].num_envs

    def reset(self):
        return [g.reset() for g in self.groups]

    def send(self, g: int, actions: np.ndarray):
        self.groups[g].step_async(actions)
        self.pending.append(g)

    def recv(self):
        if not self.pending:
            raise RuntimeError("recv() with no step in flight")
        t0 = time.perf_counter()
        while True:
            for k, g in enumerate(self.pending):
                if self.groups[g]._async_done.query():
                    del self.pending[k]
                    self.groups[g].wait_seconds += time.perf_counter() - t0
                    obs, rew, done = self.groups[g].step_wait()
                    return g, obs, rew, done
            self.spins += 1

    def drain(self):
        out = []
        while self.pending:
            out.append(self.recv())
        return out

    def close(self):
        for g in self.groups:
            g.close()
        self.groups = []
```

include/auv_b200.h:

```cpp
#ifndef AUV_B200_H
#define AUV_B200_H

#include <stdint.h>

#ifdef __cplusplus
extern "C" {
#endif

#define AUV_ABI_VERSION 22

#define AUV_EINVAL (-1)
#define AUV_ENOTSUP (-2)

#define AUV_REWARDER_COLAV 0
#define AUV_REWARDER_PATHFOLLOW 1

#define AUV_CULL_REFERENCE 0
#define AUV_CULL_EXACT 1

#define AUV_VELOCITY_ZERO 0
#define AUV_VELOCITY_NEAREST 1

#define AUV_MAX_RAYS 1024
#define AUV_MAX_OBSTACLES 1024
#ifndef AUV_PATH_BLOCK
#define AUV_PATH_BLOCK 32
#endif
#ifndef AUV_PATH_SUPER
#define AUV_PATH_SUPER 16
#endif
#define AUV_PATH_SUB 8
#define AUV_NAV_W 24
#define AUV_REC_BYTES 80
#define AUV_MAX_POLY_VERTS 192
#define AUV_STATUS_REC_OVERFLOW 1
#define AUV_STATUS_GEN_GAVE_UP 2
#define AUV_STATUS_PATH_TOO_LONG 8
#define AUV_STATUS_BOUNDS 16
#define AUV_STATUS_POLY_TOO_LARGE 4
#define AUV_STATUS_GEN_LAND_BLOCKED 32
#ifndef AUV_PATH_STAGE_BLOCKS
#define AUV_PATH_STAGE_BLOCKS 512
#endif
#define AUV_PP_W 12

typedef struct AuvConfig {
  double t_step_size;
  double thrust_max_auv;
  double moment_max_auv;
  double vessel_width;
  double look_ahead_distance;
  double sensor_range;
  double min_goal_distance;
  double min_path_progress;
  double min_cumulative_reward;
  double feasibility_width_multiplier;
  int32_t max_timesteps;
  int32_t sensor_interval_load_obstacles;
  int32_t n_sensors;
  int32_t n_sectors;
  int32_t use_lidar;
  int32_t sensor_log_transform;
  int32_t sensor_use_velocity_observations;
  int32_t rewarder;
  int32_t test_mode;
  int32_t cull_mode;
  int32_t auto_reset;
  int32_t velocity_mode;
} AuvConfig;

typedef struct AuvRayTable {
  const double* cos_sin;
  const float* weight;
  const uint8_t* sector;
  const double* unit64;
  double weight_sum;
} AuvRayTable;

typedef struct AuvPathHdr {
  int32_t v0;
  int32_t nseg;
  int32_t b0;
  int32_t s0;
  double ox, oy;
  double length;
  double end_x, end_y;
  double extent;
} AuvPathHdr;

typedef struct AuvPathBank {
  int32_t n_paths;
  int32_t n_knots;
  const AuvPathHdr* hdr;
  const double* poly_xy;
  const double* poly_cum;
  const float* poly_f32;
  const float* blk_chord;
  const float* blk_dev;
  const float* sb_chord;
  const float* sb_dev;
  const double* pp;
  const float* sub_chord;
  const float* sub_dev;
} AuvPathBank;

typedef struct AuvScenarioPool {
  int32_t n_scenarios;
  int32_t k_moving;
  int32_t k_static;
  int32_t n_world;
  const int32_t* path_id;
  const double* vessel_init;
  const double* mov_start;
  const double* mov_width;
  const int32_t* mov_track;
  const double* mov_pos0;
  const double* mov_disp0;
  const double* mov_counter0;
  const double* vel_table;
  const double* st_pos;
  const double* st_radius;
  const double* st_rec;
  const double* mov_lin;
  int32_t linear_tracks;
  int32_t lin_first_wrap;
  int32_t lin_wrap_period;
  int32_t reserved0;
  const double* world_circle;
  const int32_t* world_voff;
  const double* world_verts;
  const int32_t* world_cell_off;
  const int32_t* world_cell_items;
  double world_grid_x0, world_grid_y0, world_grid_cell;
  int32_t world_grid_nx, world_grid_ny;
  const float* reset_obs;
  const double* reset_max_progress;
  const uint32_t* reset_mask;
} AuvScenarioPool;

typedef struct AuvBatch {
  int32_t n_envs;
  int32_t mask_words;
  int32_t env_offset;
  int32_t reset_stride;
  int32_t* scn_id;
  int32_t* episode;
  double* state;
  int32_t* step_counter;
  int32_t* t_step;
  double* cum_reward;
  double* max_progress;
  double* cte_sum;
  uint32_t* nearby_mask;
  double* mov_pos;
  double* mov_disp;
  double* mov_counter;
  double* nav;
  void* rec;
  int32_t* rec_cnt;
  int32_t* status;
  int32_t rec_cap;
  int32_t reserved1;
  int32_t* obst_steps;
  int32_t* prev_seg;
  int32_t* env_pid;
} AuvBatch;

typedef struct AuvTracks {
  int32_t count;
  int32_t stride;
  int32_t capacity;
  int32_t reserved0;
  float* points;
  int32_t* head;
  double* snap;
} AuvTracks;

typedef struct AuvStepOut {
  float* obs;
  float* reward;
  uint8_t* done;
  uint8_t* collision;
  uint8_t* reached_goal;
  float* goal_distance;
  float* progress;
  float* lidar_dist;
  int32_t* windows;
  float* terminal_obs;
  float* sector_min_dist;
  float* sector_feasible_dist;
  double* stats;
  unsigned long long* seg_tests;
  float* episode_out;
  const AuvTracks* tracks;
} AuvStepOut;

#define AUV_STAT_EPISODES 0
#define AUV_STAT_REWARD 1
#define AUV_STAT_REWARD_SQ 2
#define AUV_STAT_PROGRESS 3
#define AUV_STAT_COLLISIONS 4
#define AUV_STAT_REACHED_GOAL 5
#define AUV_STAT_TIMESTEPS 6
#define AUV_STAT_CROSS_TRACK 7
#define AUV_STAT_PATHLENGTH 8
#define AUV_STAT_STEPS 9
#define AUV_N_STATS 16

#define AUV_OBSERVE_STEP 0
#define AUV_OBSERVE_RESET 1

int auv_abi_version(void);
int auv_sizeof(int which);
const char* auv_last_error(void);
int auv_obs_dim(const AuvConfig* cfg);

int auv_obstacle_update(const AuvConfig* cfg, const AuvScenarioPool* pool, AuvBatch* batch,
                        void* stream);
int auv_vessel_step(const AuvConfig* cfg, AuvBatch* batch, const float* actions ,
                    void* stream);
int auv_navigate(const AuvConfig* cfg, const AuvRayTable* rays, const AuvPathBank* paths,
                 const AuvScenarioPool* pool, AuvBatch* batch, void* stream);
int auv_observe(const AuvConfig* cfg, const AuvRayTable* rays, const AuvPathBank* paths,
                const AuvScenarioPool* pool, AuvBatch* batch, AuvStepOut* out, int mode,
                void* stream);
int auv_reset(const AuvConfig* cfg, const AuvScenarioPool* pool, AuvBatch* batch,
              const uint8_t* reset_mask, void* stream);
int auv_step(const AuvConfig* cfg, const AuvRayTable* rays, const AuvPathBank* paths,
             const AuvScenarioPool* pool, AuvBatch* batch, const float* actions,
             AuvStepOut* out, void* stream);
int auv_step_host(const AuvConfig* cfg, const AuvRayTable* rays, const AuvPathBank* paths,
                  const AuvScenarioPool* pool, AuvBatch* batch, const float* actions_host,
                  float* actions_dev, AuvStepOut* out, float* obs_host, float* reward_host,
                  uint8_t* done_host, void* stream);
typedef struct AuvPipeline AuvPipeline;
AuvPipeline* auv_pipeline_create(int n_streams);
void auv_pipeline_destroy(AuvPipeline* p);
int auv_pipeline_graph_state(const AuvPipeline* p);
int auv_step_chunked(const AuvConfig* cfg, const AuvRayTable* rays, const AuvPathBank* paths,
                     const AuvScenarioPool* pool, AuvBatch* batch, const float* actions,
                     AuvStepOut* out, void* stream, AuvPipeline* p, int n_chunks);
int auv_step_host_chunked(const AuvConfig* cfg, const AuvRayTable* rays, const AuvPathBank* paths,
                          const AuvScenarioPool* pool, AuvBatch* batch, const float* actions_host,
                          float* actions_dev, AuvStepOut* out, float* obs_host, float* reward_host,
                          uint8_t* done_host, void* stream, AuvPipeline* p, int n_chunks);
int auv_step_host_submit(const AuvConfig* cfg, const AuvRayTable* rays, const AuvPathBank* paths,
                         const AuvScenarioPool* pool, AuvBatch* batch, const float* actions_host,
                         float* actions_dev, AuvStepOut* out, float* obs_host, float* reward_host,
                         uint8_t* done_host, void* stream, AuvPipeline* p, int n_chunks);
typedef struct AuvCompact {
  float* head;
  uint32_t* mask;
  float* vals;
  int32_t* counter;
  int32_t words;
  int32_t capacity;
} AuvCompact;
int auv_step_host_compact_submit(const AuvConfig* cfg, const AuvRayTable* rays, const AuvPathBank* paths,
                                 const AuvScenarioPool* pool, AuvBatch* batch, const float* actions_host,
                                 float* actions_dev, AuvStepOut* out, const AuvCompact* cb, float* reward_host,
                                 uint8_t* done_host, void* stream, AuvPipeline* p, int n_chunks);
int auv_compact_expand(const AuvConfig* cfg, int n_envs, const AuvCompact* cb, uint32_t* prev_mask, float* obs_host,
                       int n_threads);
typedef struct AuvDelta {
  float* obs_host;
  float* shadow;
  unsigned long long* shipped;
  int32_t gran;
  int32_t ctas;
} AuvDelta;
int auv_step_host_delta_submit(const AuvConfig* cfg, const AuvRayTable* rays, const AuvPathBank* paths,
                               const AuvScenarioPool* pool, AuvBatch* batch, const float* actions_host,
                               float* actions_dev, AuvStepOut* out, const AuvDelta* d, float* reward_host,
                               uint8_t* done_host, void* stream, AuvPipeline* p, int n_chunks);
typedef struct AuvTimer AuvTimer;
AuvTimer* auv_timer_create(int capacity);
void auv_timer_destroy(AuvTimer* t);
int auv_step_timed(const AuvConfig* cfg, const AuvRayTable* rays, const AuvPathBank* paths,
                   const AuvScenarioPool* pool, AuvBatch* batch, const float* actions,
                   AuvStepOut* out, void* stream, AuvTimer* t, int slot);
int auv_timer_read(AuvTimer* t, int slot, float* ms);
typedef struct AuvGenParams {
  uint64_t seed;
  uint32_t epoch;
  int32_t post_generate_update;
  double t_step_size;
  double vessel_width;
  double init_pos_jitter;
  double mov_disp_std;
  double mov_width_mean;
  double mov_speed_lo;
  double mov_speed_hi;
  double st_disp_std;
  double st_radius_mean;
  int32_t path_group;
  int32_t path_period;
  double land_clearance;
} AuvGenParams;
int auv_generate_moving_obstacles(const AuvGenParams* gp, const AuvPathBank* paths, const AuvScenarioPool* pool,
                                  const int32_t* ids, int n_ids, int32_t* status, void* stream);
int auv_reset_cache_fill(const AuvConfig* cfg, const AuvRayTable* rays, const AuvPathBank* paths,
                         const AuvScenarioPool* pool, AuvBatch* worker, AuvStepOut* worker_out, const int32_t* ids,
                         int first, int n, void* stream);
typedef struct AuvRefreshScratch {
  int32_t* seen_episode;
  int32_t* ids;
  int32_t* count;
  int32_t capacity;
  int32_t reserved0;
} AuvRefreshScratch;
int auv_refresh_finished(const AuvConfig* cfg, const AuvRayTable* rays, const AuvPathBank* paths,
                         const AuvScenarioPool* pool, const AuvBatch* live, AuvBatch* worker, AuvStepOut* worker_out,
                         const AuvRefreshScratch* rs, const AuvGenParams* gp, void* stream);
typedef struct AuvPathBuild {
  AuvPathHdr* hdr;
  double* poly_xy;
  double* poly_cum;
  float* poly_f32;
  float* blk_chord;
  float* blk_dev;
  float* sb_chord;
  float* sb_dev;
  double* pp;
  int32_t n_knots;
  int32_t vcap;
  float* sub_chord;
  float* sub_dev;
} AuvPathBuild;
int auv_pathbank_build(const double* waypoints, const int32_t* n_wp, const int32_t* path_ids, int n,
                       const AuvPathBuild* out, int32_t* status, void* stream);
int auv_random_curve_waypoints(uint64_t seed, uint32_t epoch, double length, const int32_t* path_ids, int n,
                               double* waypoints, int32_t* n_wp, void* stream);
int auv_linear_wrap(double dt, double counter0, int vel_len, int32_t* first_wrap, int32_t* wrap_period);
int auv_pool_pack(const AuvConfig* cfg, const AuvScenarioPool* pool, const int32_t* ids, int n_ids, void* stream);
int auv_obstacle_state(const AuvConfig* cfg, const AuvScenarioPool* pool, const AuvBatch* batch, double* pos,
                       double* disp, double* counter, void* stream);
int auv_fma_probe(float* sink, int blocks, int threads, int iters, void* stream,
                  double* flops_out);

#ifdef __cplusplus
}
#endif
#endif
```

Measured before the change: 414.9 million.

## Overlap finished-episode refresh on a high-priority stream with device-bounded launches

Adds an async refresh path that forks scenario regeneration and reset-cache fill onto a separate high-priority stream, joined before lidar in the chunked step and before any host-visible access. The collect kernel becomes a single-block deterministic prefix-scan instead of per-env atomics. Nav, cull and lidar kernels gain a LIMIT variant that early-exits blocks beyond a device-side live count, so oversized fixed grids do little work. This aims to hide refresh cost behind stepping, but adds many join points and risks races if a caller misses one.

```diff
diff --git a/gym_auv_b200/_lib.py b/gym_auv_b200/_lib.py
--- a/gym_auv_b200/_lib.py
+++ b/gym_auv_b200/_lib.py
@@ -273,6 +273,8 @@
     "auv_obstacle_state",
     "auv_reset_cache_fill",
     "auv_refresh_finished",
+    "auv_refresh_finished_async",
+    "auv_pipeline_join",
     "auv_step_host_compact_submit",
     "auv_step_host_delta_submit",
     "auv_compact_expand",
@@ -340,6 +342,10 @@
                                          P(AuvStepOut), _vp, C.c_int, C.c_int, _vp]
     lib.auv_refresh_finished.argtypes = [P(AuvConfig), P(AuvRayTable), P(AuvPathBank), P(AuvScenarioPool), P(AuvBatch),
                                          P(AuvBatch), P(AuvStepOut), P(AuvRefreshScratch), P(AuvGenParams), _vp]
+    lib.auv_refresh_finished_async.argtypes = [P(AuvConfig), P(AuvRayTable), P(AuvPathBank), P(AuvScenarioPool),
+                                               P(AuvBatch), P(AuvBatch), P(AuvStepOut), P(AuvRefreshScratch),
+                                               P(AuvGenParams), _vp, _vp]
+    lib.auv_pipeline_join.argtypes = [_vp, _vp]
     lib.auv_step_host_compact_submit.argtypes = [
         P(AuvConfig), P(AuvRayTable), P(AuvPathBank), P(AuvScenarioPool), P(AuvBatch), _vp, _vp, P(AuvStepOut),
         P(AuvCompact), _vp, _vp, _vp, _vp, C.c_int,
diff --git a/gym_auv_b200/csrc/auv_kernels.cu b/gym_auv_b200/csrc/auv_kernels.cu
--- a/gym_auv_b200/csrc/auv_kernels.cu
+++ b/gym_auv_b200/csrc/auv_kernels.cu
@@ -453,16 +453,41 @@
     for (int k = lane; k < wb.mask_words; k += 32)
       const_cast<uint32_t*>(pool.reset_mask)[(long long)m * wb.mask_words + k] = wb.nearby_mask[(long long)w * wb.mask_words + k];
 }
-__global__ void __launch_bounds__(128) k_refresh_collect(AuvBatch live, int n_scenarios, int* __restrict__ seen,
-                                                         int* __restrict__ ids, int* __restrict__ count, int capacity) {
-  const int e = blockIdx.x * blockDim.x + threadIdx.x;
-  if (e >= live.n_envs) return;
-  const int ep = live.episode[e];
-  if (ep == seen[e]) return;
-  const int k = atomicAdd(count, 1);
-  if (k >= capacity) return;
-  seen[e] = ep;
-  ids[k] = (int)(((long long)live.scn_id[e] + (live.reset_stride > 0 ? live.reset_stride : live.n_envs)) % n_scenarios);
+constexpr int REFRESH_COLLECT_THREADS = 1024;
+__global__ void __launch_bounds__(REFRESH_COLLECT_THREADS) k_refresh_collect(AuvBatch live, int n_scenarios, int* __restrict__ seen,
+                                                                             int* __restrict__ ids, int* __restrict__ count,
+                                                                             int capacity) {
+  __shared__ int warp_incl[REFRESH_COLLECT_THREADS / 32];
+  const int n = live.n_envs, t = threadIdx.x, lane = t & 31, wid = t >> 5;
+  const int per = (n + REFRESH_COLLECT_THREADS - 1) / REFRESH_COLLECT_THREADS;
+  const int e0 = min(n, t * per), e1 = min(n, e0 + per);
+  int cnt = 0;
+  for (int e = e0; e < e1; ++e) cnt += live.episode[e] != seen[e];
+  int incl = cnt;
+  for (int d = 1; d < 32; d <<= 1) {
+    const int v = __shfl_up_sync(AUV_FULL, incl, d);
+    if (lane >= d) incl += v;
+  }
+  if (lane == 31) warp_incl[wid] = incl;
+  __syncthreads();
+  if (wid == 0) {
+    int w = warp_incl[lane];
+    for (int d = 1; d < 32; d <<= 1) {
+      const int v = __shfl_up_sync(AUV_FULL, w, d);
+      if (lane >= d) w += v;
+    }
+    warp_incl[lane] = w;
+  }
+  __syncthreads();
+  int rank = incl - cnt + (wid > 0 ? warp_incl[wid - 1] : 0);
+  if (t == REFRESH_COLLECT_THREADS - 1) *count = rank + cnt;
+  const int stride = live.reset_stride > 0 ? live.reset_stride : n;
+  for (int e = e0; e < e1 && rank < capacity; ++e) {
+    const int ep = live.episode[e];
+    if (ep == seen[e]) continue;
+    seen[e] = ep;
+    ids[rank++] = (int)(((long long)live.scn_id[e] + stride) % n_scenarios);
+  }
 }
 
 template <int G>
@@ -538,7 +563,9 @@
                                                                 const double2* __restrict__ unit64,
                                                                 int* __restrict__ windows_out,
                                                                 const float* __restrict__ actions,
-                                                                float* __restrict__ obs_out, int obs_dim, int e0, int e1) {
+                                                                float* __restrict__ obs_out, int obs_dim, int e0, int e1,
+                                                                const int* __restrict__ n_live) {
+  if (!DYN && n_live != nullptr && (int)blockIdx.x * (AUV_NAV_THREADS / G) >= *n_live) return;
   extern __shared__ __align__(16) unsigned char nav_smem[];
   NavStage* stages = reinterpret_cast<NavStage*>(nav_smem);
   __shared__ __align__(8) unsigned long long s_bar[NAV_SUBBLOCKS];
@@ -626,12 +653,13 @@
     cull_env_group<G>(cfg, pool, batch, unit64, windows_out, e, scn, y.x, y.y, y.psi, step_counter, n_upd, lane, gm, store);
 }
 
-template <int G>
+template <int G, bool LIMIT = false>
 __global__ void __launch_bounds__(128, 8) k_nav_cull(const __grid_constant__ AuvConfig cfg, const __grid_constant__ AuvPathBank paths,
                                                      const __grid_constant__ AuvScenarioPool pool,
                                                      const __grid_constant__ AuvBatch batch, const double2* __restrict__ unit64,
                                                      int* __restrict__ windows_out, float* __restrict__ obs_out, int obs_dim,
-                                                     int e0, int e1) {
+                                                     int e0, int e1, const int* __restrict__ n_live) {
+  if (LIMIT && (int)blockIdx.x * (128 / G) >= *n_live) return;
   const int lane = threadIdx.x & 31, sub = lane & (G - 1);
   const unsigned gm = group_mask<G>(lane);
   const int eraw = e0 + (blockIdx.x * 128 + threadIdx.x) / G;
@@ -669,7 +697,7 @@
   AuvScenarioPool pool;
   AuvBatch batch;
   AuvStepOut out;
-  const void* pad0;
+  const int* n_live;
   int mode;
   int obs_dim;
   int e0, e1;
@@ -828,8 +856,9 @@
   }
 }
 
-template <bool COUNT, bool VEL, bool WORLD, bool TRACK = false>
+template <bool COUNT, bool VEL, bool WORLD, bool TRACK = false, bool LIMIT = false>
 __global__ void __launch_bounds__(AUV_LIDAR_THREADS, AUV_LIDAR_MINB) k_lidar(const __grid_constant__ LidarArgs A) {
+  if (LIMIT && (int)blockIdx.x * A.envs_per_cta >= *A.n_live) return;
   extern __shared__ __align__(16) unsigned char smem_raw[];
   constexpr int NW = AUV_LIDAR_THREADS / 32;
   const AuvConfig& cfg = A.cfg;
@@ -1590,7 +1619,8 @@
 static int launch_vessel_nav(const AuvConfig* cfg, const AuvRayTable* rays, const AuvPathBank* paths,
                              const AuvScenarioPool* pool, AuvBatch* batch, AuvStepOut* out,
                              const float* actions, void* stream, int e0 = 0, int cnt = -1, bool with_obstacles = false,
-                             cudaEvent_t between = nullptr ) {
+                             cudaEvent_t between = nullptr ,
+                             const int* n_live = nullptr ) {
   if ((paths->sub_chord == nullptr) != (paths->sub_dev == nullptr))
     return set_err(AUV_EINVAL, "paths: sub_chord and sub_dev are both set or both NULL");
   if (cnt < 0) cnt = batch->n_envs - e0;
@@ -1607,15 +1637,20 @@
   const int od = auv_obs_dim(cfg);
   cudaStream_t s = (cudaStream_t)stream;
   if (actions && with_obstacles && pool->k_moving > 0)
-    auv::k_vessel_nav<true, true, AUV_NAV_G><<<blocks, AUV_NAV_THREADS, nsm, s>>>(*cfg, *paths, *pool, *batch, unit, win, actions, obs, od, e0, e0 + cnt);
+    auv::k_vessel_nav<true, true, AUV_NAV_G><<<blocks, AUV_NAV_THREADS, nsm, s>>>(*cfg, *paths, *pool, *batch, unit, win, actions, obs, od, e0, e0 + cnt, nullptr);
   else if (actions)
-    auv::k_vessel_nav<true, false, AUV_NAV_G><<<blocks, AUV_NAV_THREADS, nsm, s>>>(*cfg, *paths, *pool, *batch, unit, win, actions, obs, od, e0, e0 + cnt);
+    auv::k_vessel_nav<true, false, AUV_NAV_G><<<blocks, AUV_NAV_THREADS, nsm, s>>>(*cfg, *paths, *pool, *batch, unit, win, actions, obs, od, e0, e0 + cnt, nullptr);
   else
-    auv::k_vessel_nav<false, false, AUV_NAV_G><<<blocks, AUV_NAV_THREADS, nsm, s>>>(*cfg, *paths, *pool, *batch, unit, win, nullptr, obs, od, e0, e0 + cnt);
+    auv::k_vessel_nav<false, false, AUV_NAV_G><<<blocks, AUV_NAV_THREADS, nsm, s>>>(*cfg, *paths, *pool, *batch, unit, win, nullptr, obs, od, e0, e0 + cnt,
+                                                                                        n_live);
   if (AUV_NAV_SPLIT) {
     if (int rc = cuda_check(cudaGetLastError(), "k_vessel_nav")) return rc;
     if (between != nullptr) cudaEventRecord(between, s);
-    auv::k_nav_cull<AUV_NAV_G><<<(cnt + 31) / 32, 128, 0, s>>>(*cfg, *paths, *pool, *batch, unit, win, obs, od, e0, e0 + cnt);
+    const unsigned cull_blocks = (unsigned)((cnt + 128 / AUV_NAV_G - 1) / (128 / AUV_NAV_G));
+    if (n_live != nullptr && !actions)
+      auv::k_nav_cull<AUV_NAV_G, true><<<cull_blocks, 128, 0, s>>>(*cfg, *paths, *pool, *batch, unit, win, obs, od, e0, e0 + cnt, n_live);
+    else
+      auv::k_nav_cull<AUV_NAV_G><<<cull_blocks, 128, 0, s>>>(*cfg, *paths, *pool, *batch, unit, win, obs, od, e0, e0 + cnt, nullptr);
     return cuda_check(cudaGetLastError(), "k_nav_cull");
   }
   return cuda_check(cudaGetLastError(), "k_vessel_nav");
@@ -1626,13 +1661,15 @@
   int dev = 0;
   if (cudaGetDevice(&dev) != cudaSuccess || dev < 0 || dev >= 64) dev = 0;
   if (smem <= g_lidar_smem_configured[dev].load(std::memory_order_acquire)) return 0;
-  const void* fns[12] = {(const void*)auv::k_lidar<false, false, false>, (const void*)auv::k_lidar<true, false, false>,
+  const void* fns[16] = {(const void*)auv::k_lidar<false, false, false>, (const void*)auv::k_lidar<true, false, false>,
                          (const void*)auv::k_lidar<false, true, false>,  (const void*)auv::k_lidar<true, true, false>,
                          (const void*)auv::k_lidar<false, false, true>,  (const void*)auv::k_lidar<true, false, true>,
                          (const void*)auv::k_lidar<false, true, true>,   (const void*)auv::k_lidar<true, true, true>,
                          (const void*)auv::k_lidar<false, false, false, true>, (const void*)auv::k_lidar<false, true, false, true>,
-                         (const void*)auv::k_lidar<false, false, true, true>,  (const void*)auv::k_lidar<false, true, true, true>};
-  for (int i = 0; i < 12; ++i)
+                         (const void*)auv::k_lidar<false, false, true, true>,  (const void*)auv::k_lidar<false, true, true, true>,
+                         (const void*)auv::k_lidar<false, false, false, false, true>, (const void*)auv::k_lidar<false, true, false, false, true>,
+                         (const void*)auv::k_lidar<false, false, true, false, true>,  (const void*)auv::k_lidar<false, true, true, false, true>};
+  for (int i = 0; i < 16; ++i)
     if (int rc = cuda_check(cudaFuncSetAttribute(fns[i], cudaFuncAttributeMaxDynamicSharedMemorySize, (int)smem),
                             "cudaFuncSetAttribute(k_lidar)"))
       return rc;
@@ -1656,7 +1693,7 @@
 
 static int launch_lidar(const AuvConfig* cfg, const AuvRayTable* rays, const AuvPathBank* paths,
                         const AuvScenarioPool* pool, AuvBatch* batch, AuvStepOut* out, int mode,
-                        void* stream, int e0 = 0, int cnt = -1) {
+                        void* stream, int e0 = 0, int cnt = -1, const int* n_live = nullptr) {
   if (cnt < 0) cnt = batch->n_envs - e0;
   auv::LidarArgs args;
   args.cfg = *cfg;
@@ -1669,6 +1706,7 @@
   args.obs_dim = auv_obs_dim(cfg);
   args.e0 = e0;
   args.e1 = e0 + cnt;
+  args.n_live = n_live;
   args.envs_per_cta = lidar_envs_per_cta(cfg);
   args.vmax = lidar_vmax(pool);
   args.clear_closeness = -cfg->sensor_range * exp(-0.1 * cfg->sensor_range);
@@ -1686,7 +1724,13 @@
   const bool world = pool->n_world > 0;
 #define AUV_LAUNCH_LIDAR(C, V, W) auv::k_lidar<C, V, W><<<blocks, AUV_LIDAR_THREADS, smem, s>>>(args)
 #define AUV_LAUNCH_LIDAR_TRACK(V, W) auv::k_lidar<false, V, W, true><<<blocks, AUV_LIDAR_THREADS, smem, s>>>(args)
-  if (track) {
+#define AUV_LAUNCH_LIDAR_LIMIT(V, W) auv::k_lidar<false, V, W, false, true><<<blocks, AUV_LIDAR_THREADS, smem, s>>>(args)
+  if (n_live != nullptr && !track && !count) {
+    if (world && vel) AUV_LAUNCH_LIDAR_LIMIT(true, true);
+    else if (world) AUV_LAUNCH_LIDAR_LIMIT(false, true);
+    else if (vel) AUV_LAUNCH_LIDAR_LIMIT(true, false);
+    else AUV_LAUNCH_LIDAR_LIMIT(false, false);
+  } else if (track) {
     if (world && vel) AUV_LAUNCH_LIDAR_TRACK(true, true);
     else if (world) AUV_LAUNCH_LIDAR_TRACK(false, true);
     else if (vel) AUV_LAUNCH_LIDAR_TRACK(true, false);
@@ -1704,6 +1748,7 @@
   }
 #undef AUV_LAUNCH_LIDAR
 #undef AUV_LAUNCH_LIDAR_TRACK
+#undef AUV_LAUNCH_LIDAR_LIMIT
   return cuda_check(cudaGetLastError(), "k_lidar");
 }
 
@@ -1743,6 +1788,9 @@
   cudaGraphExec_t gexec;
   unsigned long long gkey;
   int graph_state;
+  cudaStream_t rst;
+  cudaEvent_t rfork, rdone;
+  int refresh_armed;
 };
 
 AuvPipeline* auv_pipeline_create(int n_streams) {
@@ -1755,7 +1803,13 @@
   p->gexec = nullptr;
   p->gkey = 0;
   p->graph_state = getenv("AUV_B200_NO_GRAPH") ? -1 : 0;
+  p->refresh_armed = 0;
   bool ok = cudaEventCreateWithFlags(&p->fork, cudaEventDisableTiming) == cudaSuccess;
+  int prio_low = 0, prio_high = 0;
+  ok = ok && cudaDeviceGetStreamPriorityRange(&prio_low, &prio_high) == cudaSuccess &&
+       cudaStreamCreateWithPriority(&p->rst, cudaStreamNonBlocking, prio_high) == cudaSuccess &&
+       cudaEventCreateWithFlags(&p->rfork, cudaEventDisableTiming) == cudaSuccess &&
+       cudaEventCreateWithFlags(&p->rdone, cudaEventDisableTiming) == cudaSuccess;
   int made = 0;
   for (; ok && made < n_streams; ++made) {
     ok = cudaStreamCreateWithFlags(&p->st[made], cudaStreamNonBlocking) == cudaSuccess &&
@@ -1778,11 +1832,20 @@
   }
   for (int c = 0; c < AUV_PIPE_MAX_CHUNKS; ++c) cudaEventDestroy(p->chunk[c]);
   cudaEventDestroy(p->fork);
+  cudaStreamDestroy(p->rst);
+  cudaEventDestroy(p->rfork);
+  cudaEventDestroy(p->rdone);
   if (p->gexec) cudaGraphExecDestroy(p->gexec);
   delete p;
 }
 
 int auv_pipeline_graph_state(const AuvPipeline* p) { return p ? p->graph_state : AUV_EINVAL; }
+
+int auv_pipeline_join(AuvPipeline* p, void* stream) {
+  if (!p) return set_err(AUV_EINVAL, "pipeline is NULL");
+  if (!p->refresh_armed) return 0;
+  return cuda_check(cudaStreamWaitEvent((cudaStream_t)stream, p->rdone, 0), "refresh join");
+}
 
 static int chunk_size(int n, int n_chunks) {
   int c = (n + n_chunks - 1) / n_chunks;
@@ -1809,12 +1872,15 @@
       used = c + 1;
     }
     if (int rc = launch_vessel_nav(cfg, rays, paths, pool, batch, out, actions, vs, e0, cnt, true)) return rc;
+    if (p->refresh_armed)
+      if (int rc = cuda_check(cudaStreamWaitEvent(cst, p->rdone, 0), "refresh wait")) return rc;
     if (int rc = launch_lidar(cfg, rays, paths, pool, batch, out, AUV_OBSERVE_STEP, vs, e0, cnt)) return rc;
   }
   for (int i = 0; i < used; ++i) {
     if (int rc = cuda_check(cudaEventRecord(p->join[i], p->st[i]), "join record")) return rc;
     if (int rc = cuda_check(cudaStreamWaitEvent(s, p->join[i], 0), "join wait")) return rc;
   }
+  p->refresh_armed = 0;
   return 0;
 }
 
@@ -1919,6 +1985,8 @@
   if (n_chunks <= 0 || n_chunks > AUV_PIPE_MAX_CHUNKS) return set_err(AUV_EINVAL, "n_chunks out of range");
   if (int rc = check_observe_args(cfg, rays, paths, pool, batch, out, AUV_OBSERVE_STEP)) return rc;
   cudaStream_t s = (cudaStream_t)stream, ds = p->st[0];
+  if (int rc = auv_pipeline_join(p, stream)) return rc;
+  p->refresh_armed = 0;
   if (p->graph_state >= 0 && p->n_streams >= 2) {
     unsigned long long key = 1469598103934665603ull;
     key = fnv1a(key, cfg, sizeof(*cfg));
@@ -2249,7 +2317,8 @@
   auv::k_worker_fill<<<(wn + threads - 1) / threads, threads, 0, s>>>(*worker, ids, first, n, n_dev);
   if (int rc = cuda_check(cudaGetLastError(), "k_worker_fill")) return rc;
   if (int rc = auv_reset(cfg, pool, worker, nullptr, stream)) return rc;
-  if (int rc = auv_observe(cfg, rays, paths, pool, worker, wout, AUV_OBSERVE_RESET, stream)) return rc;
+  if (int rc = launch_vessel_nav(cfg, rays, paths, pool, worker, wout, nullptr, stream, 0, -1, false, nullptr, n_dev)) return rc;
+  if (int rc = launch_lidar(cfg, rays, paths, pool, worker, wout, AUV_OBSERVE_RESET, stream, 0, -1, n_dev)) return rc;
   auv::k_cache_scatter<<<(n * 32 + threads - 1) / threads, threads, 0, s>>>(*pool, *worker, wout->obs, auv_obs_dim(cfg),
                                                                           cfg->use_lidar, n, n_dev);
   return cuda_check(cudaGetLastError(), "k_cache_scatter");
@@ -2263,23 +2332,48 @@
   return reset_cache_fill(cfg, rays, paths, pool, worker, worker_out, ids, first, n, nullptr, stream);
 }
 
-int auv_refresh_finished(const AuvConfig* cfg, const AuvRayTable* rays, const AuvPathBank* paths,
-                         const AuvScenarioPool* pool, const AuvBatch* live, AuvBatch* worker, AuvStepOut* worker_out,
-                         const AuvRefreshScratch* rs, const AuvGenParams* gp, void* stream) {
+static int check_refresh(const AuvConfig* cfg, const AuvRayTable* rays, const AuvPathBank* paths, const AuvScenarioPool* pool,
+                         const AuvBatch* live, AuvBatch* worker, AuvStepOut* worker_out, const AuvRefreshScratch* rs,
+                         const AuvGenParams* gp) {
   if (!cfg || !paths || !pool || !live || !worker || !worker_out || !rs || !gp) return set_err(AUV_EINVAL, "NULL argument");
   if (!rs->seen_episode || !rs->ids || !rs->count || rs->capacity <= 0 || rs->capacity > worker->n_envs)
     return set_err(AUV_EINVAL, "refresh scratch: NULL array or capacity not in 1..worker.n_envs");
   if (pool->n_scenarios != 2 * (live->reset_stride > 0 ? live->reset_stride : live->n_envs))
     return set_err(AUV_EINVAL, "refresh needs a pool of exactly 2 * reset_stride (default n_envs) scenarios");
-  if (int rc = check_gen_world(gp, pool)) return rc;
-  cudaStream_t s = (cudaStream_t)stream;
-  const int threads = 128;
-  if (int rc = cuda_check(cudaMemsetAsync(rs->count, 0, sizeof(int32_t), s), "memset")) return rc;
-  auv::k_refresh_collect<<<(live->n_envs + threads - 1) / threads, threads, 0, s>>>(*live, pool->n_scenarios, rs->seen_episode,
-                                                                                    rs->ids, rs->count, rs->capacity);
+  if (!pool->reset_obs || !pool->reset_max_progress || (cfg->use_lidar && !pool->reset_mask))
+    return set_err(AUV_EINVAL, "pool.reset_* is NULL");
+  if (int rc = check_observe_args(cfg, rays, paths, pool, worker, worker_out, AUV_OBSERVE_RESET)) return rc;
+  return check_gen_world(gp, pool);
+}
+
+static int enqueue_refresh(const AuvConfig* cfg, const AuvRayTable* rays, const AuvPathBank* paths,
+                           const AuvScenarioPool* pool, const AuvBatch* live, AuvBatch* worker, AuvStepOut* worker_out,
+                           const AuvRefreshScratch* rs, const AuvGenParams* gp, cudaStream_t s) {
+  auv::k_refresh_collect<<<1, auv::REFRESH_COLLECT_THREADS, 0, s>>>(*live, pool->n_scenarios, rs->seen_episode, rs->ids,
+                                                                      rs->count, rs->capacity);
   if (int rc = cuda_check(cudaGetLastError(), "k_refresh_collect")) return rc;
   if (int rc = launch_generate(gp, paths, pool, rs->ids, rs->capacity, rs->count, live->status, s)) return rc;
-  return reset_cache_fill(cfg, rays, paths, pool, worker, worker_out, rs->ids, 0, rs->capacity, rs->count, stream);
+  return reset_cache_fill(cfg, rays, paths, pool, worker, worker_out, rs->ids, 0, rs->capacity, rs->count, (void*)s);
+}
+
+int auv_refresh_finished(const AuvConfig* cfg, const AuvRayTable* rays, const AuvPathBank* paths,
+                         const AuvScenarioPool* pool, const AuvBatch* live, AuvBatch* worker, AuvStepOut* worker_out,
+                         const AuvRefreshScratch* rs, const AuvGenParams* gp, void* stream) {
+  if (int rc = check_refresh(cfg, rays, paths, pool, live, worker, worker_out, rs, gp)) return rc;
+  return enqueue_refresh(cfg, rays, paths, pool, live, worker, worker_out, rs, gp, (cudaStream_t)stream);
+}
+
+int auv_refresh_finished_async(const AuvConfig* cfg, const AuvRayTable* rays, const AuvPathBank* paths,
+                               const AuvScenarioPool* pool, const AuvBatch* live, AuvBatch* worker, AuvStepOut* worker_out,
+                               const AuvRefreshScratch* rs, const AuvGenParams* gp, void* stream, AuvPipeline* p) {
+  if (!p) return set_err(AUV_EINVAL, "pipeline is NULL");
+  if (int rc = check_refresh(cfg, rays, paths, pool, live, worker, worker_out, rs, gp)) return rc;
+  if (int rc = cuda_check(cudaEventRecord(p->rfork, (cudaStream_t)stream), "refresh fork")) return rc;
+  if (int rc = cuda_check(cudaStreamWaitEvent(p->rst, p->rfork, 0), "refresh fork wait")) return rc;
+  const int rc = enqueue_refresh(cfg, rays, paths, pool, live, worker, worker_out, rs, gp, p->rst);
+  p->refresh_armed = 1;
+  if (int rc2 = cuda_check(cudaEventRecord(p->rdone, p->rst), "refresh done")) return rc ? rc : rc2;
+  return rc;
 }
 
 int auv_pathbank_build(const double* waypoints, const int32_t* n_wp, const int32_t* path_ids, int n,
diff --git a/gym_auv_b200/vec_env.py b/gym_auv_b200/vec_env.py
--- a/gym_auv_b200/vec_env.py
+++ b/gym_auv_b200/vec_env.py
@@ -466,6 +466,7 @@
         M, Km = self.scenarios.n_scenarios, self.k_moving
         if Km and self._pool["vel_table"].shape[0] < M * Km:
             raise ValueError("pool.vel_table must hold n_scenarios * k_moving entries (constant-velocity tracks)")
+        self.join_refresh()
         gp = self.gen_params(seed, epoch)
         self._pool["host_stale"] = True
         idp, n = None, M
@@ -487,6 +488,7 @@
         bank = self.scenarios.bank
         if not isinstance(bank, DevicePathBank):
             raise ValueError("regenerate_paths needs a device-built path bank (scenarios built with device_paths=True)")
+        self.join_refresh()
         n = bank.n_paths
         idp = None
         if ids is not None:
@@ -517,6 +519,7 @@
         N, M = self.reset_stride or self.num_envs, self.scenarios.n_scenarios
         if M != 2 * N:
             raise ValueError("refresh_finished needs a pool of exactly 2 * reset_stride (default num_envs) scenarios")
+        self.join_refresh()
         ep = self._st["episode"]
         if getattr(self, "_seen_episode", None) is None:
             self._seen_episode = torch.zeros_like(ep)
@@ -536,6 +539,7 @@
         capacity = int(min(capacity, 65536))
         rs = getattr(self, "_refresh", None)
         if rs is None or rs["cap"] != capacity:
+            self.join_refresh()
             dev = self.device
             rs = self._refresh = dict(
                 cap=capacity, seen=self._st["episode"].clone(), ids=torch.zeros(capacity, dtype=torch.int32, device=dev),
@@ -549,13 +553,23 @@
         self._pool["host_stale"] = True
         cfg, rays, paths, pool, batch = self._refs()
         with torch.cuda.device(self.device):
-            _lib.check(self.lib.auv_refresh_finished(cfg, rays, paths, pool, batch, C.byref(w.batch), C.byref(w.out),
-                                                     C.byref(rs["struct"]), C.byref(gp), self._stream()),
-                       "auv_refresh_finished")
+            if self._pipe and self.chunks > 1:
+                _lib.check(self.lib.auv_refresh_finished_async(cfg, rays, paths, pool, batch, C.byref(w.batch), C.byref(w.out),
+                                                               C.byref(rs["struct"]), C.byref(gp), self._stream(), self._pipe),
+                           "auv_refresh_finished_async")
+            else:
+                _lib.check(self.lib.auv_refresh_finished(cfg, rays, paths, pool, batch, C.byref(w.batch), C.byref(w.out),
+                                                         C.byref(rs["struct"]), C.byref(gp), self._stream()),
+                           "auv_refresh_finished")
+
+    def join_refresh(self):
+        if self._pipe:
+            _lib.check(self.lib.auv_pipeline_join(self._pipe, self._stream()), "auv_pipeline_join")
 
     def pull_scenarios(self) -> ScenarioSet:
         import dataclasses
 
+        self.join_refresh()
         p = self._pool
         h = lambda k: p[k].cpu().numpy().copy()
         return dataclasses.replace(
@@ -568,6 +582,7 @@
         return dict(ray=self._ray, bank=self._bank, pool=self._pool, linear=self.linear)
 
     def obstacle_state(self):
+        self.join_refresh()
         if self.linear is None:
             return self._st["mov_pos"], self._st["mov_disp"], self._st["mov_counter"]
         N, Km = self.num_envs, max(self.k_moving, 1)
@@ -588,6 +603,7 @@
         return C.byref(self.cfg), C.byref(self.rays), C.byref(self.paths), C.byref(self.pool), C.byref(self.batch)
 
     def check_status(self):
+        self.join_refresh()
         st = int(self._scratch["status"].item())
         if st & _lib.STATUS_GEN_GAVE_UP:
             raise RuntimeError("scenario generator: an obstacle slot was still rejected after 100000 draws")
@@ -616,6 +632,7 @@
         return self.observation_dict(obs) if self.dict_observation else obs
 
     def reset(self, check: bool = True) -> torch.Tensor:
+        self.join_refresh()
         cfg, rays, paths, pool, batch = self._refs()
         with torch.cuda.device(self.device):
             _lib.check(self.lib.auv_reset(cfg, pool, batch, None, self._stream()), "auv_reset")
@@ -628,6 +645,7 @@
         return self._fmt(self._out["obs"])
 
     def reset_envs(self, mask: torch.Tensor, scenario_ids: Optional[torch.Tensor] = None) -> torch.Tensor:
+        self.join_refresh()
         mask = mask.to(device=self.device, dtype=torch.uint8).contiguous()
         if scenario_ids is not None:
             sel = mask.bool()
@@ -654,6 +672,7 @@
                     "auv_step_chunked",
                 )
             else:
+                self.join_refresh()
                 _lib.check(
                     self.lib.auv_step(cfg, rays, paths, pool, batch, C.c_void_p(a.data_ptr()), C.byref(self.out), self._stream()),
                     "auv_step",
@@ -665,6 +684,7 @@
         if self.host_transfer != "dense":
             self.step_async(actions)
             return self.step_wait()
+        self.join_refresh()
         pin = self.step_host_buffers()
         pin["act"].numpy()[...] = actions
         cfg, rays, paths, pool, batch = self._refs()
@@ -818,23 +838,27 @@
         )
 
     def obstacle_update(self):
+        self.join_refresh()
         cfg, _, _, pool, batch = self._refs()
         with torch.cuda.device(self.device):
             _lib.check(self.lib.auv_obstacle_update(cfg, pool, batch, self._stream()), "auv_obstacle_update")
 
     def vessel_step(self, actions: torch.Tensor):
+        self.join_refresh()
         a = actions.to(device=self.device, dtype=torch.float32).contiguous()
         cfg, _, _, _, batch = self._refs()
         with torch.cuda.device(self.device):
             _lib.check(self.lib.auv_vessel_step(cfg, batch, C.c_void_p(a.data_ptr()), self._stream()), "auv_vessel_step")
 
     def navigate(self):
+        self.join_refresh()
         cfg, rays, paths, pool, batch = self._refs()
         with torch.cuda.device(self.device):
             _lib.check(self.lib.auv_navigate(cfg, rays, paths, pool, batch, self._stream()), "auv_navigate")
         return self._st["nav"]
 
     def observe(self, mode=_lib.OBSERVE_STEP):
+        self.join_refresh()
         cfg, rays, paths, pool, batch = self._refs()
         with torch.cuda.device(self.device):
             _lib.check(
@@ -874,6 +898,7 @@
                                 self._path_table, self.scenarios.world_polygons)
 
     def last_episode(self, i: int) -> Optional[dict]:
+        self.join_refresh()
         slot = self._track_slot(i)
         if slot is None:
             return None
@@ -886,6 +911,7 @@
         return self._assemble(head[p], tk["points"][slot, p].cpu().numpy(), tk["snap"][slot, p].cpu().numpy())
 
     def current_episode(self, i: int) -> Optional[dict]:
+        self.join_refresh()
         slot = self._track_slot(i)
         if slot is None:
             return None
@@ -936,6 +962,7 @@
 
     def close(self):
         if self._pipe:
+            self.join_refresh()
             torch.cuda.synchronize(self.device)
             self.lib.auv_pipeline_destroy(self._pipe)
             self._pipe = None
diff --git a/include/auv_b200.h b/include/auv_b200.h
--- a/include/auv_b200.h
+++ b/include/auv_b200.h
@@ -312,6 +312,10 @@
 int auv_refresh_finished(const AuvConfig* cfg, const AuvRayTable* rays, const AuvPathBank* paths,
                          const AuvScenarioPool* pool, const AuvBatch* live, AuvBatch* worker, AuvStepOut* worker_out,
                          const AuvRefreshScratch* rs, const AuvGenParams* gp, void* stream);
+int auv_refresh_finished_async(const AuvConfig* cfg, const AuvRayTable* rays, const AuvPathBank* paths,
+                               const AuvScenarioPool* pool, const AuvBatch* live, AuvBatch* worker, AuvStepOut* worker_out,
+                               const AuvRefreshScratch* rs, const AuvGenParams* gp, void* stream, AuvPipeline* p);
+int auv_pipeline_join(AuvPipeline* p, void* stream);
 typedef struct AuvPathBuild {
   AuvPathHdr* hdr;
   double* poly_xy;
```

New measurement: 390.2 million (median of 6 runs). -6.0%, worse.
